# dbking77/ar_slam

Hardware: AMD Instinct MI355X
Metric: LM iterations/sec + ms-to-converged reproj-RMS, 10k-capture synthetic graph (higher is better)
Workload: dtype f64

## Files before the change

### ar_slam_amd/csrc/lm_capi.hip

```cpp
#include "lm_handle.h"

arslam_lm::~arslam_lm() {
  for (auto &t : timers) t.destroy();
  for (auto e : upd_events) (void)hipEventDestroy(e);
  if (ev_sync) (void)hipEventDestroy(ev_sync);
  for (auto e : cov_ev)
    if (e) (void)hipEventDestroy(e);
  arslam::selinv_plan_free(cov_sp);
  for (auto e : pair_ev)
    if (e) (void)hipEventDestroy(e);
  arslam::tile_solve_plan_free(cov_tp);
  arslam::llt_plan_free(plan);
  if (comm) (void)ncclCommDestroy(comm);
  if (stream) (void)hipStreamDestroy(stream);
}


namespace {
thread_local std::string g_last_error;
}
namespace arslam {
void set_last_error(const std::string &msg) { g_last_error = msg; }
}
namespace {
// ... 310 lines not shown
            "parameter block is not part of the problem");
    fail_if(!h->pk_loaded || h->pk_dirty, ARSLAM_E_STATE,
            "covariance_block: no completed arslam_lm_solve of the problem as it stands");
    if (!h->cov_valid) h->covariance();
    if (key == h->camera_ptr) {
      std::fill(cov, cov + 9, 0.0);
      cov[0] = h->cov_var_f;
      const bool ok = h->cov_var_f >= 0.0;
      if (!ok) std::fill(cov, cov + 9, -1.0);
      if (status)
        *status = ok ? ARSLAM_COV_OK
                     : h->cov_info.status == ARSLAM_COV_RANK_DEFICIENT && !h->constant.count(key) ? ARSLAM_COV_RANK_DEFICIENT
                                                                                                   : ARSLAM_COV_UNAVAILABLE;
      return;
    }
    const bool is_cap = ci != h->cap_of.end();
    const int i = is_cap ? ci->second : ti->second;
    const std::vector<double> &c = is_cap ? h->cov_cap : h->cov_tag;
    const std::vector<int> &st = is_cap ? h->cov_cap_status : h->cov_tag_status;
    fail_if((size_t)i >= st.size(), ARSLAM_E_STATE, "covariance_block: the block is not part of the solved problem");
    std::memcpy(cov, c.data() + 36L * i, 36 * sizeof(double));
    if (status) *status = st[i];
  });
}

int arslam_lm_covariance_pairs(arslam_lm *h, const arslam_lm_cov_pair *pairs, int n_pairs, double *cov, int *status,
                               arslam_lm_cov_info *info) {
  if (!h || n_pairs < 0 || (n_pairs > 0 && (!pairs || !cov))) return ARSLAM_E_INVALID_ARG;
  return guarded([&] { h->covariance_pairs(pairs, n_pairs, cov, status, info); });
}

int arslam_lm_covariance_block_pair(arslam_lm *h, const double *block_a, const double *block_b, double *cov,
                                    int *status) {
  if (!h || !block_a || !block_b || !cov) return ARSLAM_E_INVALID_ARG;
  return guarded([&] {
    arslam_lm_cov_pair pr{};
    int size[2] = {6, 6};
    const double *blocks[2] = {block_a, block_b};
    for (int s = 0; s < 2; ++s) {
      double *key = const_cast<double *>(blocks[s]);
      const auto ci = h->cap_of.find(key);
      const auto ti = h->tag_of.find(key);
      fail_if(key != h->camera_ptr && ci == h->cap_of.end() && ti == h->tag_of.end(), ARSLAM_E_INVALID_ARG,
              "parameter block is not part of the problem");
      const int kind = key == h->camera_ptr ? ARSLAM_BLOCK_CAMERA : ci != h->cap_of.end() ? ARSLAM_BLOCK_CAPTURE : ARSLAM_BLOCK_TAG;
      const int index = kind == ARSLAM_BLOCK_CAMERA ? 0 : kind == ARSLAM_BLOCK_CAPTURE ? ci->second : ti->second;
      if (kind == ARSLAM_BLOCK_CAMERA) size[s] = 3;
      (s == 0 ? pr.kind_a : pr.kind_b) = kind;
      (s == 0 ? pr.index_a : pr.index_b) = index;
    }
    fail_if(!h->pk_loaded || h->pk_dirty, ARSLAM_E_STATE,
            "covariance_block_pair: no completed arslam_lm_solve of the problem as it stands");
    double c[36];
    int st = ARSLAM_COV_UNAVAILABLE;
    h->covariance_pairs(&pr, 1, c, &st, nullptr);
    const int ra = size[0], cb = size[1];
    if (st != ARSLAM_COV_OK) {
      std::fill(cov, cov + ra * cb, -1.0);
    } else {
      std::fill(cov, cov + ra * cb, 0.0);
      if (ra == 6 && cb == 6) std::copy(c, c + 36, cov);
      else if (ra == 3 && cb == 6) std::copy(c, c + 6, cov);
      else if (ra == 6 && cb == 3) for (int r = 0; r < 6; ++r) cov[3 * r] = c[r];
      else cov[0] = c[0];
    }
    if (status) *status = st;
  });
}

int arslam_lm_debug_reduced_rows(arslam_lm *h, int *cap_row, int *tag_row, int *cam_row) {
  if (!h) return ARSLAM_E_INVALID_ARG;
  return guarded([&] {
    fail_if(!h->loaded || h->multi() || h->elim_used == ARSLAM_ELIM_MIXED, ARSLAM_E_STATE,
            "reduced_rows: a one-rank problem loaded with capture or tag elimination");
    const bool swapped = h->elim_used == ARSLAM_ELIM_TAGS;
    int *e_row = swapped ? tag_row : cap_row, *f_row = swapped ? cap_row : tag_row;
    for (int c = 0; c < h->nc && e_row; ++c) e_row[c] = -1;
    for (int t = 0; t < h->nt && f_row; ++t) f_row[t] = (size_t)t < h->lay.tag_row.size() ? h->lay.tag_row[t] : -1;
    if (cam_row) *cam_row = h->has_f ? h->P.cam_row : -1;
  });
}

int arslam_comm_unique_id(unsigned char id[ARSLAM_COMM_ID_BYTES]) {
  if (!id) return ARSLAM_E_INVALID_ARG;
  return guarded([&] {
    static_assert(sizeof(ncclUniqueId) <= ARSLAM_COMM_ID_BYTES, "id size");
    ncclUniqueId u;
    NCCL_CHECK(ncclGetUniqueId(&u));
    std::memset(id, 0, ARSLAM_COMM_ID_BYTES);
    std::memcpy(id, &u, sizeof(u));
  });
}

int arslam_lm_set_comm_callback(arslam_lm *h, int rank, int nranks, arslam_allreduce_fn fn, void *ctx) {
  if (!h || nranks < 1 || rank < 0 || rank >= nranks || ((nranks > 1 || h->force_multi) && !fn))
    return ARSLAM_E_INVALID_ARG;
  return guarded([&] {
    if (h->comm) { (void)ncclCommDestroy(h->comm); h->comm = nullptr; }
    h->rank = rank;
    h->nranks = nranks;
    h->comm_cb = h->multi() ? fn : nullptr;
    h->comm_cb_ctx = ctx;
    h->loaded = false;
    h->pk_dirty = true;
  });
}

int arslam_lm_set_comm(arslam_lm *h, int rank, int nranks, const unsigned char id[ARSLAM_COMM_ID_BYTES]) {
  if (!h || !id || nranks < 1 || rank < 0 || rank >= nranks) return ARSLAM_E_INVALID_ARG;
  return guarded([&] {
    h->ensure_stream();
    if (h->comm) { (void)ncclCommDestroy(h->comm); h->comm = nullptr; }
    h->comm_cb = nullptr;
    h->rank = rank;
    h->nranks = nranks;
    h->loaded = false;
    h->pk_dirty = true;
    if (h->multi()) {
      ncclUniqueId u;
      std::memcpy(&u, id, sizeof(u));
      NCCL_CHECK(ncclCommInitRank(&h->comm, nranks, u, rank));
    }
  });
}

int arslam_lm_owned_captures(const arslam_lm *h, int *out, int cap, int *n) {
  if (!h || !n || (cap > 0 && !out)) return ARSLAM_E_INVALID_ARG;
  if (!h->loaded) return ARSLAM_E_STATE;
  const int k = h->multi() ? (int)h->own_caps.size() : h->nc_user;
  for (int i = 0; i < k && i < cap; ++i) out[i] = h->multi() ? h->own_caps[i] : i;
  *n = k;
  return ARSLAM_OK;
}

int arslam_device_count(void) {
  int n = 0;
  if (hipGetDeviceCount(&n) != hipSuccess) return 0;
  return n;
}

int arslam_lm_set_iteration_callback(arslam_lm *h, arslam_iteration_callback fn, void *ctx) {
  if (!h) return ARSLAM_E_INVALID_ARG;
  h->iter_cb = fn;
  h->iter_cb_ctx = ctx;
  return ARSLAM_OK;
}

int arslam_lm_debug_force_indefinite(arslam_lm *h, unsigned long long step_mask) {
  if (!h) return ARSLAM_E_INVALID_ARG;
  h->dbg_indefinite_mask = step_mask;
  return ARSLAM_OK;
}

int arslam_lm_debug_force_multirank(arslam_lm *h, int on) {
  if (!h || (on != 0 && on != 1)) return ARSLAM_E_INVALID_ARG;
  return guarded([&] {
    if (h->comm) { (void)ncclCommDestroy(h->comm); h->comm = nullptr; }
    h->comm_cb = nullptr;
    h->rank = 0;
    h->nranks = 1;
    h->force_multi = on != 0;
    h->loaded = false;
    h->pk_dirty = true;
  });
}

int arslam_lm_debug_break_dependency(arslam_lm *h, long ticket, long *broken) {
  if (!h || ticket < 0) return ARSLAM_E_INVALID_ARG;
  return guarded([&] {
    fail_if(!h->loaded || !h->has_f || h->opt.factor_executor != 1, ARSLAM_E_STATE,
            "break_dependency needs a loaded problem on the persistent executor");
    arslam::LltPlan &pl = h->plan;
    long t = ticket;
    while (t < pl.n_dag_tasks && pl.h_dag_wait_off[t] == pl.h_dag_wait_off[t + 1]) ++t;
    fail_if(t >= pl.n_dag_tasks, ARSLAM_E_INVALID_ARG, "no task at or after this ticket waits on anything");
    const int w = pl.h_dag_wait_off[t];
    h->restore_patched_wait();
    pl.h_dag_waits[w].y += 1 << 28;
    h->dbg_patched_wait = w;
    HIP_CHECK(hipMemcpyAsync(pl.dag_waits + w, &pl.h_dag_waits[w], sizeof(int2), hipMemcpyHostToDevice,
                             h->stream));
    HIP_CHECK(hipStreamSynchronize(h->stream));
    if (broken) *broken = t;
  });
}

int arslam_lm_debug_tag_pair_tile(arslam_lm *h, const double *tag_a, const double *tag_b, int *status) {
  if (!h || !tag_a || !tag_b || !status) return ARSLAM_E_INVALID_ARG;
  return guarded([&] {
    fail_if(!h->loaded || h->multi() || h->elim_used != ARSLAM_ELIM_CAPTURES || !h->has_f, ARSLAM_E_STATE,
            "tag_pair_tile needs a pointer-keyed problem loaded with capture elimination on one rank");
    const auto ia = h->tag_of.find(const_cast<double *>(tag_a)), ib = h->tag_of.find(const_cast<double *>(tag_b));
    *status = -1;
    if (ia == h->tag_of.end() || ib == h->tag_of.end()) return;
    const int ra = h->lay.tag_row[ia->second], rb = h->lay.tag_row[ib->second];
    if (ra < 0 || rb < 0) return;
    const int T = h->lay.T;
    int st = 2;
    for (int x : {ra, ra + 5})
      for (int y : {rb, rb + 5}) {
        int ti = x / 64, tj = y / 64;
        if (ti < tj) std::swap(ti, tj);
        const int id = h->plan.h_tile_id[(size_t)ti * T + tj];
        st = std::min(st, id < 0 ? 0 : (id < h->plan.n_assembled ? 2 : 1));
      }
    *status = st;
  });
}

const char *arslam_lm_last_error(void) { return g_last_error.c_str(); }

#ifndef ARSLAM_BUILD_ID
#define ARSLAM_BUILD_ID "unknown"
#endif
const char *arslam_lm_version(void) { return "arslam_lm 0.2 (gfx950, fp64) build " ARSLAM_BUILD_ID; }

}
```

### ar_slam_amd/csrc/lm_handle.h

```cpp
#pragma once
#include "host_threads.h"
#include "lm_internal.h"
#include "loss.h"
#include "arslam_lm.h"
#include "arslam_lm_debug.h"

#include <rccl/rccl.h>

#include <algorithm>
#include <atomic>
#include <cfloat>
#include <chrono>
#include <cmath>
#include <cstddef>
#include <cstdio>
#include <cstdlib>
#include <cstring>
#include <memory>
#include <stdexcept>
#include <string>
#include <unordered_map>
#include <thread>
#include <unordered_set>
#include <vector>

namespace arslam {
namespace lmh {

using Error = arslam::ApiError;

#define HIP_CHECK(expr)                                                                      \
  do {                                                                                       \
    hipError_t _e = (expr);                                                                  \
    if (_e != hipSuccess)                                                                    \
      throw Error(_e == hipErrorOutOfMemory ? ARSLAM_E_OUT_OF_MEMORY : ARSLAM_E_HIP,         \
                  std::string(#expr) + ": " + hipGetErrorString(_e));                       \
  } while (0)

#define NCCL_CHECK(expr)                                                                     \
  do {                                                                                       \
    ncclResult_t _r = (expr);                                                                \
    if (_r != ncclSuccess)                                                                   \
      throw Error(ARSLAM_E_COMM, std::string(#expr) + ": " + ncclGetErrorString(_r));       \
  } while (0)

inline void fail_if(bool cond, int code, const std::string &msg) {
  if (cond) throw Error(code, msg);
}

inline double now_s() {
  return std::chrono::duration<double>(std::chrono::steady_clock::now().time_since_epoch()).count();
}

struct DebugEnv {
  const char *dag_trace = std::getenv("ARSLAM_DAG_TRACE");
  int dag_trace_skip = std::getenv("ARSLAM_DAG_TRACE_SKIP") ? std::atoi(std::getenv("ARSLAM_DAG_TRACE_SKIP")) : 0;
  bool setup_profile = std::getenv("ARSLAM_SETUP_PROFILE") != nullptr;
  bool write_back_dma = std::getenv("ARSLAM_WRITE_BACK_DMA") != nullptr;
};
inline const DebugEnv &debug_env() {
  static const DebugEnv e;
  return e;
}

std::string executor_fault_message(int code, int rank, int iteration, const arslam::LltPlan &plan, hipStream_t s);

template <class T>
struct DevBuf {
  T *p = nullptr;
  size_t n = 0, cap = 0;
  void alloc(size_t count) {
    n = count;
    if (count <= cap) return;
    if (p) (void)hipFree(p);
    p = nullptr;
    cap = 0;
    const size_t want = cap == 0 && count <= 16 ? count : count + count / 2;
    HIP_CHECK(hipMalloc(&p, want * sizeof(T)));
    cap = want;
  }
  void upload(const T *h, size_t count, hipStream_t s) {
    if (count) HIP_CHECK(hipMemcpyAsync(p, h, count * sizeof(T), hipMemcpyHostToDevice, s));
  }
  void release() {
    if (p) (void)hipFree(p);
    p = nullptr;
    n = cap = 0;
  }
  ~DevBuf() { release(); }
};

struct PinnedBuf {
  double *p = nullptr;
  size_t cap = 0;
  void alloc(size_t count) {
    if (count <= cap) return;
    if (p) (void)hipHostFree(p);
    p = nullptr;
    cap = 0;
    const size_t want = count + count / 2;
    HIP_CHECK(hipHostMalloc(&p, want * sizeof(double), hipHostMallocDefault));
    cap = want;
  }
  ~PinnedBuf() {
    if (p) (void)hipHostFree(p);
  }
};

struct UploadArena {
  char *dev = nullptr, *host = nullptr;
  size_t dev_cap = 0, host_cap = 0;
  struct Piece { void **dst; const void *src; size_t bytes, off; };
  std::vector<Piece> pieces;
  hipEvent_t copied = nullptr;
  template <class T>
  void add(T **dst, const T *src, size_t count) { pieces.push_back({reinterpret_cast<void **>(dst), src, count * sizeof(T), 0}); }
  void commit(hipStream_t s) {
    if (copied) HIP_CHECK(hipEventSynchronize(copied));
    size_t used = 0;
    for (Piece &p : pieces) {
      p.off = used;
      used += (std::max<size_t>(p.bytes, 1) + 255) & ~size_t(255);
    }
    if (used > host_cap) {
      if (host) (void)hipHostFree(host);
      host = nullptr;
      host_cap = 0;
      HIP_CHECK(hipHostMalloc(&host, used + used / 2, hipHostMallocDefault));
      host_cap = used + used / 2;
    }
    if (used > dev_cap) {
      if (dev) (void)hipFree(dev);
      dev = nullptr;
      dev_cap = 0;
      HIP_CHECK(hipMalloc(&dev, used + used / 2));
      dev_cap = used + used / 2;
    }
    for (Piece &p : pieces) {
      if (p.bytes) std::memcpy(host + p.off, p.src, p.bytes);
      *p.dst = dev + p.off;
    }
    if (used) {
      HIP_CHECK(hipMemcpyAsync(dev, host, used, hipMemcpyHostToDevice, s));
      if (!copied) HIP_CHECK(hipEventCreateWithFlags(&copied, hipEventDisableTiming));
      HIP_CHECK(hipEventRecord(copied, s));
    }
    pieces.clear();
  }
  ~UploadArena() {
    if (copied) (void)hipEventDestroy(copied);
    if (dev) (void)hipFree(dev);
    if (host) (void)hipHostFree(host);
  }
};

struct Timer {
  hipEvent_t a = nullptr, b = nullptr;
  double acc_ms = 0.0;
  bool pending = false;
  bool on = true;
  void init() {
    if (!a) {
      HIP_CHECK(hipEventCreateWithFlags(&a, hipEventDisableSystemFence));
      HIP_CHECK(hipEventCreateWithFlags(&b, hipEventDisableSystemFence));
    }
  }
  void start(hipStream_t s) {
    if (on) HIP_CHECK(hipEventRecord(a, s));
  }
  void stop(hipStream_t s) {
    if (!on) return;
    HIP_CHECK(hipEventRecord(b, s));
    pending = true;
  }
  void collect() {
    if (!pending) return;
    float ms = 0.f;
    HIP_CHECK(hipEventSynchronize(b));
    HIP_CHECK(hipEventElapsedTime(&ms, a, b));
    acc_ms += ms;
    pending = false;
  }
  void destroy() {
    if (a) (void)hipEventDestroy(a);
    if (b) (void)hipEventDestroy(b);
    a = b = nullptr;
  }
};

enum { PH_LIN, PH_SCHUR, PH_CHOL, PH_SOLVE, PH_BACK, PH_COST, PH_FAC0, PH_FAC1, PH_N };

}
}
using namespace arslam::lmh;

struct arslam_lm {
  arslam_lm_options opt;

  double *camera_ptr = nullptr;
  std::unordered_map<double *, int> cap_of, tag_of;
  std::vector<double *> cap_ptrs, tag_ptrs;
  std::vector<int> pk_obs_cap, pk_obs_tag;
  std::vector<double> pk_corners;
  std::vector<unsigned char> pk_loss_kind;
  std::vector<double> pk_loss_a;
  int def_loss_kind = ARSLAM_LOSS_NONE;
  double def_loss_a = 0.0;
  std::vector<unsigned char> soa_loss_kind;
  std::vector<double> soa_loss_a;
  arslam::ObsLoss default_obs_loss(int n_obs) {
    if (def_loss_kind == ARSLAM_LOSS_NONE || n_obs <= 0) return arslam::ObsLoss{};
    soa_loss_kind.assign(n_obs, (unsigned char)def_loss_kind);
    soa_loss_a.assign(n_obs, def_loss_a);
    return arslam::ObsLoss{soa_loss_kind.data(), soa_loss_a.data()};
  }
  std::unordered_set<double *> constant;
  bool pk_dirty = true;

  bool loaded = false;
  arslam_soa_problem soa{};
  int nc = 0, nt = 0, nb = 0;
  long n = 0, nR = 0, N = 0;
  bool has_f = false;
  std::vector<unsigned char> slot_free;
  std::vector<double> x0;
  long nb_global = 0;
  double setup_s = 0.0;
  double setup_phase[5] = {0, 0, 0, 0, 0};
  double comm_bytes = 0.0;
  long comm_calls = 0;
  arslam::DevProblem P{};
  hipStream_t stream = nullptr;
  int device = 0;

  UploadArena upload;
  int *u_cap_start = nullptr, *u_obs_tag = nullptr, *u_obs_lblk = nullptr, *u_cap_blk_start = nullptr,
      *u_blk_tag = nullptr, *u_tag_start = nullptr, *u_obs_tpos = nullptr, *u_tag_row = nullptr,
      *u_row_slot = nullptr, *u_fslot_row = nullptr, *u_dest_start = nullptr, *u_big_caps = nullptr;
  unsigned char *u_f_own = nullptr;
  unsigned char *u_cap_kind = nullptr;
  int *u_f_alias = nullptr;
  std::vector<unsigned char> f_own;
  std::vector<int> big_caps;
  std::vector<int> chunk_caps;
  int *u_chunk_caps = nullptr;
  unsigned char *u_obs_active = nullptr, *u_slot_free = nullptr;
  double *u_corners = nullptr, *u_x0 = nullptr;
  unsigned char *u_loss_kind = nullptr;
  double *u_loss_a = nullptr;
  long *u_cap_off = nullptr;
  int2 *u_dest_row = nullptr;
  int4 *u_gather_items = nullptr, *u_gather_splits = nullptr;
  arslam::SchurContrib *u_contrib = nullptr;
  long n_clear = 0;
  DevBuf<double> d_xa, d_xb, d_xbest, d_g, d_colnorm, d_scale, d_diag;
  DevBuf<double> d_obs_tg, d_parts, d_fparts, d_red, d_S, d_z, d_yF;
  double *Sp = nullptr;
  long s_pre = 0;
  int *u_top_slots = nullptr;
  int n_top_slots = 0;
  long top_tail_len() const { return 2L * n_top_slots + 2; }
  double *d_norms_p = nullptr;
  DevBuf<int> d_flag;
  DevBuf<double> d_slab, d_jrows, d_cap_ui;
  DevBuf<double> d_gather_part;
  arslam::LltPlan plan;
  double *x = nullptr, *xc = nullptr, *xbest = nullptr;
  unsigned long long dbg_indefinite_mask = 0;
  arslam_iteration_callback iter_cb = nullptr;
  void *iter_cb_ctx = nullptr;
  int n_fparts = 0;

  Timer timers[PH_N];
  arslam::LaunchTiming upd_timing;
  std::vector<hipEvent_t> upd_events;
  double dom_ms = 0.0, dom_flops = 0.0;
  double scalar_flops = 0.0;
  long dom_launches = 0;

  void timing_begin();
  void timing_collect();

  int rank = 0, nranks = 1;
  ncclComm_t comm = nullptr;
  bool force_multi = false;
  bool multi() const { return nranks > 1 || force_multi; }

  ~arslam_lm();

  arslam_allreduce_fn comm_cb = nullptr;
  void *comm_cb_ctx = nullptr;
  std::vector<unsigned char> comm_stage;

  void allreduce_any(void *buf, size_t count, int dtype, int op);
  void allreduce(double *buf, size_t count, int op) { allreduce_any(buf, count, ARSLAM_DT_F64, op); }

  DevBuf<double> d_split_hash;
  void check_same_split(const arslam::RankSplit &sp);

  int dag_workgroups = 512;
  const DebugEnv &env = debug_env();

  int cus_device = -1, cus = 0;
  std::thread::id ready_thread{};
  int ready_opt_device = -2;
  void ensure_stream();

  void load(const arslam_soa_problem *p, const arslam::ObsLoss &in_loss);
  int choose_side(const arslam::SchurSide &cs);
  void local_rank_problem(const arslam_soa_problem *p, const arslam::ObsLoss &in_loss, bool can_reuse,
                          arslam::HostProblem &h, arslam::ReducedLayout &L, std::vector<int> &col_class);
  void upload_problem(const arslam::HostProblem &h, const arslam::ReducedLayout &L, int extend_from = -1);
  void alloc_solve_buffers();
  arslam::SchurGather sg;
  bool sg_ready = false;
  bool try_append(const arslam_soa_problem *p, const arslam::ObsLoss &in_loss);
  bool append_as_captures(const arslam_soa_problem *p);
  bool append_as_mixed(const arslam_soa_problem *p, arslam::MixedProblem &m);
  bool same_reduced_rows(const arslam::HostProblem &h) const;
  bool groups_fit_plan(const arslam::HostProblem &h, const std::vector<int> &groups) const;
  bool order_outgrown(const arslam::HostProblem &h, const std::vector<int> &groups);
  arslam::ReducedLayout lay;
  bool pk_appended_only = false;
  int setup_kind = ARSLAM_SETUP_LOAD;
  int elim_used = ARSLAM_ELIM_CAPTURES;
  arslam::MixedProblem mx;
  int ceres_e_cap = 0, ceres_e_tag = 0;
  void reload_values(const arslam_soa_problem *p);
  bool pk_loaded = false;
  int nc_full = 0;
  int nc_user = 0;
  std::vector<int> own_caps;
  std::vector<double> loc_cap, loc_corners;
  std::vector<int> loc_obs_cap, loc_obs_tag;
  std::vector<unsigned char> loc_cap_const;
  std::vector<unsigned char> loc_loss_kind;
  std::vector<double> loc_loss_a;
  double split_top_work = 0.0, split_max_rank_work = 0.0, split_total_work = 0.0;
  int split_active = 1;
  std::vector<uint64_t> covis;
  long covis_nt = 0, covis_edges = 0;
  void covis_build(const arslam::HostProblem &h, const arslam::ReducedLayout &L);
  void covis_add(const arslam::HostProblem &h, const arslam::ReducedLayout &L, int c);
  bool reuse_order = false;
  std::vector<int> prev_tag_row;
  std::vector<int> prev_mx_tag_row, prev_mx_cap_row;
  int prev_ordering = -1, prev_skip = -1;
  long prev_order_edges = 0;
  int prev_order_nc = 0;
  bool last_order_reused = false;
  int prev_order_height = 0;
  static int etree_height(const arslam::ReducedLayout &L);
  void linearize(double *x_cost, double *fixed_cost, double *gmax, double *gnorm, double *xnorm);
  void linearize_launch();
  void linearize_collect(double *x_cost, double *fixed_cost, double *gmax, double *gnorm, double *xnorm);
  bool lin_xpending = false, norms_pending = false;
  DevBuf<double> d_lx, d_ag;
  static constexpr int kLinSave = 16 + 8 + 6 * arslam::kNormBlocks;
  void complete_pending_lin();
  void lin_norms();
  void exchange_scalars(arslam::AgFields fl, arslam::HostOut *ho = nullptr);
  void exchange_norms() {
    if (norms_pending) exchange_scalars(arslam::AgFields{});
  }
  PinnedBuf h_lin;
  double lin_seq = 0.0;
  void lin_sync() {
    if (!multi() && lin_seq > 0.0) flag_sync(h_lin.p + 16 + arslam::kHostSeq, lin_seq);
    else spin_sync();
  }
  bool diag_in_lin = false;
  PinnedBuf h_x;
  PinnedBuf h_step;
  hipEvent_t ev_sync = nullptr;
  void spin_sync() {
    if (!ev_sync) HIP_CHECK(hipEventCreateWithFlags(&ev_sync, hipEventDisableTiming));
    HIP_CHECK(hipEventRecord(ev_sync, stream));
    hipError_t e;
    while ((e = hipEventQuery(ev_sync)) == hipErrorNotReady) {
    }
    HIP_CHECK(e);
  }
  double host_seq = 0.0;
  DevBuf<int> d_seq_done;
  double next_seq(double *word) {
    *(volatile double *)word = -1.0;
    return host_seq += 1.0;
  }
  void flag_sync(const double *word, double seq) {
    for (long k = 1;; ++k) {
      if (*(const volatile double *)word == seq) break;
      if ((k & 4095) == 0) {
        const hipError_t e = hipStreamQuery(stream);
        if (e == hipErrorNotReady) continue;
        HIP_CHECK(e);
        if (*(const volatile double *)word == seq) break;
        throw Error(ARSLAM_E_DEVICE, "the stream finished without storing the host sequence word");
      }
    }
    std::atomic_thread_fence(std::memory_order_acquire);
  }
  void solve(arslam_lm_summary *s);
  void begin_solve(arslam_lm_summary *s);
  double enqueue_step(double radius, bool reuse_diag, int solve_index);
  bool prepare_step(bool reuse_diag, arslam::ExecReset *er);
  void factor_reduced(long first_store, bool record, double radius = 0.0, bool force_indefinite = false);
  void dump_dag_trace(long first_store);
  void back_substitute(double radius);
  double reduce_step_scalars();
  void fill_summary(arslam_lm_summary *s);
  void write_back(const double *d_src);
  const arslam_soa_problem *pk_stage = nullptr;
  void scatter_to_blocks();
  int dbg_patched_wait = -1;
  void restore_patched_wait();
  bool any_iter_cb = false;
  DevBuf<double> d_cb;
  int agree_callback(int r);

  int solve_state = 0;
  arslam::SelinvPlan cov_sp;
  bool cov_sp_ready = false;
  DevBuf<double> d_cov_Z, d_cov_Q, d_cov_Y, d_cov_R, d_cov_out, d_cov_diag;
  DevBuf<int> d_cov_status;
  hipEvent_t cov_ev[5] = {nullptr, nullptr, nullptr, nullptr, nullptr};
  bool cov_valid = false;
  std::vector<double> cov_cap, cov_tag;
  std::vector<int> cov_cap_status, cov_tag_status;
  double cov_var_f = -1.0;
  arslam_lm_cov_info cov_info{};
  void covariance();
  void cov_invalidate() {
    solve_state = 0;
    cov_valid = false;
  }
  struct CovFactor {
    std::vector<int> cap_start;
    bool deficient = false;
    bool factored = false;
    arslam_lm_cov_info info{};
  };
  bool cov_e_free(int c) const { return slot_free[3 + 6L * c] != 0; }
  bool cov_f_free(int t) const { return slot_free[3 + 6L * nc + 6L * t] != 0; }
  void cov_check_state(const char *who) const;
  void cov_factor(CovFactor &cf);
  void cov_numeric_test(CovFactor &cf);

  arslam::TileSolvePlan cov_tp;
  bool cov_tp_ready = false;
  static constexpr int kCovBatchPanels = 16;
  static constexpr size_t kCovBatchBytes = 256u << 20;
  DevBuf<unsigned char> d_pair_mask;
  DevBuf<double> d_pair_B, d_pair_out;
  DevBuf<int2> d_pair_rhs;
  DevBuf<arslam::CovPairTask> d_pair_tasks;
  DevBuf<int> d_pair_status;
  std::vector<hipEvent_t> pair_ev;
  void covariance_pairs(const arslam_lm_cov_pair *pairs, int n_pairs, double *cov, int *status,
                        arslam_lm_cov_info *info);
};
```

### ar_slam_amd/csrc/lm_internal.h

```cpp
#pragma once
#include <hip/hip_runtime.h>
#include <algorithm>
#include <climits>
#include <cstdint>
#include <stdexcept>
#include <vector>

#include "host_structure.h"

namespace arslam {
constexpr int kCuFlags = 2048;
constexpr int kDagOffTicket0 = 0;
constexpr int kDagOffInflight = 1;
constexpr int kDagOffCuFlags = 2;
constexpr int kDagOffTicket1 = 2 + kCuFlags;
constexpr int kDagOffFault = 3 + kCuFlags;
enum DagFaultField {
  kFaultTicket = 0,
  kFaultKind = 1,
  kFaultCounter = 2,
  kFaultSeen = 3,
  kFaultNeed = 4,
  kFaultDrawn = 5,
  kFaultInflight = 6,
// ... 93 lines not shown
  const int4 *gather_splits;
  double *gather_part;
  int n_items, n_splits;
  const signed char *tile_class;
  const unsigned char *f_own = nullptr;
  double *jrows;
  double *cap_ui;
  const unsigned char *obs_loss_kind = nullptr;
  const double *obs_loss_a = nullptr;
};

__device__ inline double *reduced_elem(double *S, const DevProblem &P, long r, long c) {
  return S + (long)P.tile_id[(r >> 6) * P.T + (c >> 6)] * 4096 + (r & 63) * 64 + (c & 63);
}

#ifndef ARSLAM_NORM_BLOCKS
#define ARSLAM_NORM_BLOCKS 64
#endif
constexpr int kNormBlocks = ARSLAM_NORM_BLOCKS;
static_assert(kNormBlocks <= 256 && (kNormBlocks & (kNormBlocks - 1)) == 0, "k_slot_norms: one 256-thread tree");

enum DagRecField {
  kRecType = 0, kRecY, kRecZ, kRecW,
  kRecSub, kRecLate, kRecWait0, kRecWait1,
  kRecCont, kRecContAkk, kRecMaxdep,
  kRecContMaxdep, kRecContWait0, kRecContLate,
  kRecQ0 = 16, kRecQ1,
  kRecFoldK0, kRecFoldTile0,
  kRecSid = 18, kRecTi, kRecTj,
  kRecSplitN, kRecSplitP,
  kRecTile0I, kRecTile0J,
  kDagRecInts = 32
};

enum DagTraceWord {
  kTrDraw = 0,
  kTrMet = 1,
  kTrEnd = 2,
  kTrWg = 3,
  kTrLoaded = 4,
  kTrFactored = 5,
  kTrPublished = 6,
  kTrSubPublished = 7,
  kDagTraceWords = 8
};
enum DagProgressSlot {
  kProgTicket = 0,
  kProgPhase = 1,
  kProgType = 2,
  kDagProgressInts = 4
};

struct LltPlan {
  char *arena = nullptr;
  size_t arena_bytes = 0;
  int T = 0;
  long lda = 0;
  int nlev = 0;
  int2 *panel = nullptr;
  int2 *upd_targets = nullptr;
  int *upd_kstart = nullptr;
  int *upd_ks = nullptr;
  int4 *upd_items = nullptr;
  int2 *upd_split = nullptr;
  int *upd_cnt = nullptr;
  double *upd_part = nullptr;
  long n_split = 0, n_part = 0;
  std::vector<int> h_item_off;
  int *bs_cols = nullptr;
  int2 *bs_gather = nullptr;
  int *bs_gbeg = nullptr;
  int *bs_gtile = nullptr;
  double *bs_part = nullptr;
  int *bs_counters = nullptr;
  int *tile_id = nullptr;
  std::vector<int> h_tile_id;
  long n_tiles = 0;
  long n_assembled = 0;
  bool fill_first_ok = false;
  int n_phases = 1;
  long phase_split = 0;
  long n_top_tiles = 0;
  std::vector<int> h_col_class;
  std::vector<int> h_dag_phase;
  signed char *tile_class = nullptr;
  double *ldiag = nullptr;
  std::vector<int> h_panel_off;
  std::vector<int> h_upd_off;
  std::vector<int> h_bs_off;
  std::vector<int> h_bsg_off;
  std::vector<double> h_upd_flops;
  std::vector<int2> h_dag_sub;
  int *dag_claimed = nullptr;
  std::vector<int> h_dag_cont, h_dag_maxdep, h_dag_cont_akk;
  int *dag_rec = nullptr;
  int2 *dag_ks_tiles = nullptr;
  std::vector<int> h_dag_rec;
  std::vector<int2> h_dag_ks_tiles;
  int2 *dag_waits = nullptr;
  int *dag_counters = nullptr;
  long n_dag_tasks = 0;
  std::vector<int4> h_dag_tasks;
  std::vector<int> h_dag_wait_off;
  std::vector<int2> h_dag_waits;
  std::vector<int2> h_panel, h_targets, h_gather, h_split;
  std::vector<int> h_kstart, h_ks, h_bcols, h_gbeg, h_gtile;
  std::vector<int4> h_items;
  double total_upd_flops = 0.0;
  double total_factor_flops = 0.0;
  long total_upd_tiles = 0;
};

void llt_plan_symbolic(LltPlan &plan, int T, long lda, std::vector<uint8_t> &pattern,
                       const std::vector<int> *col_class = nullptr);
void tile_fill(int T, std::vector<uint8_t> &pattern, std::vector<int> &parent);
struct RankSplit {
  std::vector<int> col_owner;
  std::vector<int> cap_owner;
  int n_top_cols = 0;
  int n_active = 0;
  double top_work = 0.0, max_rank_work = 0.0, total_work = 0.0;
  std::vector<int> col_class(int rank) const {
    std::vector<int> c(col_owner.size());
    for (size_t k = 0; k < c.size(); ++k) c[k] = col_owner[k] < 0 ? 1 : (col_owner[k] == rank ? 0 : 2);
    return c;
  }
};
RankSplit rank_split(const HostProblem &h, const ReducedLayout &L, int nranks);
bool dag_check(const LltPlan &plan);
bool dag_simulate(const LltPlan &plan, int n_workers, unsigned seed, int policy = 0, int n_started = -1);
constexpr int kDagSimPolicies = 4;
constexpr int kDagSimNoCap = 16;
constexpr int kDagSimGridCap = 32;
std::string dag_fault_detail(const LltPlan &plan, const int *rec);
void llt_plan_upload(LltPlan &plan, hipStream_t s);
void llt_plan_build(LltPlan &plan, int T, long lda, std::vector<uint8_t> &pattern, hipStream_t s,
                    const std::vector<int> *col_class = nullptr);
void llt_plan_free(LltPlan &plan);
void llt_plan_reset(LltPlan &plan);


struct ExecReset;
void launch_linearize(const DevProblem &P, const double *x, double *g, double *colnorm,
                      double *obs_tg, double *parts, hipStream_t s);
void launch_lin_reduce(const DevProblem &P, const double *obs_tg, double *g, double *colnorm,
                       const double *parts, double *out, hipStream_t s, double *hout = nullptr,
                       double *save = nullptr);
struct LmDiagArgs;
void launch_scale(const DevProblem &P, const double *colnorm, int jacobi, double *scale,
                  hipStream_t s, const LmDiagArgs *ld = nullptr);
void launch_lm_diag(const DevProblem &P, const double *scale, const double *colnorm, double dmin,
                    double dmax, double *diag, hipStream_t s);
void set_schur_big_lds_attribute();
void launch_schur(const DevProblem &P, const double *x, const double *scale, const double *diag,
                  double radius, double *S, hipStream_t s, bool prep = false, long zero_tiles = 0,
                  const ExecReset *er = nullptr);
void launch_schur_gather(const DevProblem &P, const double *diag, double radius, double *S, hipStream_t s);
void launch_prep_reduced(const DevProblem &P, const double *diag, double radius, double *S,
                         hipStream_t s, int which = -1);
void launch_mask_y(const DevProblem &P, double *yF, int rank, hipStream_t s, bool keep_top = false);
void launch_own_copy(const DevProblem &P, long first, long count, const double *src, double *dst, hipStream_t s);
void launch_backsub(const DevProblem &P, const double *x, const double *scale, const double *diag,
                    double radius, const double *yF, double *xc, double *parts, hipStream_t s,
                    bool reuse_ui = false, bool with_cost = false);
void launch_update_f(const DevProblem &P, const double *x, const double *scale, const double *yF,
                     double *xc, double *fparts, hipStream_t s);
void launch_cost(const DevProblem &P, const double *x, double *parts, hipStream_t s);
void launch_copy_out(const double *src, long n, double *dst, int *seq_done, double *word, double seq, hipStream_t s);
void launch_reduce_parts(const double *parts, int nc, const double *fparts, int nfparts,
                         double *out, hipStream_t s, const int *flag = nullptr,
                         double *hout = nullptr, int *seq_done = nullptr, double seq = 0.0);
void debug_set_reduced_diag(const DevProblem &P, double *S, long row, double v, hipStream_t s);
struct PackSegs {
  int n = 0;
  double *p[4] = {nullptr, nullptr, nullptr, nullptr};
  long len[4] = {0, 0, 0, 0}, off[4] = {0, 0, 0, 0};
  void add(double *ptr, long count) {
    p[n] = ptr;
    len[n] = count;
    off[n] = n ? off[n - 1] + len[n - 1] : 0;
    ++n;
  }
  long total() const { return n ? off[n - 1] + len[n - 1] : 0; }
};
void launch_pack(const PackSegs &sg, double *buf, bool unpack, hipStream_t s);
void launch_top_tail(const int *idx, int m, double *g, double *cn, double *red, double *tail, bool unpack,
                     hipStream_t s);
constexpr int kAgFields = 32;
struct AgFields {
  int n = 0;
  int idx[kAgFields] = {};
  unsigned max = 0;
  void add(int i, bool is_max) {
    if (n >= kAgFields) throw std::logic_error("AgFields: more than kAgFields scalars");
    if (is_max) max |= 1u << n;
    idx[n++] = i;
  }
};
void launch_ag_put(const double *src, const AgFields &fl, double *ag, int nranks, int rank, hipStream_t s);
struct HostOut {
  const double *src[3] = {};
  double *dst[3] = {};
  int len[3] = {};
  int n = 0;
  double *seq_word = nullptr;
  double seq = 0.0;
  void add(const double *s, double *d, int l) {
    if (n >= 3) throw std::logic_error("HostOut: more than 3 ranges");
    src[n] = s;
    dst[n] = d;
    len[n++] = l;
  }
};
void launch_ag_reduce(const double *ag, const AgFields &fl, double *dst, int nranks, hipStream_t s,
                      const HostOut *ho = nullptr);
void launch_slot_norms(const DevProblem &P, const double *red, double *g, double *colnorm, const double *x,
                       double *out, hipStream_t s, double *hout = nullptr, const LmDiagArgs *ld = nullptr,
                       double seq = 0.0);
constexpr int kHostSeq = 15;

struct LaunchTiming {
  hipEvent_t *ev = nullptr;
  int cap = 0;
  int used = 0;
  double flops = 0.0;
};

void launch_dense_llt(const LltPlan &P, double *S, int *flag, hipStream_t s,
                      LaunchTiming *timing = nullptr);
void set_dag_workgroup_limit(int k);
inline int dag_launch_grid(long n_tasks, int n_workgroups) {
  return (int)std::min<long>(n_workgroups, std::max<long>(std::min<long>(64, n_tasks), n_tasks / 4));
}
void launch_dense_llt_dag(const LltPlan &P, double *S, int *flag, hipStream_t s, int n_workgroups,
                          int *progress = nullptr, unsigned long long *trace = nullptr, bool reset = true,
                          int phase = -1, long first_store = LONG_MAX);
struct LmDiagArgs {
  long n;
  const double *scale, *colnorm;
  double dmin, dmax;
  double *diag;
  double *ysent = nullptr;
  long nys = 0;
};
constexpr unsigned long long kYSentinel = 0x7ff47ff47ff47ff4ull;
void launch_exec_reset(const LltPlan &P, int *flag, hipStream_t s, const LmDiagArgs *ld = nullptr);
struct ExecReset {
  int *flag = nullptr;
  int *a = nullptr, *b = nullptr, *c = nullptr, *d = nullptr;
  long na = 0, nb = 0, nc = 0, nd = 0;
  double *ysent = nullptr;
  long nys = 0;
  __host__ __device__ long n() const { return na + nb + nc + nd > nys ? na + nb + nc + nd : nys; }
};
ExecReset exec_reset_args(const LltPlan &P, int *flag, double *ysent, long nys);
__device__ __forceinline__ void exec_reset_elem(const ExecReset &r, long e) {
  if (e < r.nys) r.ysent[e] = __longlong_as_double((long long)kYSentinel);
  if (e < r.na) r.a[e] = 0;
  else if (e < r.na + r.nb) r.b[e - r.na] = 0;
  else if (e < r.na + r.nb + r.nc) r.c[e - r.na - r.nb] = 0;
  else if (e < r.na + r.nb + r.nc + r.nd) r.d[e - r.na - r.nb - r.nc] = 0;
  if (e == 0 && r.flag) *r.flag = 0;
}
void launch_dense_back_solve(const LltPlan &P, const double *S, long nR, double *z, double *yF,
                             const int *flag, hipStream_t s);
void launch_dense_back_solve_dag(const LltPlan &P, const double *S, long nR, double *yF, int *flag,
                                 hipStream_t s, int n_workgroups, bool reset = true);
void launch_zero_tiles(const LltPlan &P, double *S, hipStream_t s);
void launch_scatter_diag(const LltPlan &P, double *S, hipStream_t s);

struct SelinvPlan {
  int *gcol = nullptr;
  long n_products = 0;
};
void selinv_plan_build(const LltPlan &P, SelinvPlan &sp, hipStream_t s);
void selinv_plan_free(SelinvPlan &sp);
void launch_selinv(const LltPlan &P, const SelinvPlan &sp, double *S, long nR, double *Z, const int *flag,
                   hipStream_t s);
void launch_cov_blocks(const DevProblem &P, const double *Z, const double *scale, const double *Gb, const double *Rb,
                       double *cov_e, int *status_e, double *cov_f, double *var_f, const int *flag, hipStream_t s);
void launch_cov_schur(const DevProblem &P, const double *scale, double *Qb, double *Gb, double *Rb, bool write_slab,
                      hipStream_t s);

struct TileSolvePlan {
  int *fbeg = nullptr;
  int2 *flist = nullptr;
  std::vector<int> h_fbeg;
  std::vector<int2> h_flist;
  std::vector<int> parent;
};
void tile_solve_plan_build(const LltPlan &P, TileSolvePlan &tp, hipStream_t s);
void tile_solve_plan_free(TileSolvePlan &tp);
void tile_solve_mark(const TileSolvePlan &tp, unsigned char *mask, long row);
long tile_solve_products(const LltPlan &P, const TileSolvePlan &tp, const unsigned char *active,
                         const unsigned char *needed);
void launch_tile_solve(const LltPlan &P, const TileSolvePlan &tp, const double *S, long nR, double *B, int n_panels,
                       const unsigned char *active, const unsigned char *needed, const int *flag, hipStream_t s);
enum { kCovFocal = 0, kCovF = 1, kCovE = 2 };
constexpr int kCovPanelBlocks = 10;
void launch_cov_pair_rhs(const DevProblem &P, const double *Gb, const double *Rb, const int2 *rhs, int n_rhs,
                         double *B, hipStream_t s);
struct CovPairTask {
  int role_a, idx_a, role_b, idx_b, slot, out;
};
void launch_cov_pair_blocks(const DevProblem &P, const double *X, const double *scale, const double *Gb,
                            const double *Rb, const CovPairTask *tasks, int n_tasks, double *out, int *status,
                            const int *flag, hipStream_t s);

}
// ... 1 lines not shown
```

### ar_slam_amd/csrc/lm_kernels.hip

```cpp
#include "lm_internal.h"
#include "projection.h"
#include "loss.h"
#include "schur_store_table.h"

#include <cfloat>
#include <mutex>
#include <string>
#include <vector>

#include "arslam_lm.h"
#include <cmath>

namespace arslam {

#ifdef ARSLAM_SCHUR_STAMPS
__device__ unsigned long long g_schur_ph[16];
#define SCHUR_STAMP_INIT unsigned long long _st0 = clock64()
#define SCHUR_STAMP(k)                                                         \
  do {                                                                         \
    const unsigned long long _n = clock64();                                   \
    if (threadIdx.x == 0) atomicAdd(&g_schur_ph[k], _n - _st0);                \
    _st0 = _n;                                                                 \
  } while (0)
void debug_read_schur_stamps(unsigned long long *out) {
  (void)hipMemcpyFromSymbol(out, HIP_SYMBOL(g_schur_ph), sizeof(g_schur_ph));
}
#else
#define SCHUR_STAMP_INIT do {} while (0)
#define SCHUR_STAMP(k) do {} while (0)
void debug_read_schur_stamps(unsigned long long *out) {
  for (int i = 0; i < 16; ++i) out[i] = 0;
}
#endif

namespace {

__device__ const SchurStoreTable g_schur_store = make_schur_store_table();

__device__ __forceinline__ long slot_cap(const DevProblem &P, int c) { return 3 + 6L * c; }
__device__ __forceinline__ long slot_tag(const DevProblem &P, int t) { return 3 + 6L * P.nc + 6L * t; }

__device__ __forceinline__ bool group_swapped(const DevProblem &P, int c) {
  return P.cap_kind ? P.cap_kind[c] == kMixTag : P.swap_roles != 0;
}
__device__ __forceinline__ bool group_direct(const DevProblem &P, int c) {
  return P.cap_kind && P.cap_kind[c] == kMixDirect;
}

__device__ __forceinline__ double lm_d2(const double *diag, long slot, double radius) {
  const double d = sqrt(diag[slot] / radius);
  return d * d;
}

__device__ __forceinline__ double robustify_row(int kind, double a, double &r, double J[13]) {
  const double s = obs_sum8(r * r);
  double rho, rho1;
  loss_eval(kind, a, s, &rho, &rho1);
  const double w = sqrt(rho1);
#pragma unroll
  for (int j = 0; j < 13; ++j) J[j] *= w;
  r *= w;
  return rho;
}

template <bool kLoss = false>
__device__ __forceinline__ void fill_rows(const DevProblem &P, const double *x, const double *scale, int c,
                          int o0, int row0, int nr, int nrows, double *rows, double *gout = nullptr,
                          double *ocost = nullptr) {
  const double *cam = x;
  const double *cap = x + slot_cap(P, c);
  for (int lr = threadIdx.x; lr < nr; lr += kWave) {
    const int row = row0 + lr;
    const int q = row >> 3, corner = (row >> 1) & 3, comp = row & 1;
    const int obs = o0 + q;
    const int t = P.obs_tag[obs];
    const double *tag = x + slot_tag(P, t);
    double J[13];
    const bool sw = group_swapped(P, c);
    double r = residual_jacobian_row(cam, sw ? tag : cap, sw ? cap : tag, corner, comp,
                                     P.corners[8L * obs + 2 * corner + comp], J);
    if (kLoss) {
      const double rho = robustify_row(P.obs_loss_kind[obs], P.obs_loss_a[obs], r, J);
      if (ocost && (lr & 7) == 0) ocost[lr >> 3] = 0.5 * rho;
    }
    if (sw) {
#pragma unroll
      for (int j = 1; j < 7; ++j) {
        const double v = J[j];
        J[j] = J[j + 6];
        J[j + 6] = v;
      }
    }
    double *dst = rows + (long)lr * kRowStride;
    if (scale) {
      const double *sc = scale + slot_cap(P, c);
      const double *st = scale + slot_tag(P, t);
      dst[0] = J[0] * scale[0];
#pragma unroll
      for (int j = 0; j < 6; ++j) {
        dst[1 + j] = J[1 + j] * sc[j];
        dst[7 + j] = J[7 + j] * st[j];
      }
    } else {
#pragma unroll
      for (int j = 0; j < 13; ++j) dst[j] = J[j];
    }
    dst[13] = r;
    if (gout) {
      double *g = gout + 8L * o0 * kJStored + row;
#pragma unroll
      for (int j = 0; j < 13; ++j)
        if (j < 7 || j > 9) g[(long)jrow_col(j) * nrows] = J[j];
      g[(long)jrow_col(13) * nrows] = r;
    }
  }
}

__device__ __forceinline__ void load_rows_q(const DevProblem &P, const double *scale, const double *yF, double yf, int c, int o0,
                            int row0, int nr, int nrows, double *rows, double *qv) {
  const double *sc = scale + slot_cap(P, c);
  for (int lr = threadIdx.x; lr < nr; lr += kWave) {
    const int row = row0 + lr;
    const double *g = P.jrows + 8L * o0 * kJStored + row;
    const int t = P.obs_tag[o0 + (row >> 3)];
    const int tr = P.tag_row[t];
    double u[kJStored], v[14];
#pragma unroll
    for (int j = 0; j < kJStored; ++j) u[j] = g[(long)j * nrows];
#pragma unroll
    for (int j = 0; j < 14; ++j) v[j] = u[jrow_col(j)];
    const double *st = scale + slot_tag(P, t);
    double yt[6];
#pragma unroll
    for (int j = 0; j < 6; ++j) yt[j] = tr >= 0 ? yF[tr + j] : 0.0;
    double *dst = rows + (long)lr * kRowStride;
    double d[14];
    d[0] = v[0] * scale[0];
#pragma unroll
    for (int j = 0; j < 6; ++j) {
      d[1 + j] = v[1 + j] * sc[j];
      d[7 + j] = v[7 + j] * st[j];
    }
    d[13] = v[13];
#pragma unroll
    for (int j = 0; j < 14; ++j) dst[j] = d[j];
    double q = d[0] * yf;
    if (tr >= 0) {
#pragma unroll
      for (int j = 0; j < 6; ++j) q += d[7 + j] * yt[j];
    }
    qv[lr] = q;
  }
}

#ifdef ARSLAM_BACKSUB_RECOMPUTE
template <bool kLoss>
__device__ __forceinline__ void eval_rows_q(const DevProblem &P, const double *x, const double *scale, const double *yF,
                                            double yf, int c, int o0, int row0, int nr, int nrows, double *rows,
                                            double *qv) {
  fill_rows<kLoss>(P, x, scale, c, o0, row0, nr, nrows, rows);
  for (int lr = threadIdx.x; lr < nr; lr += kWave) {
    const int row = row0 + lr;
    const int tr = P.tag_row[P.obs_tag[o0 + (row >> 3)]];
    const double *d = rows + (long)lr * kRowStride;
    double q = d[0] * yf;
    if (tr >= 0) {
#pragma unroll
      for (int j = 0; j < 6; ++j) q += d[7 + j] * yF[tr + j];
    }
    qv[lr] = q;
  }
}
#define ARSLAM_BACKSUB_ROWS(...) eval_rows_q<kLoss>(P, x, __VA_ARGS__)
#else
#define ARSLAM_BACKSUB_ROWS(...) load_rows_q(P, __VA_ARGS__)
#endif

__device__ __forceinline__ void upper6(int e, int &a, int &b) {
  a = 0;
  int rem = e;
  while (rem >= 6 - a) { rem -= 6 - a; ++a; }
  b = a + rem;
}

__device__ void inv6(const double *U, double *Ui) {
  double L[36];
#pragma unroll
  for (int i = 0; i < 36; ++i) L[i] = U[i];
#pragma unroll
  for (int j = 0; j < 6; ++j) {
    double xj = L[6 * j + j];
#pragma unroll
    for (int p = 0; p < j; ++p) xj -= L[6 * j + p] * L[6 * j + p];
    const double d = sqrt(xj);
    L[6 * j + j] = d;
#pragma unroll
    for (int i = j + 1; i < 6; ++i) {
      double v = L[6 * i + j];
#pragma unroll
      for (int p = 0; p < j; ++p) v -= L[6 * i + p] * L[6 * j + p];
      L[6 * i + j] = v / d;
    }
  }
#pragma unroll
  for (int col = 0; col < 6; ++col) {
    double e[6];
#pragma unroll
    for (int i = 0; i < 6; ++i) {
      double v = (i == col) ? 1.0 : 0.0;
#pragma unroll
      for (int p = 0; p < i; ++p) v -= L[6 * i + p] * e[p];
      e[i] = v / L[6 * i + i];
    }
#pragma unroll
    for (int i = 5; i >= 0; --i) {
      double v = e[i];
#pragma unroll
      for (int p = i + 1; p < 6; ++p) v -= L[6 * p + i] * e[p];
      e[i] = v / L[6 * i + i];
    }
#pragma unroll
    for (int i = 0; i < 6; ++i) Ui[6 * i + col] = e[i];
  }
}


__device__ __forceinline__ double row_prod(const double *rr, int ca, int cb) {
#pragma clang fp contract(off)
  return rr[ca] * rr[cb];
}

template <bool kChunked>
__device__ __forceinline__ int chunk_capture(const DevProblem &P, int &k) {
  const int c = kChunked ? P.chunk_caps[blockIdx.x] : (int)blockIdx.x;
  k = P.cap_start[c + 1] - P.cap_start[c];
  return (!kChunked && k > kObsChunk) ? -1 : c;
}

template <bool kChunked, bool kLoss>
__global__ __launch_bounds__(kWave) __attribute__((amdgpu_waves_per_eu(4, 8))) void k_linearize(DevProblem P, const double *__restrict__ x,
                                                     double *__restrict__ g,
                                                     double *__restrict__ colnorm,
                                                     double *__restrict__ obs_tg,
                                                     double *__restrict__ parts) {
  extern __shared__ __attribute__((aligned(16))) double sm[];
  const int c = kChunked ? P.chunk_caps[blockIdx.x] : (int)blockIdx.x, lane = threadIdx.x;
  const int o0 = P.cap_start[c], k = P.cap_start[c + 1] - o0;
  if (!kChunked && k > kObsChunk) return;
  const int nrows = 8 * k;
  double *rows = sm;
  double *ocost = rows + (long)8 * kObsChunk * kRowStride;
  double *accs = ocost + kObsChunk;
  auto chunk = [&](int q0) __attribute__((always_inline)) {
    const int kc = min(kObsChunk, k - q0), nr = 8 * kc;
    fill_rows<kLoss>(P, x, nullptr, c, o0, 8 * q0, nr, nrows, rows, P.jrows, kLoss ? ocost : nullptr);
    __syncthreads();
    for (int e = lane; e < 13 * kc; e += kWave) {
      const int q = e / 13, it = e % 13;
      const double *rq = rows + (long)q * 8 * kRowStride;
      const int ca = it == 0 ? 13 : it <= 6 ? 6 + it : it, cb = it <= 6 ? 13 : it;
      double s = 0.0;
#pragma unroll
      for (int rr = 0; rr < 8; ++rr) s += rq[rr * kRowStride + ca] * rq[rr * kRowStride + cb];
      if (it == 0) {
        if (!kLoss) ocost[q] = 0.5 * s;
      }
      else obs_tg[12L * P.obs_tpos[o0 + q0 + q] + (it - 1)] = s;
    }
    if (lane < 14) {
      const int ca = lane < 6 ? 1 + lane : lane < 12 ? lane - 5 : 0;
      const int cb = lane < 6 ? 13 : lane < 12 ? lane - 5 : lane == 12 ? 13 : 0;
      double ps = q0 ? accs[lane] : 0.0;
#pragma unroll 8
      for (int r = 0; r < nr; ++r) ps += row_prod(rows + (long)r * kRowStride, ca, cb);
      accs[lane] = ps;
    }
    __syncthreads();
    if (lane == 0) {
      double act = q0 ? accs[14] : 0.0, fix = q0 ? accs[15] : 0.0;
      for (int q = 0; q < kc; ++q) {
        if (P.obs_active[o0 + q0 + q]) act += ocost[q]; else fix += ocost[q];
      }
      accs[14] = act;
      accs[15] = fix;
    }
  };
  if (!kChunked) {
    chunk(0);
  } else {
    for (int q0 = 0; q0 < k; q0 += kObsChunk) {
      if (q0) __syncthreads();
      chunk(q0);
    }
  }
  if (lane < 14) {
    const double ps = k ? accs[lane] : 0.0;
    if (lane < 12) {
      const long slot = slot_cap(P, c) + (lane % 6);
      const double v = P.slot_free[slot] ? ps : 0.0;
      if (lane < 6) g[slot] = v; else colnorm[slot] = v;
    } else if (lane == 12) {
      parts[(long)P_GF * P.nc + c] = ps;
    } else {
      parts[(long)P_CF * P.nc + c] = ps;
    }
  }
  if (lane == 0) {
    parts[(long)P_COST * P.nc + c] = k ? accs[14] : 0.0;
    parts[(long)P_FIXED * P.nc + c] = k ? accs[15] : 0.0;
  }
}

__device__ __forceinline__ void tag_reduce_elem(const DevProblem &P, const double *__restrict__ obs_tg, long e,
                                                double *__restrict__ g, double *__restrict__ colnorm) {
  if (e >= 12L * P.nt) return;
  const int t = (int)(e / 12), j = (int)(e % 12);
  double s = 0.0;
  const int qa = P.tag_start[t], qb = P.tag_start[t + 1];
  for (int q0 = qa; q0 < qb; q0 += 32) {
    double v[32];
#pragma unroll
    for (int u = 0; u < 32; ++u) v[u] = obs_tg[12L * min(q0 + u, qb - 1) + j];
#pragma unroll
    for (int u = 0; u < 32; ++u) s += (q0 + u < qb) ? v[u] : 0.0;
  }
  const long slot = slot_tag(P, t) + (j % 6);
  if (P.f_alias) {
    const int d = P.f_alias[t];
    if (d >= 0) {
      double *dv = (j < 6 ? g : colnorm) + slot_cap(P, d) + (j % 6);
      s += *dv;
      *dv = P.slot_free[slot] ? s : 0.0;
    }
  }
  const double v = P.slot_free[slot] ? s : 0.0;
  if (j < 6) g[slot] = v; else colnorm[slot] = v;
}

__global__ void k_scale(long n, const unsigned char *__restrict__ free_, const double *__restrict__ colnorm,
                        int jacobi, double *__restrict__ scale, double dmin, double dmax, double *__restrict__ diag) {
  const long i = (long)blockIdx.x * blockDim.x + threadIdx.x;
  if (i >= n) return;
  const double sv = free_[i] ? (jacobi ? 1.0 / (1.0 + sqrt(colnorm[i])) : 1.0) : 0.0;
  scale[i] = sv;
  if (diag) diag[i] = fmin(fmax(sv * sv * colnorm[i], dmin), dmax);
}

__global__ void k_lm_diag(long n, const double *__restrict__ scale, const double *__restrict__ colnorm,
                          double dmin, double dmax, double *__restrict__ diag) {
  const long i = (long)blockIdx.x * blockDim.x + threadIdx.x;
  if (i >= n) return;
  const double d = scale[i] * scale[i] * colnorm[i];
  diag[i] = fmin(fmax(d, dmin), dmax);
}

__device__ void store_direct_group(double *out, int nblk, int m, const double *U, const double *Etr, const double *W,
                                   const double *Ftr, const double *FF, double ff00, int lane) {
  const int own = nblk - 1;
  auto cls = [&](int x, int &u, int &i) {
    u = x >= 1 && x < m ? (x - 1) / 6 : 0;
    i = x >= 1 && x < m ? (x - 1) - 6 * u : 0;
    return x == 0 ? 0 : x == m ? 3 : (u == own ? 2 : 1);
  };
  for (int Ub = 0; Ub <= nblk + 1; ++Ub) {
    const int sU = schur_blk_size(Ub, nblk), p0 = schur_blk_start(Ub, nblk), ncol = p0 + sU;
    double *dst = out + schur_block_off(Ub, 0, nblk);
    for (int e = lane; e < sU * ncol; e += kWave) {
      const int ip = e / ncol, q = e - ip * ncol, p = p0 + ip;
      int ua, ia, ub, ib;
      int ka = cls(q, ua, ia), kb = cls(p, ub, ib);
      if (ka > kb || (ka == kb && q > p)) {
        const int tk = ka, tu = ua, ti = ia;
        ka = kb; ua = ub; ia = ib;
        kb = tk; ub = tu; ib = ti;
      }
      double v = 0.0;
      if (ka == 0) {
        v = kb == 0 ? ff00 : kb == 1 ? FF[28 * ub + 21 + ib] : kb == 2 ? W[ib * m] : Ftr[0];
      } else if (ka == 1) {
        if (kb == 1) {
          if (ua == ub) {
            const int lo = min(ia, ib), hi = max(ia, ib);
            v = FF[28 * ua + lo * 6 - lo * (lo - 1) / 2 + (hi - lo)];
          }
        } else {
          v = kb == 2 ? W[ib * m + 1 + 6 * ua + ia] : Ftr[1 + 6 * ua + ia];
        }
      } else if (ka == 2) {
        v = kb == 2 ? U[6 * ia + ib] : Etr[ia];
      }
      const int V = schur_blk(q, m), q0V = schur_blk_start(V, nblk);
      dst[(long)sU * q0V + ip * schur_blk_size(V, nblk) + (q - q0V)] = v;
    }
  }
}

template <bool kBig>
__global__ __launch_bounds__(kWave) void k_schur(DevProblem P, const double *__restrict__ scale,
                                                 const double *__restrict__ diag, double radius,
                                                 double *__restrict__ zero_tiles, long n_zero, ExecReset er,
                                                 const int *__restrict__ cap_list) {
  extern __shared__ __attribute__((aligned(16))) double sm[];
  SCHUR_STAMP_INIT;
  const int c = kBig ? cap_list[blockIdx.x] : (int)blockIdx.x, lane = threadIdx.x;
  if (c >= P.nc + n_zero) {
    exec_reset_elem(er, (long)(c - P.nc - n_zero) * kWave + lane);
    return;
  }
  if (c >= P.nc) {
    typedef double d2 __attribute__((ext_vector_type(2)));
    d2 *z = reinterpret_cast<d2 *>(zero_tiles + (long)(c - P.nc) * 4096);
#pragma unroll 8
    for (int e = lane; e < 2048; e += kWave) z[e] = d2{0.0, 0.0};
    return;
  }
  const int o0 = P.cap_start[c], k = P.cap_start[c + 1] - o0;
  if (k == 0) return;
  const int nrows = 8 * k;
  const int b0 = P.cap_blk_start[c], nblk = P.cap_blk_start[c + 1] - b0;
  if (!kBig && nblk > kSchurMfmaBlocks) return;
  const int m = 1 + 6 * nblk;
  const SchurLds lds = schur_lds(nblk);
  double *stage = sm;
  double *tscale = sm + lds.tscale;
  double *U = sm + lds.U;
  double *Ui = sm + lds.Ui;
  double *Etr = sm + lds.Etr;
  double *W = sm + lds.W;
  double *Ftr = sm + lds.Ftr;
  double *FF = sm + lds.FF;
  int *lblk = (int *)(sm + lds.lblk);
  double *ff00 = sm + lds.ff00;

  const int li = lane & 15, lk = lane >> 4;
  const bool valid = li < 14;
  const double *jb = P.jrows + 8L * o0 * kJStored + (long)jrow_col(min(li, 13)) * nrows;
  double jv[16];
#pragma unroll
  for (int u = 0; u < 8; ++u)
#pragma unroll
    for (int st = 0; st < 2; ++st)
      jv[2 * u + st] = (valid && u < k) ? jb[8 * u + 4 * st + lk] : 0.0;
  static_assert(kObsChunk == 8, "k_schur's operand registers hold eight observations");
  auto stage_chunk = [&](int q0) {
    const int kc = min(kObsChunk, k - q0);
    if (lane < kc) lblk[lane] = P.obs_lblk[o0 + q0 + lane];
    if (lane < 6 * kc) tscale[lane] = scale[slot_tag(P, P.obs_tag[o0 + q0 + lane / 6]) + lane % 6];
  };
  stage_chunk(0);
  __syncthreads();
  SCHUR_STAMP(0);
  {
    for (int e = lane; e < 6 * m + m + (m & 1) + 28 * nblk; e += kWave) W[e] = 0.0;
    __builtin_amdgcn_fence(__ATOMIC_RELEASE, "wavefront");
    __builtin_amdgcn_wave_barrier();
    __builtin_amdgcn_fence(__ATOMIC_ACQUIRE, "wavefront");
    typedef double dbl4v __attribute__((ext_vector_type(4)));
    dbl4v tot = {0, 0, 0, 0};
    const double *sc = scale + slot_cap(P, c);
    const double cs = li == 0 ? scale[0] : li <= 6 ? sc[li - 1] : 1.0;
    const bool tagcol = li >= 7 && li <= 12;
    int acc_off[4], acc_stride[4];
    const int w_base = (int)(W - sm);
    {
      const int c = li, ftr0 = 6 * m, ff0 = ftr0 + m + (m & 1);
#pragma unroll
      for (int reg = 0; reg < 4; ++reg) {
        const int r = lk + 4 * reg;
        int off = -1, st = 0;
        if (r >= 1 && r <= 6 && c >= 7 && c <= 12) { off = (r - 1) * m + 1 + (c - 7); st = 6; }
        else if (r >= 7 && r <= 12 && c == 13) { off = ftr0 + 1 + (r - 7); st = 6; }
        else if (r >= 7 && r <= 12 && c >= r && c <= 12) {
          const int a = r - 7, b = c - 7;
          off = ff0 + a * 6 - a * (a - 1) / 2 + (b - a); st = 28;
        } else if (r == 0 && c >= 7 && c <= 12) { off = ff0 + 21 + (c - 7); st = 28; }
        acc_off[reg] = off >= 0 ? w_base + off : 0;
        acc_stride[reg] = st;
      }
    }
    for (int q = 0; q < k; ++q) {
      if ((q & 7) == 0 && q > 0) {
#pragma unroll
        for (int u = 0; u < 8; ++u)
#pragma unroll
          for (int st = 0; st < 2; ++st)
            jv[2 * u + st] = (valid && q + u < k) ? jb[8 * (q + u) + 4 * st + lk] : 0.0;
        stage_chunk(q);
        __builtin_amdgcn_fence(__ATOMIC_RELEASE, "wavefront");
        __builtin_amdgcn_wave_barrier();
        __builtin_amdgcn_fence(__ATOMIC_ACQUIRE, "wavefront");
      }
      dbl4v g = {0, 0, 0, 0};
      const double s = tagcol ? tscale[6 * (q & 7) + li - 7] : cs;
#pragma unroll
      for (int st = 0; st < 2; ++st) {
        double v = 0.0;
        switch (q & 7) {
          case 0: v = jv[0 + st]; break;
          case 1: v = jv[2 + st]; break;
          case 2: v = jv[4 + st]; break;
          case 3: v = jv[6 + st]; break;
          case 4: v = jv[8 + st]; break;
          case 5: v = jv[10 + st]; break;
          case 6: v = jv[12 + st]; break;
          default: v = jv[14 + st]; break;
        }
        v = li == 13 ? v : v * s;
        g = __builtin_amdgcn_mfma_f64_16x16x4f64(v, v, g, 0, 0, 0);
      }
      tot += g;
      const int u = lblk[q & 7] - 1;
      int di[4];
      double dv[4];
#pragma unroll
      for (int reg = 0; reg < 4; ++reg) {
        di[reg] = acc_off[reg] + acc_stride[reg] * u;
        dv[reg] = sm[di[reg]];
      }
#pragma unroll
      for (int reg = 0; reg < 4; ++reg) sm[di[reg]] = dv[reg] + g[reg];
      __builtin_amdgcn_fence(__ATOMIC_RELEASE, "wavefront");
      __builtin_amdgcn_wave_barrier();
      __builtin_amdgcn_fence(__ATOMIC_ACQUIRE, "wavefront");
    }
#pragma unroll
    for (int reg = 0; reg < 4; ++reg) {
      const int r = lk + 4 * reg, c = li;
      const double v = tot[reg];
      if (r >= 1 && r <= 6 && c >= 1 && c <= 6) U[6 * (r - 1) + (c - 1)] = v;
      else if (r >= 1 && r <= 6 && c == 13) Etr[r - 1] = v;
      else if (r >= 1 && r <= 6 && c == 0) W[(r - 1) * m] = v;
      else if (r == 0 && c == 13) Ftr[0] = v;
      else if (r == 0 && c == 0) *ff00 = v;
    }
  }
  __syncthreads();
  SCHUR_STAMP(1);
  if (group_direct(P, c)) {
    store_direct_group(P.slab + P.cap_off[c], nblk, m, U, Etr, W, Ftr, FF, *ff00, lane);
    return;
  }
  {
    const long sc = slot_cap(P, c);
    double L[21];
    double rd[6];
    int e = 0;
#pragma unroll
    for (int i = 0; i < 6; ++i)
#pragma unroll
      for (int j = 0; j <= i; ++j) L[e++] = U[6 * i + j] + (i == j ? lm_d2(diag, sc + i, radius) : 0.0);
#define LI6(i, j) L[(i) * ((i) + 1) / 2 + (j)]
#pragma unroll
    for (int j = 0; j < 6; ++j) {
      double d = LI6(j, j);
#pragma unroll
      for (int p = 0; p < j; ++p) d -= LI6(j, p) * LI6(j, p);
      const double sd = sqrt(d);
      rd[j] = 1.0 / sd;
      LI6(j, j) = sd;
#pragma unroll
      for (int i = j + 1; i < 6; ++i) {
        double v = LI6(i, j);
#pragma unroll
        for (int p = 0; p < j; ++p) v -= LI6(i, p) * LI6(j, p);
        LI6(i, j) = v * rd[j];
      }
    }
    if (lane < 6) {
      double ev[6];
#pragma unroll
      for (int i = 0; i < 6; ++i) {
        double v = (i == lane) ? 1.0 : 0.0;
#pragma unroll
        for (int p = 0; p < i; ++p) v -= LI6(i, p) * ev[p];
        ev[i] = v * rd[i];
      }
#pragma unroll
      for (int i = 5; i >= 0; --i) {
        double v = ev[i];
#pragma unroll
        for (int p = i + 1; p < 6; ++p) v -= LI6(p, i) * ev[p];
        ev[i] = v * rd[i];
      }
#pragma unroll
      for (int i = 0; i < 6; ++i) Ui[6 * i + lane] = ev[i];
    }
#undef LI6
  }
  __syncthreads();
  if (lane < 36) P.cap_ui[36L * c + lane] = Ui[lane];
  SCHUR_STAMP(2);
  SCHUR_STAMP(3);
  double *out = P.slab + P.cap_off[c];
  auto make_z = [&](int q, double z[6]) {
    if (q < m) {
      double wq[6];
#pragma unroll
      for (int b = 0; b < 6; ++b) wq[b] = W[b * m + q];
#pragma unroll
      for (int a = 0; a < 6; ++a) {
        double s = 0.0;
#pragma unroll
        for (int b = 0; b < 6; ++b) s += Ui[6 * a + b] * wq[b];
        z[a] = s;
      }
    } else {
#pragma unroll
      for (int a = 0; a < 6; ++a) z[a] = 0.0;
    }
  };
  const bool one_chunk = !kBig;
  typedef unsigned int u4v __attribute__((ext_vector_type(4)));
  const u4v *desc = reinterpret_cast<const u4v *>(&g_schur_store.e[one_chunk ? nblk - 1 : 0][0][lane][0]);
  u4v dsc[4];
  if (one_chunk) {
    dsc[0] = desc[0];
    dsc[1] = desc[kWave];
  }
  double z[6];
  if (one_chunk) make_z(lane, z);
  if (one_chunk) {
    const int M = m + 1;
    const int li = lane & 15, lk = lane >> 4;
    double *Zs = stage;
    if (lane < M)
#pragma unroll
      for (int a = 0; a < 6; ++a) Zs[a * M + lane] = z[a];
    __builtin_amdgcn_fence(__ATOMIC_RELEASE, "wavefront");
    __builtin_amdgcn_wave_barrier();
    __builtin_amdgcn_fence(__ATOMIC_ACQUIRE, "wavefront");
    double Aop[4][2], Bop[4][2];
#pragma unroll
    for (int r = 0; r < 4; ++r)
#pragma unroll
      for (int kb = 0; kb < 2; ++kb) {
        const int a = 4 * kb + lk, pq = 16 * r + li;
        const bool in = a < 6 && pq < M;
        Aop[r][kb] = in ? (pq < m ? W[a * m + pq] : Etr[a]) : 0.0;
        Bop[r][kb] = in ? Zs[a * M + pq] : 0.0;
      }
    typedef double dbl4v __attribute__((ext_vector_type(4)));
    typedef unsigned int u2v __attribute__((ext_vector_type(2)));
    const __amdgpu_buffer_rsrc_t slab_rsrc =
        __builtin_amdgcn_make_buffer_rsrc(out, 0, (int)(schur_slab_size(nblk) * sizeof(double)), 0x00020000);
#pragma unroll
    for (int r = 0; r < 4; ++r) {
      if (16 * r >= M) break;
      u4v dn[4];
      if (r < 3) {
#pragma unroll
        for (int cc = 0; cc < 4; ++cc)
          if (cc <= r + 2) dn[cc] = desc[(schur_store_row_tile(r + 1) + cc) * kWave];
      }
#pragma unroll
      for (int cc = 0; cc < 4; ++cc) {
        if (cc > r + 1 || 16 * cc >= M) break;
        dbl4v acc = {0, 0, 0, 0};
        acc = __builtin_amdgcn_mfma_f64_16x16x4f64(Aop[r][0], Bop[cc][0], acc, 0, 0, 0);
        acc = __builtin_amdgcn_mfma_f64_16x16x4f64(Aop[r][1], Bop[cc][1], acc, 0, 0, 0);
        double ff[4];
#pragma unroll
        for (int reg = 0; reg < 4; ++reg)
          ff[reg] = *reinterpret_cast<const double *>(
              reinterpret_cast<const char *>(sm) + ((dsc[cc][reg] >> kSchurStoreLdsShift) & kSchurStoreMask));
#pragma unroll
        for (int reg = 0; reg < 4; ++reg)
          __builtin_amdgcn_raw_buffer_store_b64(__builtin_bit_cast(u2v, ff[reg] - acc[reg]), slab_rsrc,
                                                (int)(dsc[cc][reg] & kSchurStoreMask), 0, 0);
      }
      if (r < 3) {
#pragma unroll
        for (int cc = 0; cc < 4; ++cc)
          if (cc <= r + 2) dsc[cc] = dn[cc];
      }
    }
  } else
  for (int U = 0; U <= nblk + 1; ++U) {
    const int sU = schur_blk_size(U, nblk), p0U = schur_blk_start(U, nblk), ncol = p0U + sU;
    double *dst = out + schur_block_off(U, 0, nblk);
    for (int q0 = 0; q0 < ncol; q0 += kWave) {
      const int q = q0 + lane;
      if (!one_chunk) make_z(q, z);
      const int V = schur_blk(min(q, m), m), sV = schur_blk_size(V, nblk), q0V = schur_blk_start(V, nblk);
      const int uq = V - 1, iq = q - q0V;
      if (sU == 6) {
        const int up = U - 1;
        double wv[6][6];
#pragma unroll
        for (int i = 0; i < 6; ++i)
#pragma unroll
          for (int a = 0; a < 6; ++a) wv[i][a] = W[a * m + p0U + i];
#pragma unroll
        for (int i = 0; i < 6; ++i) {
          double s = 0.0;
#pragma unroll
          for (int a = 0; a < 6; ++a) s += wv[i][a] * z[a];
          double ff = 0.0;
          if (q == 0) {
            ff = FF[28 * up + 21 + i];
          } else if (uq == up) {
            const int lo = min(i, iq), hi = max(i, iq);
            ff = FF[28 * up + lo * 6 - lo * (lo - 1) / 2 + (hi - lo)];
          }
          if (q < ncol) dst[6 * q0V + i * sV + (q - q0V)] = ff - s;
        }
      } else {
        const int p = p0U;
        const double *wp = p < m ? W + p : Etr;
        const int st = p < m ? m : 1;
        double s = 0.0;
#pragma unroll
        for (int a = 0; a < 6; ++a) s += wp[a * st] * z[a];
        double ff = 0.0;
        if (p == m) ff = q < m ? Ftr[q] : 0.0;
        else ff = *ff00;
        if (q < ncol) dst[q0V + (q - q0V)] = ff - s;
      }
    }
  }
  SCHUR_STAMP(4);
}

struct GatherLane {
  int E, G, el, grp, i, j;
  __device__ GatherLane(const DevProblem &P, int2 rr, int lane) {
    const int sx = (rr.x == P.nR || rr.x == P.cam_row) ? 1 : 6;
    const int sy = rr.y == P.cam_row ? 1 : 6;
    E = sx * sy;
    G = kWave / E;
    el = lane % E;
    grp = lane / E;
    i = el / sy;
    j = el % sy;
  }
};

__device__ __forceinline__ double gather_groups(double s, const GatherLane &g, double *part, int lane) {
  if (g.G == 1) return s;
  part[lane] = s;
  __builtin_amdgcn_fence(__ATOMIC_RELEASE, "wavefront");
  __builtin_amdgcn_wave_barrier();
  __builtin_amdgcn_fence(__ATOMIC_ACQUIRE, "wavefront");
  double t = 0.0;
  if (lane < g.E)
    for (int q = 0; q < g.G; ++q) t += part[q * g.E + lane];
  return t;
}

__device__ __forceinline__ double prep_d2(const DevProblem &P, const double *diag, double radius, long r,
                                          long col) {
  if (!diag || r != col || r >= P.nR) return 0.0;
  const int slot = P.row_slot[r];
  return slot >= 0 ? lm_d2(diag, slot, radius) : 0.0;
}

__device__ __forceinline__ void prep_pad_row(const DevProblem &P, const double *diag, double radius, double *S,
                                             long i) {
  if (i >= P.N) return;
  if (i < P.nR && P.row_slot[i] >= 0) {
    if (P.cam_row >= 0 && i > P.cam_row && i <= P.cam_row + 2)
      *reduced_elem(S, P, i, i) = lm_d2(diag, P.row_slot[i], radius);
    return;
  }
  *reduced_elem(S, P, i, i) = i == P.nR ? 1e300 : 1.0;
}

__global__ __launch_bounds__(256) void k_schur_gather(DevProblem P, double *__restrict__ S,
                                                      const double *__restrict__ diag, double radius) {
  __shared__ double part[4][kWave];
  __shared__ SchurContrib cts[4][kWave];
  const int w = threadIdx.x >> 6, lane = threadIdx.x & 63;
  const int n_item_blocks = (P.n_items + 3) / 4;
  if (diag && (int)blockIdx.x >= n_item_blocks) {
    prep_pad_row(P, diag, radius, S, (long)(blockIdx.x - n_item_blocks) * 256 + threadIdx.x);
    return;
  }
  const int it = blockIdx.x * 4 + w;
  if (it >= P.n_items) return;
  const int4 item = P.gather_items[it];
  const int2 rr = P.dest_row[item.x];
  const GatherLane g(P, rr, lane);
  const int nk = item.z - item.y;
  const bool staged = nk <= kWave;
  if (staged && lane < nk) cts[w][lane] = P.contrib[item.y + lane];
  __builtin_amdgcn_fence(__ATOMIC_RELEASE, "wavefront");
  __builtin_amdgcn_wave_barrier();
  __builtin_amdgcn_fence(__ATOMIC_ACQUIRE, "wavefront");
  double s = 0.0;
  auto sum = [&](const SchurContrib *src) __attribute__((always_inline)) {
    for (int t0 = g.grp; t0 < nk; t0 += 8 * g.G) {
      double v[8];
#pragma unroll
      for (int u = 0; u < 8; ++u) {
        const int t = min(t0 + u * g.G, nk - 1);
        const SchurContrib ct = src[t];
        v[u] = P.slab[ct.off + (ct.tr ? g.j * ct.ld + g.i : g.i * ct.ld + g.j)];
      }
#pragma unroll
      for (int u = 0; u < 8; ++u) s += (t0 + u * g.G < nk) ? v[u] : 0.0;
    }
  };
  if (g.grp < g.G) {
    if (staged) sum(cts[w]);
    else sum(P.contrib + item.y);
  }
  s = gather_groups(s, g, part[w], lane);
  if (lane >= g.E) return;
  if (item.w >= 0) {
    P.gather_part[(long)item.w * 36 + lane] = s;
  } else {
    const long r = rr.x + g.i, col = rr.y + g.j;
    if (r >= col && !(diag && r == P.nR && col == P.nR)) *reduced_elem(S, P, r, col) = s + prep_d2(P, diag, radius, r, col);
  }
}

__global__ __launch_bounds__(256) void k_schur_combine(DevProblem P, double *__restrict__ S,
                                                       const double *__restrict__ diag, double radius) {
  __shared__ double part[4][kWave];
  const int w = threadIdx.x >> 6, lane = threadIdx.x & 63;
  const int sp = blockIdx.x * 4 + w;
  if (sp >= P.n_splits) return;
  const int4 split = P.gather_splits[sp];
  const int2 rr = P.dest_row[split.x];
  const GatherLane g(P, rr, lane);
  double s = 0.0;
  if (g.grp < g.G) {
    for (int t0 = g.grp; t0 < split.z; t0 += 8 * g.G) {
      double v[8];
#pragma unroll
      for (int u = 0; u < 8; ++u)
        v[u] = P.gather_part[(long)(split.y + min(t0 + u * g.G, split.z - 1)) * 36 + g.el];
#pragma unroll
      for (int u = 0; u < 8; ++u) s += (t0 + u * g.G < split.z) ? v[u] : 0.0;
    }
  }
  s = gather_groups(s, g, part[w], lane);
  const long r = rr.x + g.i, col = rr.y + g.j;
  if (lane < g.E && r >= col && !(diag && r == P.nR && col == P.nR))
    *reduced_elem(S, P, r, col) = s + prep_d2(P, diag, radius, r, col);
}

__global__ void k_prep_reduced(DevProblem P, const double *__restrict__ diag, double radius,
                               double *__restrict__ S, int which) {
  const long i = (long)blockIdx.x * blockDim.x + threadIdx.x;
  if (i >= P.N) return;
  if (which >= 0 && P.tile_class[i >> 6] != which) return;
  double *d = reduced_elem(S, P, i, i);
  if (i < P.nR) {
    const int slot = P.row_slot[i];
    if (slot >= 0) *d += lm_d2(diag, slot, radius);
    else *d = 1.0;
  } else if (i == P.nR) {
    *d = 1e300;
  } else {
    *d = 1.0;
  }
}

__global__ void k_mask_y(DevProblem P, double *__restrict__ yF, int rank, int keep_top) {
  const long i = (long)blockIdx.x * blockDim.x + threadIdx.x;
  if (i >= P.nR) return;
  const int c = P.tile_class[i >> 6];
  if (!(c == 0 || (c == 1 && (rank == 0 || keep_top)))) yF[i] = 0.0;
}

__global__ void k_own_copy(DevProblem P, long first, long count, const double *__restrict__ src,
                           double *__restrict__ dst) {
  const long i = (long)blockIdx.x * blockDim.x + threadIdx.x;
  if (i < count) dst[i] = P.f_own[first + i] ? src[i] : 0.0;
}

template <bool kChunked, bool kLoss>
__device__ __forceinline__ void capture_cost(const DevProblem &P, const double *__restrict__ x, const double *cap,
                                             int c, double *__restrict__ parts) {
  __shared__ double sq[kWave];
  __shared__ double ocost[kObsChunk];
  const int lane = threadIdx.x;
  const int o0 = P.cap_start[c], k = P.cap_start[c + 1] - o0;
  const int nrows = 8 * k;
  const double *cam = x;
  const AngleAxis ac = aa_prepare(cap + 3);
  double bad = 0.0, act = 0.0, fix = 0.0;
  for (int base = 0; base < (kChunked ? nrows : 1); base += kWave) {
    const int row = base + lane;
    double r2 = 0.0;
    if (row < nrows) {
      const int q = row >> 3, corner = (row >> 1) & 3, comp = row & 1;
      const int obs = o0 + q;
      const double *tag = x + slot_tag(P, P.obs_tag[obs]);
      const AngleAxis at = aa_prepare(tag + 3);
      const double obsv = P.corners[8L * obs + 2 * corner + comp];
      const bool sw = group_swapped(P, c);
      const double r = residual_row(sw ? at : ac, sw ? tag : cap, sw ? ac : at, sw ? cap : tag, cam[0], corner,
                                    comp, obsv, nullptr, nullptr);
      if (!isfinite(r)) bad = 1.0;
      r2 = r * r;
    }
    sq[lane] = r2;
    __syncthreads();
    if (lane < 8 && base / 8 + lane < k) {
      double s = 0.0;
#pragma unroll
      for (int rr = 0; rr < 8; ++rr) s += sq[8 * lane + rr];
      if (kLoss) {
        const int obs = o0 + base / 8 + lane;
        double rho1;
        loss_eval(P.obs_loss_kind[obs], P.obs_loss_a[obs], s, &s, &rho1);
      }
      ocost[lane] = 0.5 * s;
    }
    __syncthreads();
    if (kChunked && lane == 0)
      for (int q = base / 8; q < min(k, base / 8 + kObsChunk); ++q) {
        if (P.obs_active[o0 + q]) act += ocost[q - base / 8]; else fix += ocost[q - base / 8];
      }
  }
  if (!kChunked && lane == 0)
    for (int q = 0; q < k; ++q) {
      if (P.obs_active[o0 + q]) act += ocost[q]; else fix += ocost[q];
    }
  bad = wave_max(bad);
  if (lane == 0) {
    parts[(long)P_COST * P.nc + c] = act;
    parts[(long)P_FIXED * P.nc + c] = fix;
    parts[(long)P_CBAD * P.nc + c] = bad;
  }
}

template <bool kChunked, bool kLoss>
__global__ __launch_bounds__(kWave) void k_cost(DevProblem P, const double *__restrict__ x,
                                                double *__restrict__ parts) {
  int k;
  const int c = chunk_capture<kChunked>(P, k);
  if (c < 0) return;
  capture_cost<kChunked, kLoss>(P, x, x + slot_cap(P, c), c, parts);
}

template <bool kChunked, bool kLoss>
__global__ __launch_bounds__(kWave) void k_backsub(DevProblem P, const double *__restrict__ x,
                                                   const double *__restrict__ scale,
                                                   const double *__restrict__ diag, double radius,
                                                   const double *__restrict__ yF,
                                                   double *__restrict__ xc,
                                                   double *__restrict__ parts, int reuse_ui, int with_cost) {
  extern __shared__ __attribute__((aligned(16))) double sm[];
  int k;
  const int c = chunk_capture<kChunked>(P, k), lane = threadIdx.x;
  if (c < 0) return;
  const int o0 = P.cap_start[c];
  const long sc = slot_cap(P, c);
  if (k == 0) {
    if (lane < 6) xc[sc + lane] = x[sc + lane];
    if (lane == 0) {
      parts[(long)P_MODEL * P.nc + c] = 0.0;
      parts[(long)P_STEP2 * P.nc + c] = 0.0;
      parts[(long)P_YBAD * P.nc + c] = 0.0;
      if (with_cost) {
        parts[(long)P_COST * P.nc + c] = 0.0;
        parts[(long)P_FIXED * P.nc + c] = 0.0;
        parts[(long)P_CBAD * P.nc + c] = 0.0;
      }
    }
    return;
  }
  const int nrows = 8 * k;
  constexpr int kChunkRows = 8 * kObsChunk;
  double *rows = sm;
  double *qv = rows + (long)kChunkRows * kRowStride;
  double *U = qv + kChunkRows;
  double *Ui = U + 36;
  double *v = Ui + 36;
  double *yc = v + 8;
  const double yf = P.cam_row >= 0 ? yF[P.cam_row] : 0.0;
  if (reuse_ui && lane < 36) Ui[lane] = P.cap_ui[36L * c + lane];
  auto chunk = [&](int r0) __attribute__((always_inline)) {
    const int nr = min(kChunkRows, nrows - r0);
    ARSLAM_BACKSUB_ROWS(scale, yF, yf, c, o0, r0, nr, nrows, rows, qv);
    __syncthreads();
    const int va = reuse_ui ? lane - 32 : lane - 21;
    if (!reuse_ui && lane < 21) {
      int a, b;
      upper6(lane, a, b);
      double s = r0 ? U[6 * a + b] : 0.0;
      for (int r = 0; r < nr; ++r) s += rows[(long)r * kRowStride + 1 + a] * rows[(long)r * kRowStride + 1 + b];
      U[6 * a + b] = s;
      U[6 * b + a] = s;
    } else if (va >= 0 && va < 6) {
      double s = r0 ? v[va] : 0.0;
      for (int r = 0; r < nr; ++r) {
        const double *rr = rows + (long)r * kRowStride;
        s += rr[1 + va] * (rr[13] - qv[r]);
      }
// ... 60 lines not shown
  double st = 0.0, bad = 0.0;
  double *capc = v;
  if (lane < 6) {
    const double yv = yc[lane];
    const double d = -yv * scale[sc + lane];
    const double xo = x[sc + lane];
    const double xn = xo + d;
    xc[sc + lane] = xn;
    capc[lane] = xn;
    if (P.slot_free[sc + lane] && !direct) st = (xo - xn) * (xo - xn);
    bad = isfinite(yv) ? 0.0 : 1.0;
  }
  st = wave_sum(st);
  bad = wave_max(bad);
  if (lane == 0) {
    parts[(long)P_MODEL * P.nc + c] = mpart;
    parts[(long)P_STEP2 * P.nc + c] = st;
    parts[(long)P_YBAD * P.nc + c] = bad;
  }
  if (with_cost) {
    __syncthreads();
    capture_cost<kChunked, kLoss>(P, xc, capc, c, parts);
  }
}

__device__ __forceinline__ double wave_tree_sum(double v, int n) {
#pragma unroll
  for (int off = 32; off > 0; off >>= 1)
    if (off < n) v += __shfl_down(v, off, kWave);
  return v;
}
__device__ __forceinline__ double wave_tree_max(double v, int n) {
#pragma unroll
  for (int off = 32; off > 0; off >>= 1)
    if (off < n) v = fmax(v, __shfl_down(v, off, kWave));
  return v;
}

__global__ __launch_bounds__(256) void k_update_f(DevProblem P, const double *__restrict__ x,
                                                  const double *__restrict__ scale,
                                                  const double *__restrict__ yF,
                                                  double *__restrict__ xc,
                                                  double *__restrict__ fparts) {
  __shared__ double red[2][256];
  const long i = (long)blockIdx.x * blockDim.x + threadIdx.x;
  double st = 0.0, bad = 0.0;
  const long slot = i < P.nR ? P.row_slot[i] : -1;
  if (slot >= 0) {
    const double yv = yF[i];
    const double xo = x[slot];
    const double xn = xo + (-yv * scale[slot]);
    xc[slot] = xn;
    if (P.slot_free[slot] && (!P.f_own || P.f_own[slot])) st = (xo - xn) * (xo - xn);
    bad = isfinite(yv) ? 0.0 : 1.0;
  }
  if (i < P.nf && P.fslot_row[i] < 0) {
    const long fs = i < 3 ? i : 3 + 6L * P.nc + (i - 3);
    xc[fs] = x[fs];
  }
  if ((long)blockIdx.x * blockDim.x >= P.nR) return;
  red[0][threadIdx.x] = st;
  red[1][threadIdx.x] = bad;
  __syncthreads();
  for (int off = 128; off >= kWave; off >>= 1) {
    if (threadIdx.x < off) {
      red[0][threadIdx.x] += red[0][threadIdx.x + off];
      red[1][threadIdx.x] = fmax(red[1][threadIdx.x], red[1][threadIdx.x + off]);
    }
    __syncthreads();
  }
  if (threadIdx.x < kWave) {
    const double s0 = wave_tree_sum(red[0][threadIdx.x], kWave);
    const double s1 = wave_tree_max(red[1][threadIdx.x], kWave);
    if (threadIdx.x == 0) {
      fparts[2L * blockIdx.x] = s0;
      fparts[2L * blockIdx.x + 1] = s1;
    }
  }
}

__device__ __forceinline__ void reduce_parts_block(int p, const double *__restrict__ parts, int nc,
                                                   const double *__restrict__ fparts, int nfparts,
                                                   double *__restrict__ out, const int *__restrict__ flag,
                                                   double *red, double *__restrict__ hout,
                                                   int *seq_done = nullptr, double seq = 0.0,
                                                   double *__restrict__ save = nullptr) {
  const int t = threadIdx.x;
  const bool is_max = (p == P_YBAD || p == P_CBAD || p == NPART + 1);
  const double *src = p < NPART ? parts + (long)p * nc : fparts;
  const int len = p < NPART ? nc : (fparts ? nfparts : 0);
  const int stride = p < NPART ? 1 : 2, off0 = p < NPART ? 0 : p - NPART;
  double acc = 0.0;
  for (int i0 = t; i0 < len; i0 += 8 * 1024) {
    double v[8];
#pragma unroll
    for (int u = 0; u < 8; ++u) v[u] = src[(long)stride * min(i0 + u * 1024, len - 1) + off0];
#pragma unroll
    for (int u = 0; u < 8; ++u) {
      const double w = (i0 + u * 1024 < len) ? v[u] : 0.0;
      acc = is_max ? fmax(acc, w) : acc + w;
    }
  }
  red[t] = acc;
  __syncthreads();
  for (int off = 512; off >= kWave; off >>= 1) {
    if (t < off) red[t] = is_max ? fmax(red[t], red[t + off]) : red[t] + red[t + off];
    __syncthreads();
  }
  if (t < kWave) {
    const double r = is_max ? wave_tree_max(red[t], kWave) : wave_tree_sum(red[t], kWave);
    if (t == 0) {
      out[p] = r;
      if (hout) hout[p] = r;
      if (save && p < 2) save[p] = r;
    }
  }
  if (flag && p == 0 && t == 0) {
    const int f = *flag;
    const double v[3] = {f > 0 ? 1.0 : 0.0,
                         f < 0 ? 1.0 : 0.0,
                         (double)f};
    for (int q = 0; q < 3; ++q) {
      out[NPART + 2 + q] = v[q];
      if (hout) hout[NPART + 2 + q] = v[q];
    }
  }
  if (hout && t == 0) {
    __threadfence_system();
    if (seq_done && seq > 0.0 &&
        __hip_atomic_fetch_add(seq_done, 1, __ATOMIC_ACQ_REL, __HIP_MEMORY_SCOPE_SYSTEM) == (int)gridDim.x - 1) {
      atomicExch(seq_done, 0);
      __hip_atomic_store(hout + kHostSeq, seq, __ATOMIC_RELEASE, __HIP_MEMORY_SCOPE_SYSTEM);
    }
  }
}

__global__ __launch_bounds__(1024) void k_reduce_parts(const double *__restrict__ parts, int nc,
                                                       const double *__restrict__ fparts,
                                                       int nfparts, double *__restrict__ out,
                                                       const int *__restrict__ flag,
                                                       double *__restrict__ hout, int *seq_done, double seq) {
  __shared__ double red[1024];
  reduce_parts_block(blockIdx.x, parts, nc, fparts, nfparts, out, flag, red, hout, seq_done, seq);
}

__global__ __launch_bounds__(1024) void k_lin_reduce(DevProblem P, const double *__restrict__ obs_tg,
                                                     double *__restrict__ g, double *__restrict__ colnorm,
                                                     const double *__restrict__ parts, double *__restrict__ out,
                                                     double *__restrict__ hout, double *__restrict__ save) {
  __shared__ double red[1024];
  if ((int)blockIdx.x < NPART + 2)
    reduce_parts_block(blockIdx.x, parts, P.nc, nullptr, 0, out, nullptr, red, hout, nullptr, 0.0, save);
  else
    tag_reduce_elem(P, obs_tg, (long)(blockIdx.x - (NPART + 2)) * 1024 + threadIdx.x, g, colnorm);
}


__global__ __launch_bounds__(256) void k_slot_norms(long n, long cap_lo, long cap_hi,
                                                    const unsigned char *__restrict__ free_,
                                                    const unsigned char *__restrict__ f_own,
                                                    double *__restrict__ g, double *__restrict__ colnorm,
                                                    const double *__restrict__ red,
                                                    const double *__restrict__ x,
                                                    double *__restrict__ out,
                                                    double *__restrict__ hout, const double *__restrict__ scale,
                                                    double dmin, double dmax, double *__restrict__ diag, double seq) {
  __shared__ double rs[6][256];
  __shared__ int last;
  const int t = threadIdx.x;
  const double g0 = free_[0] ? red[P_GF] : 0.0;
  if (blockIdx.x == 0 && t == 0) {
    g[0] = g0;
    colnorm[0] = free_[0] ? red[P_CF] : 0.0;
    g[1] = g[2] = 0.0;
    colnorm[1] = colnorm[2] = 0.0;
  }
  const double cn0 = free_[0] ? red[P_CF] : 0.0;
  double v[6] = {0, 0, 0, 0, 0, 0};
  for (long i = (long)blockIdx.x * 256 + t; i < n; i += (long)kNormBlocks * 256) {
    if (diag) {
      const double cn = i >= 3 ? colnorm[i] : (i == 0 ? cn0 : 0.0);
      diag[i] = fmin(fmax(scale[i] * scale[i] * cn, dmin), dmax);
    }
    if (!free_[i] || (f_own && !f_own[i])) continue;
    const int o = (i >= cap_lo && i < cap_hi) ? 0 : 3;
    const double gv = i >= 3 ? g[i] : (i == 0 ? g0 : 0.0), xv = x[i];
    v[o] = fmax(v[o], fabs(gv));
    v[o + 1] += gv * gv;
    v[o + 2] += xv * xv;
  }
  for (int q = 0; q < 6; ++q) rs[q][t] = v[q];
  __syncthreads();
  for (int off = 128; off >= kWave; off >>= 1) {
    if (t < off) {
      rs[0][t] = fmax(rs[0][t], rs[0][t + off]);
      rs[1][t] += rs[1][t + off];
      rs[2][t] += rs[2][t + off];
      rs[3][t] = fmax(rs[3][t], rs[3][t + off]);
      rs[4][t] += rs[4][t + off];
      rs[5][t] += rs[5][t + off];
    }
    __syncthreads();
  }
  if (t < kWave)
    for (int q = 0; q < 6; ++q) {
      const double r = (q % 3 == 0) ? wave_tree_max(rs[q][t], kWave) : wave_tree_sum(rs[q][t], kWave);
      if (t == 0) rs[q][0] = r;
    }
  double *part = out + 8;
  int *done = reinterpret_cast<int *>(out + 7);
  if (t == 0) {
    for (int q = 0; q < 6; ++q) part[6L * blockIdx.x + q] = rs[q][0];
    __threadfence();
    last = atomicAdd(done, 1) == kNormBlocks - 1;
  }
  __syncthreads();
  if (!last) return;
  __threadfence();
  if (t < kNormBlocks)
    for (int q = 0; q < 6; ++q) rs[q][t] = part[6L * t + q];
  __syncthreads();
  for (int off = kNormBlocks / 2; off >= kWave; off >>= 1) {
    if (t < off)
      for (int q = 0; q < 6; ++q)
        rs[q][t] = (q % 3 == 0) ? fmax(rs[q][t], rs[q][t + off]) : rs[q][t] + rs[q][t + off];
    __syncthreads();
  }
  if (t < kWave) {
    const int left = kNormBlocks < kWave ? kNormBlocks : kWave;
    double r6[6];
    for (int q = 0; q < 6; ++q) {
      const double v0 = t < left ? rs[q][t] : 0.0;
      r6[q] = (q % 3 == 0) ? wave_tree_max(v0, left) : wave_tree_sum(v0, left);
    }
    if (t == 0)
      for (int q = 0; q < 6; ++q) rs[q][0] = r6[q];
  }
  __syncthreads();
  if (t < 6) {
    out[t] = rs[t][0];
    if (hout) {
      hout[t] = rs[t][0];
      __threadfence_system();
    }
  }
  if (t == 0) atomicExch(done, 0);
  if (hout && seq > 0.0) {
    __syncthreads();
    if (t == 0) __hip_atomic_store(hout + kHostSeq, seq, __ATOMIC_RELEASE, __HIP_MEMORY_SCOPE_SYSTEM);
  }
}

__global__ void k_pack(PackSegs sg, double *__restrict__ buf, int unpack) {
  long e = (long)blockIdx.x * blockDim.x + threadIdx.x;
  for (int q = 0; q < sg.n; ++q) {
    if (e < sg.len[q]) {
      if (unpack) sg.p[q][e] = buf[sg.off[q] + e];
      else buf[sg.off[q] + e] = sg.p[q][e];
      return;
    }
    e -= sg.len[q];
  }
}

__global__ void k_top_tail(const int *__restrict__ idx, int m, double *__restrict__ g, double *__restrict__ cn,
                           double *__restrict__ red, double *__restrict__ tail, int unpack) {
  const int e = blockIdx.x * blockDim.x + threadIdx.x;
  if (e >= 2 * m + 2) return;
  double *v = e < m ? g + idx[e] : e < 2 * m ? cn + idx[e - m] : red + (e == 2 * m ? P_GF : P_CF);
  if (unpack) *v = tail[e];
  else tail[e] = *v;
}

__global__ void k_ag_put(const double *__restrict__ src, AgFields fl, double *__restrict__ ag, int nranks, int rank) {
  const int e = blockIdx.x * blockDim.x + threadIdx.x;
  if (e >= nranks * kAgFields) return;
  const int r = e / kAgFields, f = e % kAgFields;
  ag[e] = (r == rank && f < fl.n) ? src[fl.idx[f]] : 0.0;
}

__global__ void k_ag_reduce(const double *__restrict__ ag, AgFields fl, double *__restrict__ dst, int nranks,
                            HostOut ho) {
  const int f = threadIdx.x;
  if (f < fl.n) {
    const bool mx = (fl.max >> f) & 1u;
    double v = ag[f];
    for (int r = 1; r < nranks; ++r) {
      const double w = ag[r * kAgFields + f];
      v = mx ? fmax(v, w) : v + w;
    }
    dst[fl.idx[f]] = v;
  }
  if (!ho.seq_word) return;
  __syncthreads();
  for (int q = 0; q < ho.n; ++q)
    for (int e = f; e < ho.len[q]; e += blockDim.x) ho.dst[q][e] = ho.src[q][e];
  __threadfence_system();
  __syncthreads();
  if (f == 0) __hip_atomic_store(ho.seq_word, ho.seq, __ATOMIC_RELEASE, __HIP_MEMORY_SCOPE_SYSTEM);
}

__global__ void k_debug_rj(int n, const double *__restrict__ cam, const double *__restrict__ cap,
                           const double *__restrict__ tag, const double *__restrict__ corners,
                           double *__restrict__ r, double *__restrict__ J) {
  const long e = (long)blockIdx.x * blockDim.x + threadIdx.x;
  if (e >= 8L * n) return;
  const long o = e / 8;
  const int row = (int)(e % 8), corner = row >> 1, comp = row & 1;
  double j13[13];
  r[e] = residual_jacobian_row(cam + 3 * o, cap + 6 * o, tag + 6 * o, corner, comp,
                               corners[8 * o + row], j13);
  double *out = J + e * 15;
  out[0] = j13[0];
  out[1] = 0.0;
  out[2] = 0.0;
  for (int j = 0; j < 12; ++j) out[3 + j] = j13[1 + j];
}

__global__ void k_debug_rj_loss(int n, const double *__restrict__ cam, const double *__restrict__ cap,
                                const double *__restrict__ tag, const double *__restrict__ corners,
                                const unsigned char *__restrict__ kind, const double *__restrict__ a,
                                double *__restrict__ r, double *__restrict__ J, double *__restrict__ rho) {
  const long e = (long)blockIdx.x * blockDim.x + threadIdx.x;
  if (e >= 8L * n) return;
  const long o = e / 8;
  const int row = (int)(e % 8), corner = row >> 1, comp = row & 1;
  double j13[13];
  double rv = residual_jacobian_row(cam + 3 * o, cap + 6 * o, tag + 6 * o, corner, comp,
                                    corners[8 * o + row], j13);
  const double rh = robustify_row(kind[o], a[o], rv, j13);
  r[e] = rv;
  if (row == 0) rho[o] = rh;
  double *out = J + e * 15;
  out[0] = j13[0];
  out[1] = 0.0;
  out[2] = 0.0;
  for (int j = 0; j < 12; ++j) out[3 + j] = j13[1 + j];
}

__global__ void k_debug_aa(int n, const double *__restrict__ w, const double *__restrict__ p,
                           double *__restrict__ out, int *__restrict__ branch) {
  const int i = blockIdx.x * blockDim.x + threadIdx.x;
  if (i >= n) return;
  const AngleAxis a = aa_prepare(w + 3L * i);
  aa_rotate(a, p + 3L * i, out + 3L * i);
  branch[i] = a.big ? 1 : 0;
}

__global__ void k_debug_set_diag(DevProblem P, double *S, long row, double v) {
  if (threadIdx.x == 0) *reduced_elem(S, P, row, row) = v;
}

size_t lds_rows(int maxk) { return (size_t)8 * maxk * kRowStride * sizeof(double); }

}


void launch_linearize(const DevProblem &P, const double *x, double *g, double *colnorm,
                      double *obs_tg, double *parts, hipStream_t s) {
  if (P.nc == 0) return;
  const size_t lds = lds_rows(kObsChunk) + sizeof(double) * (kObsChunk + 16);
  const bool loss = P.obs_loss_kind != nullptr;
  hipLaunchKernelGGL((loss ? k_linearize<false, true> : k_linearize<false, false>), dim3(P.nc), dim3(kWave), lds, s, P,
                     x, g, colnorm, obs_tg, parts);
  if (P.n_chunk_caps)
    hipLaunchKernelGGL((loss ? k_linearize<true, true> : k_linearize<true, false>), dim3(P.n_chunk_caps), dim3(kWave),
                       lds, s, P, x, g, colnorm, obs_tg, parts);
}

void launch_lin_reduce(const DevProblem &P, const double *obs_tg, double *g, double *colnorm,
                       const double *parts, double *out, hipStream_t s, double *hout, double *save) {
  const unsigned tag_blocks = (unsigned)((12L * P.nt + 1023) / 1024);
  hipLaunchKernelGGL(k_lin_reduce, dim3(NPART + 2 + tag_blocks), dim3(1024), 0, s, P, obs_tg, g, colnorm, parts,
                     out, hout, save);
}

void launch_scale(const DevProblem &P, const double *colnorm, int jacobi, double *scale, hipStream_t s,
                  const LmDiagArgs *ld) {
  hipLaunchKernelGGL(k_scale, dim3((unsigned)((P.n + 255) / 256)), dim3(256), 0, s, P.n, P.slot_free,
                     colnorm, jacobi, scale, ld ? ld->dmin : 0.0, ld ? ld->dmax : 0.0, ld ? ld->diag : nullptr);
}

void launch_lm_diag(const DevProblem &P, const double *scale, const double *colnorm, double dmin,
                    double dmax, double *diag, hipStream_t s) {
  hipLaunchKernelGGL(k_lm_diag, dim3((unsigned)((P.n + 255) / 256)), dim3(256), 0, s, P.n, scale,
                     colnorm, dmin, dmax, diag);
}

void set_schur_big_lds_attribute() {
  static std::mutex m;
  static std::vector<char> done;
  int dev = 0;
  if (hipGetDevice(&dev) != hipSuccess) throw ApiError(ARSLAM_E_HIP, "hipGetDevice");
  std::lock_guard<std::mutex> g(m);
  if ((int)done.size() <= dev) done.resize(dev + 1, 0);
  if (done[dev]) return;
  const hipError_t e = hipFuncSetAttribute(reinterpret_cast<const void *>(&k_schur<true>),
                                           hipFuncAttributeMaxDynamicSharedMemorySize,
                                           (int)schur_lds_bytes(kMaxSchurBlocks));
  if (e != hipSuccess)
    throw ApiError(ARSLAM_E_HIP, std::string("hipFuncSetAttribute(k_schur, dynamic LDS): ") + hipGetErrorString(e));
  done[dev] = 1;
}

void launch_schur(const DevProblem &P, const double *x, const double *scale, const double *diag,
                  double radius, double *S, hipStream_t s, bool prep, long zero_tiles, const ExecReset *er) {
  const ExecReset r = er ? *er : ExecReset{};
  if (P.nc == 0) {
    if (zero_tiles) (void)hipMemsetAsync(S, 0, (size_t)zero_tiles * 4096 * sizeof(double), s);
    if (prep) launch_prep_reduced(P, diag, radius, S, s);
    return;
  }
  const size_t lds = schur_lds_bytes(std::min(P.max_blk_per_cap, kSchurMfmaBlocks));
  const long reset_blocks = (r.n() + kWave - 1) / kWave;
  hipLaunchKernelGGL(k_schur<false>, dim3((unsigned)(P.nc + zero_tiles + reset_blocks)), dim3(kWave), lds, s, P, scale,
                     diag, radius, S, zero_tiles, r, (const int *)nullptr);
  if (P.n_big_caps > 0) {
    const size_t lds_big = schur_lds_bytes(P.max_blk_per_cap);
    hipLaunchKernelGGL(k_schur<true>, dim3((unsigned)P.n_big_caps), dim3(kWave), lds_big, s, P, scale, diag, radius, S,
                       0L, ExecReset{}, P.big_caps);
  }
  const double *pd = prep ? diag : nullptr;
  const unsigned gb = (unsigned)((P.n_items + 3) / 4) + (prep ? (unsigned)((P.N + 255) / 256) : 0u);
  if (gb) hipLaunchKernelGGL(k_schur_gather, dim3(gb), dim3(256), 0, s, P, S, pd, radius);
  if (P.n_splits)
    hipLaunchKernelGGL(k_schur_combine, dim3((unsigned)((P.n_splits + 3) / 4)), dim3(256), 0, s, P, S, pd,
                       radius);
}

void launch_schur_gather(const DevProblem &P, const double *diag, double radius, double *S, hipStream_t s) {
  const unsigned gb = (unsigned)((P.n_items + 3) / 4) + (unsigned)((P.N + 255) / 256);
  hipLaunchKernelGGL(k_schur_gather, dim3(gb), dim3(256), 0, s, P, S, diag, radius);
  if (P.n_splits)
    hipLaunchKernelGGL(k_schur_combine, dim3((unsigned)((P.n_splits + 3) / 4)), dim3(256), 0, s, P, S, diag, radius);
}

void launch_prep_reduced(const DevProblem &P, const double *diag, double radius, double *S,
                         hipStream_t s, int which) {
  hipLaunchKernelGGL(k_prep_reduced, dim3((unsigned)((P.N + 255) / 256)), dim3(256), 0, s, P, diag,
                     radius, S, which);
}

void launch_mask_y(const DevProblem &P, double *yF, int rank, hipStream_t s, bool keep_top) {
  if (P.nR == 0) return;
  hipLaunchKernelGGL(k_mask_y, dim3((unsigned)((P.nR + 255) / 256)), dim3(256), 0, s, P, yF, rank, keep_top ? 1 : 0);
}

void launch_own_copy(const DevProblem &P, long first, long count, const double *src, double *dst, hipStream_t s) {
  if (count <= 0) return;
  hipLaunchKernelGGL(k_own_copy, dim3((unsigned)((count + 255) / 256)), dim3(256), 0, s, P, first, count, src, dst);
}

void launch_backsub(const DevProblem &P, const double *x, const double *scale, const double *diag,
                    double radius, const double *yF, double *xc, double *parts, hipStream_t s,
                    bool reuse_ui, bool with_cost) {
  if (P.nc == 0) return;
  const size_t lds = lds_rows(kObsChunk) + sizeof(double) * (8L * kObsChunk + 36 + 36 + 16);
  const bool loss = P.obs_loss_kind != nullptr;
  hipLaunchKernelGGL((loss ? k_backsub<false, true> : k_backsub<false, false>), dim3(P.nc), dim3(kWave), lds, s, P, x,
                     scale, diag, radius, yF, xc, parts, reuse_ui ? 1 : 0, with_cost ? 1 : 0);
  if (P.n_chunk_caps)
    hipLaunchKernelGGL((loss ? k_backsub<true, true> : k_backsub<true, false>), dim3(P.n_chunk_caps), dim3(kWave), lds, s,
                       P, x, scale, diag, radius, yF, xc, parts, reuse_ui ? 1 : 0, with_cost ? 1 : 0);
}

void launch_update_f(const DevProblem &P, const double *x, const double *scale, const double *yF,
                     double *xc, double *fparts, hipStream_t s) {
  const long n = std::max<long>(P.nR, P.nf);
  if (n == 0) return;
  hipLaunchKernelGGL(k_update_f, dim3((unsigned)((n + 255) / 256)), dim3(256), 0, s, P, x, scale, yF, xc, fparts);
}

void launch_cost(const DevProblem &P, const double *x, double *parts, hipStream_t s) {
  if (P.nc == 0) return;
  const bool loss = P.obs_loss_kind != nullptr;
  hipLaunchKernelGGL((loss ? k_cost<false, true> : k_cost<false, false>), dim3(P.nc), dim3(kWave), 0, s, P, x, parts);
  if (P.n_chunk_caps)
    hipLaunchKernelGGL((loss ? k_cost<true, true> : k_cost<true, false>), dim3(P.n_chunk_caps), dim3(kWave), 0, s, P, x,
                       parts);
}

__global__ __launch_bounds__(256) void k_copy_out(const double *__restrict__ src, long n, double *__restrict__ dst,
                                                  int *seq_done, double *word, double seq) {
  for (long i = (long)blockIdx.x * 256 + threadIdx.x; i < n; i += (long)gridDim.x * 256) dst[i] = src[i];
  __threadfence_system();
  __syncthreads();
  if (threadIdx.x == 0 &&
      __hip_atomic_fetch_add(seq_done, 1, __ATOMIC_ACQ_REL, __HIP_MEMORY_SCOPE_SYSTEM) == (int)gridDim.x - 1) {
    atomicExch(seq_done, 0);
    __hip_atomic_store(word, seq, __ATOMIC_RELEASE, __HIP_MEMORY_SCOPE_SYSTEM);
  }
}

void launch_copy_out(const double *src, long n, double *dst, int *seq_done, double *word, double seq, hipStream_t s) {
  const unsigned blocks = (unsigned)std::min<long>((n + 255) / 256, 1024);
  hipLaunchKernelGGL(k_copy_out, dim3(std::max(blocks, 1u)), dim3(256), 0, s, src, n, dst, seq_done, word, seq);
}

void launch_reduce_parts(const double *parts, int nc, const double *fparts, int nfparts, double *out,
                         hipStream_t s, const int *flag, double *hout, int *seq_done, double seq) {
  hipLaunchKernelGGL(k_reduce_parts, dim3(NPART + 2), dim3(1024), 0, s, parts, nc, fparts, nfparts, out, flag, hout,
                     seq_done, seq);
}

void launch_slot_norms(const DevProblem &P, const double *red, double *g, double *colnorm, const double *x,
                       double *out, hipStream_t s, double *hout, const LmDiagArgs *ld, double seq) {
  hipLaunchKernelGGL(k_slot_norms, dim3(kNormBlocks), dim3(256), 0, s, P.n, 3L, 3L + 6L * P.nc, P.slot_free, P.f_own, g,
                     colnorm, red, x, out, hout, ld ? ld->scale : nullptr, ld ? ld->dmin : 0.0,
                     ld ? ld->dmax : 0.0, ld ? ld->diag : nullptr, seq);
}

void launch_pack(const PackSegs &sg, double *buf, bool unpack, hipStream_t s) {
  long tot = 0;
  for (int q = 0; q < sg.n; ++q) tot += sg.len[q];
  if (tot == 0) return;
  hipLaunchKernelGGL(k_pack, dim3((unsigned)((tot + 255) / 256)), dim3(256), 0, s, sg, buf, unpack ? 1 : 0);
}

void launch_top_tail(const int *idx, int m, double *g, double *cn, double *red, double *tail, bool unpack,
                     hipStream_t s) {
  hipLaunchKernelGGL(k_top_tail, dim3((unsigned)((2 * m + 2 + 255) / 256)), dim3(256), 0, s, idx, m, g, cn, red, tail,
                     unpack ? 1 : 0);
}

void launch_ag_put(const double *src, const AgFields &fl, double *ag, int nranks, int rank, hipStream_t s) {
  hipLaunchKernelGGL(k_ag_put, dim3((unsigned)((nranks * kAgFields + 255) / 256)), dim3(256), 0, s, src, fl, ag,
                     nranks, rank);
}

void launch_ag_reduce(const double *ag, const AgFields &fl, double *dst, int nranks, hipStream_t s,
                      const HostOut *ho) {
  hipLaunchKernelGGL(k_ag_reduce, dim3(1), dim3(kAgFields), 0, s, ag, fl, dst, nranks, ho ? *ho : HostOut{});
}

void debug_residual_jacobian(int n, const double *cam, const double *cap, const double *tag,
                             const double *corners, double *r, double *J, hipStream_t s) {
  const long m = 8L * n;
  hipLaunchKernelGGL(k_debug_rj, dim3((unsigned)((m + 127) / 128)), dim3(128), 0, s, n, cam, cap, tag,
                     corners, r, J);
}

void debug_residual_jacobian_loss(int n, const double *cam, const double *cap, const double *tag,
                                  const double *corners, const unsigned char *kind, const double *a, double *r,
                                  double *J, double *rho, hipStream_t s) {
  const long m = 8L * n;
  hipLaunchKernelGGL(k_debug_rj_loss, dim3((unsigned)((m + 127) / 128)), dim3(128), 0, s, n, cam, cap, tag, corners,
                     kind, a, r, J, rho);
}

void debug_set_reduced_diag(const DevProblem &P, double *S, long row, double v, hipStream_t s) {
  hipLaunchKernelGGL(k_debug_set_diag, dim3(1), dim3(64), 0, s, P, S, row, v);
}

void debug_angle_axis(int n, const double *w, const double *p, double *out, int *branch, hipStream_t s) {
  hipLaunchKernelGGL(k_debug_aa, dim3((unsigned)((n + 127) / 128)), dim3(128), 0, s, n, w, p, out, branch);
}

}
```

### ar_slam_amd/csrc/lm_solve.hip

```cpp
#include "lm_handle.h"

std::string arslam::lmh::executor_fault_message(int code, int rank, int iteration, const arslam::LltPlan &plan,
                                                hipStream_t s) {
  std::string what;
  const int c = -code;
  if (code == 0) what = "on another rank";
  else if (c >= 4000000) what = "backward-solve column " + std::to_string(c - 4000000) + ": dependency wait timed out";
  else if (c >= 3000000) what = "ticket " + std::to_string(c - 3000000) + ": late wait (fused TRSM / folded TRSM's L_kk) timed out";
  else if (c >= 2000000) what = "ticket " + std::to_string(c - 2000000) + ": in-order update wait timed out";
  else if (c >= 1000000) what = "ticket " + std::to_string(c - 1000000) + ": dependency wait timed out";
  else what = "code " + std::to_string(code);
  const std::string m = "reduced-system executor fault (rank " + std::to_string(rank) + ", LM iteration " +
                        std::to_string(iteration) + "): " + what;
  if (code > -1000000 || code <= -4000000 || !plan.dag_counters) return m;
  int rec[arslam::kDagFaultSlots];
  if (hipMemcpyAsync(rec, plan.dag_counters + 2 * plan.n_tiles + arslam::kDagOffFault, sizeof(rec),
                     hipMemcpyDeviceToHost, s) != hipSuccess ||
      hipStreamSynchronize(s) != hipSuccess || rec[arslam::kFaultTicket] != (-code) % 1000000)
    return m;
  return m + " -- " + arslam::dag_fault_detail(plan, rec);
}

void arslam_lm::timing_begin() {
  if (!opt.kernel_timing || !has_f) return;
  const int need = plan.nlev + 1;
  if ((int)upd_events.size() < 2 * need) {
    for (auto e : upd_events) (void)hipEventDestroy(e);
    upd_events.assign(2 * need, nullptr);
    for (auto &e : upd_events) HIP_CHECK(hipEventCreateWithFlags(&e, hipEventDisableSystemFence));
  }
  upd_timing.ev = upd_events.data();
  upd_timing.cap = need;
  upd_timing.used = 0;
  upd_timing.flops = 0.0;
}

void arslam_lm::timing_collect() {
  if (!opt.kernel_timing || !has_f) return;
  for (int i = 0; i < upd_timing.used; ++i) {
    float ms = 0.f;
    HIP_CHECK(hipEventSynchronize(upd_events[2 * i + 1]));
    HIP_CHECK(hipEventElapsedTime(&ms, upd_events[2 * i], upd_events[2 * i + 1]));
    dom_ms += ms;
  }
  dom_launches += upd_timing.used;
  dom_flops += upd_timing.flops;
  upd_timing.used = 0;
  upd_timing.flops = 0.0;
}

void arslam_lm::allreduce_any(void *buf, size_t count, int dtype, int op) {
  if (!multi() || count == 0) return;
  const size_t bytes = count * (dtype == ARSLAM_DT_F64 ? sizeof(double) : 1);
  comm_bytes += (double)bytes;
  ++comm_calls;
  if (comm_cb) {
    comm_stage.resize(bytes);
    HIP_CHECK(hipMemcpyAsync(comm_stage.data(), buf, bytes, hipMemcpyDeviceToHost, stream));
    HIP_CHECK(hipStreamSynchronize(stream));
    fail_if(comm_cb(comm_cb_ctx, comm_stage.data(), count, dtype, op) != 0, ARSLAM_E_COMM,
            "all-reduce callback failed");
    HIP_CHECK(hipMemcpyAsync(buf, comm_stage.data(), bytes, hipMemcpyHostToDevice, stream));
    HIP_CHECK(hipStreamSynchronize(stream));
    return;
  }
  fail_if(!comm, ARSLAM_E_STATE, "the multi-rank path without a communicator");
  NCCL_CHECK(ncclAllReduce(buf, buf, count, dtype == ARSLAM_DT_F64 ? ncclDouble : ncclUint8,
                           op == ARSLAM_OP_SUM ? ncclSum : ncclMax, comm, stream));
}

void arslam_lm::linearize_launch() {
  h_lin.alloc(32);
  const bool direct = !multi();
  timers[PH_LIN].start(stream);
  arslam::launch_linearize(P, x, d_g.p, d_colnorm.p, d_obs_tg.p, d_parts.p, stream);
  arslam::launch_lin_reduce(P, d_obs_tg.p, d_g.p, d_colnorm.p, d_parts.p, d_red.p, stream,
                            direct ? h_lin.p : nullptr, multi() ? d_red.p + kLinSave : nullptr);
  if (multi()) lin_xpending = true;
  const arslam::LmDiagArgs ld{n, d_scale.p, d_colnorm.p, opt.min_lm_diagonal, opt.max_lm_diagonal, d_diag.p};
  lin_seq = direct ? next_seq(h_lin.p + 16 + arslam::kHostSeq) : 0.0;
  arslam::launch_slot_norms(P, d_red.p, d_g.p, d_colnorm.p, x, d_norms_p, stream, direct ? h_lin.p + 16 : nullptr,
                            diag_in_lin ? &ld : nullptr, lin_seq);
  timers[PH_LIN].stop(stream);
}

void arslam_lm::lin_norms() {
  const arslam::LmDiagArgs ld{n, d_scale.p, d_colnorm.p, opt.min_lm_diagonal, opt.max_lm_diagonal, d_diag.p};
  arslam::launch_slot_norms(P, d_red.p, d_g.p, d_colnorm.p, x, d_norms_p, stream, nullptr, diag_in_lin ? &ld : nullptr);
  lin_xpending = false;
  norms_pending = true;
}

void arslam_lm::complete_pending_lin() {
  if (!lin_xpending) return;
  const long t0 = 3 + 6L * nc;
  arslam::PackSegs sg;
  sg.add(d_g.p + t0, n - t0);
  sg.add(d_colnorm.p + t0, n - t0);
  sg.add(d_red.p + arslam::P_GF, 2);
  d_lx.alloc(sg.total());
  arslam::launch_pack(sg, d_lx.p, false, stream);
  allreduce(d_lx.p, sg.total(), ARSLAM_OP_SUM);
  arslam::launch_pack(sg, d_lx.p, true, stream);
  lin_norms();
}

void arslam_lm::exchange_scalars(arslam::AgFields fl, arslam::HostOut *ho) {
  const bool with_norms = norms_pending;
  if (with_norms) {
    const int nb0 = (int)(d_norms_p - d_red.p);
    for (int q = 0; q < 6; ++q) fl.add(nb0 + q, q % 3 == 0);
    fl.add(kLinSave, false);
    fl.add(kLinSave + 1, false);
  }
  if (fl.n == 0 && !ho) return;
  d_ag.alloc((size_t)nranks * arslam::kAgFields);
  arslam::launch_ag_put(d_red.p, fl, d_ag.p, nranks, rank, stream);
  allreduce(d_ag.p, (size_t)nranks * arslam::kAgFields, ARSLAM_OP_SUM);
  if (with_norms && ho) {
    h_lin.alloc(32);
    ho->add(d_norms_p, h_lin.p + 16, 6);
    ho->add(d_red.p + kLinSave, h_lin.p, 2);
  }
  arslam::launch_ag_reduce(d_ag.p, fl, d_red.p, nranks, stream, ho);
  if (with_norms) {
    if (!ho) {
      HIP_CHECK(hipMemcpyAsync(h_lin.p + 16, d_norms_p, 6 * sizeof(double), hipMemcpyDeviceToHost, stream));
      HIP_CHECK(hipMemcpyAsync(h_lin.p, d_red.p + kLinSave, 2 * sizeof(double), hipMemcpyDeviceToHost, stream));
    }
    norms_pending = false;
  }
}

void arslam_lm::linearize_collect(double *x_cost, double *fixed_cost, double *gmax, double *gnorm,
                                  double *xnorm) {
  const double *red = h_lin.p, *norms = h_lin.p + 16;
  *x_cost = red[arslam::P_COST];
  *fixed_cost = red[arslam::P_FIXED];
  *gmax = std::max(norms[0], norms[3]);
  *gnorm = std::sqrt(norms[1] + norms[4]);
  *xnorm = std::sqrt(norms[2] + norms[5]);
  timers[PH_LIN].collect();
}

void arslam_lm::linearize(double *x_cost, double *fixed_cost, double *gmax, double *gnorm,
                          double *xnorm) {
  linearize_launch();
  complete_pending_lin();
  exchange_norms();
  lin_sync();
  linearize_collect(x_cost, fixed_cost, gmax, gnorm, xnorm);
}

void arslam_lm::write_back(const double *d_src) {
  h_x.alloc(n + 1);
  const bool dma = env.write_back_dma;
  if (!multi() && !dma) {
    const double seq = next_seq(h_x.p + n);
    arslam::launch_copy_out(d_src, n, h_x.p, d_seq_done.p, h_x.p + n, seq, stream);
    flag_sync(h_x.p + n, seq);
  } else {
    HIP_CHECK(hipMemcpyAsync(h_x.p, d_src, n * sizeof(double), hipMemcpyDeviceToHost, stream));
  }
  if (multi()) {
    const long t0 = 3 + 6L * nc;
    d_lx.alloc(3 + n - t0);
    arslam::launch_own_copy(P, 0, 3, d_src, d_lx.p, stream);
    arslam::launch_own_copy(P, t0, n - t0, d_src + t0, d_lx.p + 3, stream);
    allreduce(d_lx.p, 3 + n - t0, ARSLAM_OP_SUM);
    HIP_CHECK(hipMemcpyAsync(h_x.p, d_lx.p, 3 * sizeof(double), hipMemcpyDeviceToHost, stream));
    HIP_CHECK(hipMemcpyAsync(h_x.p + t0, d_lx.p + 3, (n - t0) * sizeof(double), hipMemcpyDeviceToHost, stream));
  }
  if (multi() || dma) spin_sync();
  const double *h = h_x.p;
  std::memcpy(soa.camera, h, 3 * sizeof(double));
  if (elim_used == ARSLAM_ELIM_MIXED) {
    for (int g = 0; g < nc; ++g)
      if (mx.kind[g] != arslam::kMixDirect)
        std::memcpy((mx.kind[g] == arslam::kMixTag ? soa.tag : soa.cap) + 6L * mx.group_src[g], h + 3 + 6L * g,
                    6 * sizeof(double));
    for (int f = 0; f < nt; ++f)
      std::memcpy((mx.f_is_cap[f] ? soa.cap : soa.tag) + 6L * mx.f_src[f], h + 3 + 6L * nc + 6L * f,
                  6 * sizeof(double));
  } else if (multi()) {
    for (int c = 0; c < nc; ++c) std::memcpy(soa.cap + 6L * own_caps[c], h + 3 + 6L * c, 6 * sizeof(double));
  } else if (nc) {
    std::memcpy(soa.cap, h + 3, 6L * nc * sizeof(double));
  }
  if (nt && elim_used != ARSLAM_ELIM_MIXED) std::memcpy(soa.tag, h + 3 + 6L * nc, 6L * nt * sizeof(double));
  if (pk_stage) scatter_to_blocks();
}

void arslam_lm::scatter_to_blocks() {
  const arslam_soa_problem &p = *pk_stage;
  std::memcpy(camera_ptr, p.camera, 3 * sizeof(double));
  for (size_t c = 0; c < cap_ptrs.size(); ++c) std::memcpy(cap_ptrs[c], p.cap + 6 * c, 6 * sizeof(double));
  for (size_t t = 0; t < tag_ptrs.size(); ++t) std::memcpy(tag_ptrs[t], p.tag + 6 * t, 6 * sizeof(double));
}

void arslam_lm::restore_patched_wait() {
  if (dbg_patched_wait < 0) return;
  const int w = dbg_patched_wait;
  dbg_patched_wait = -1;
  plan.h_dag_waits[w].y -= 1 << 28;
  HIP_CHECK(hipMemcpyAsync(plan.dag_waits + w, &plan.h_dag_waits[w], sizeof(int2), hipMemcpyHostToDevice, stream));
  HIP_CHECK(hipStreamSynchronize(stream));
}

int arslam_lm::agree_callback(int r) {
  if (!multi()) return r;
  const double v = r == ARSLAM_SOLVER_ABORT ? 2.0 : r == ARSLAM_SOLVER_TERMINATE_SUCCESSFULLY ? 1.0 : 0.0;
  d_cb.alloc(1);
  HIP_CHECK(hipMemcpyAsync(d_cb.p, &v, sizeof(double), hipMemcpyHostToDevice, stream));
  allreduce(d_cb.p, 1, ARSLAM_OP_MAX);
  double m = 0.0;
  HIP_CHECK(hipMemcpyAsync(&m, d_cb.p, sizeof(double), hipMemcpyDeviceToHost, stream));
  HIP_CHECK(hipStreamSynchronize(stream));
  return m >= 2.0 ? ARSLAM_SOLVER_ABORT : m >= 1.0 ? ARSLAM_SOLVER_TERMINATE_SUCCESSFULLY : ARSLAM_SOLVER_CONTINUE;
}

namespace {

void print_header() {
  std::printf("iter      cost      cost_change  |gradient|   |step|    tr_ratio  tr_radius  ls_iter  iter_time  total_time\n");
}

void print_row(const arslam_lm_iteration &it) {
  std::printf("% 4d % 8e   % 3.2e   % 3.2e  % 3.2e  % 3.2e % 3.2e     % 4d   % 3.2e   % 3.2e\n",
              it.iteration, it.cost, it.cost_change, it.gradient_max_norm, it.step_norm,
              it.relative_decrease, it.trust_region_radius, 0, it.iteration_time, it.cumulative_time);
  std::fflush(stdout);
}

}

void arslam_lm::begin_solve(arslam_lm_summary *s) {
  std::memset(s, 0, sizeof(*s));
  for (auto &t : timers) {
    t.acc_ms = 0.0;
    t.on = opt.phase_timing != 0;
  }
  dom_ms = dom_flops = 0.0;
  dom_launches = 0;
  norms_pending = lin_xpending = false;
  s->n_obs = nb;
  s->n_reduced = has_f ? (int)nR : 0;
  s->setup_time_s = setup_s;
  for (int i = 0; i < 5; ++i) s->setup_phase_s[i] = setup_phase[i];
  s->setup_kind = setup_kind;
  x = d_xa.p;
  xc = d_xb.p;
  xbest = x;
  HIP_CHECK(hipMemcpyAsync(x, u_x0, n * sizeof(double), hipMemcpyDeviceToDevice, stream));
  if (opt.minimizer_progress_to_stdout && rank == 0) print_header();
  any_iter_cb = agree_callback(iter_cb ? ARSLAM_SOLVER_TERMINATE_SUCCESSFULLY : ARSLAM_SOLVER_CONTINUE) !=
                ARSLAM_SOLVER_CONTINUE;
  comm_bytes = 0.0;
  comm_calls = 0;
}

bool arslam_lm::prepare_step(bool reuse_diag, arslam::ExecReset *er) {
  const bool exec_dag = has_f && opt.factor_executor == 1;
  if (exec_dag && nc > 0) {
    *er = arslam::exec_reset_args(plan, d_flag.p, d_yF.p, nR);
    return true;
  }
  if (exec_dag) {
    const arslam::LmDiagArgs ld{0, d_scale.p, d_colnorm.p, opt.min_lm_diagonal, opt.max_lm_diagonal, d_diag.p, d_yF.p, nR};
    arslam::launch_exec_reset(plan, d_flag.p, stream, &ld);
  } else {
    if (!reuse_diag)
      arslam::launch_lm_diag(P, d_scale.p, d_colnorm.p, opt.min_lm_diagonal, opt.max_lm_diagonal, d_diag.p, stream);
    HIP_CHECK(hipMemsetAsync(d_flag.p, 0, sizeof(int), stream));
  }
  return false;
}

namespace {
bool g_dag_traced = false;
int g_dag_trace_seen = 0;
}

void arslam_lm::dump_dag_trace(long first_store) {
  DevBuf<unsigned long long> tr;
  tr.alloc(arslam::kDagTraceWords * plan.n_dag_tasks);
  HIP_CHECK(hipMemsetAsync(tr.p, 0, tr.n * 8, stream));
  arslam::launch_dense_llt_dag(plan, Sp, d_flag.p, stream, dag_workgroups, nullptr, tr.p, false, -1, first_store);
  std::vector<unsigned long long> h(arslam::kDagTraceWords * plan.n_dag_tasks);
  HIP_CHECK(hipMemcpyAsync(h.data(), tr.p, h.size() * 8, hipMemcpyDeviceToHost, stream));
  HIP_CHECK(hipStreamSynchronize(stream));
  if (FILE *f = std::fopen(env.dag_trace, "wb")) {
    const long n = plan.n_dag_tasks;
    std::fwrite(&n, 8, 1, f);
    std::fwrite(plan.h_dag_tasks.data(), sizeof(int4), n, f);
    std::fwrite(h.data(), 8, h.size(), f);
    const long nw = (long)plan.h_dag_waits.size();
    std::fwrite(&nw, 8, 1, f);
    std::fwrite(plan.h_dag_wait_off.data(), sizeof(int), n + 1, f);
    std::fwrite(plan.h_dag_waits.data(), sizeof(int2), nw, f);
    std::fwrite(plan.h_dag_sub.data(), sizeof(int2), n, f);
    std::fclose(f);
  }
  g_dag_traced = true;
}

void arslam_lm::factor_reduced(long first_store, bool record, double radius, bool force_indefinite) {
  if (opt.factor_executor != 1) {
    arslam::launch_dense_llt(plan, Sp, d_flag.p, stream, record ? &upd_timing : nullptr);
    return;
  }
  const bool rec = record && upd_timing.used < upd_timing.cap;
  if (rec) HIP_CHECK(hipEventRecord(upd_timing.ev[2 * upd_timing.used], stream));
  if (env.dag_trace && !g_dag_traced && g_dag_trace_seen++ >= env.dag_trace_skip) {
    dump_dag_trace(first_store);
  } else if (multi()) {
    timers[PH_FAC0].start(stream);
    arslam::launch_dense_llt_dag(plan, Sp, d_flag.p, stream, dag_workgroups, nullptr, nullptr, false, 0);
    timers[PH_FAC0].stop(stream);
    const long tail = lin_xpending ? top_tail_len() : 0;
    if (tail) arslam::launch_top_tail(u_top_slots, n_top_slots, d_g.p, d_colnorm.p, d_red.p, Sp - tail, false, stream);
    allreduce(Sp - tail, (size_t)tail + (size_t)plan.n_top_tiles * 4096, ARSLAM_OP_SUM);
    if (tail) {
      arslam::launch_top_tail(u_top_slots, n_top_slots, d_g.p, d_colnorm.p, d_red.p, Sp - tail, true, stream);
      lin_norms();
    }
    arslam::launch_prep_reduced(P, d_diag.p, radius, Sp, stream, 1);
    if (force_indefinite)
      arslam::debug_set_reduced_diag(P, Sp, P.cam_row >= 0 ? P.cam_row : nR - 1, -1.0, stream);
    timers[PH_FAC1].start(stream);
    arslam::launch_dense_llt_dag(plan, Sp, d_flag.p, stream, dag_workgroups, nullptr, nullptr, false, 1);
    timers[PH_FAC1].stop(stream);
  } else {
    arslam::launch_dense_llt_dag(plan, Sp, d_flag.p, stream, dag_workgroups, nullptr, nullptr, false, -1, first_store);
  }
  if (rec) {
    HIP_CHECK(hipEventRecord(upd_timing.ev[2 * upd_timing.used + 1], stream));
    upd_timing.used++;
    upd_timing.flops += plan.total_factor_flops;
  }
}

void arslam_lm::back_substitute(double radius) {
  if (has_f) {
    timers[PH_SOLVE].start(stream);
    if (opt.factor_executor == 1)
      arslam::launch_dense_back_solve_dag(plan, Sp, nR, d_yF.p, d_flag.p, stream, dag_workgroups, false);
    else
      arslam::launch_dense_back_solve(plan, Sp, nR, d_z.p, d_yF.p, d_flag.p, stream);
    if (multi()) {
      arslam::launch_mask_y(P, d_yF.p, rank, stream, true);
    }
    timers[PH_SOLVE].stop(stream);
  }
  timers[PH_BACK].start(stream);
  arslam::launch_update_f(P, x, d_scale.p, d_yF.p, xc, d_fparts.p, stream);
  arslam::launch_backsub(P, x, d_scale.p, d_diag.p, radius, d_yF.p, xc, d_parts.p, stream, has_f, true);
  timers[PH_BACK].stop(stream);
}

double arslam_lm::reduce_step_scalars() {
  timers[PH_COST].start(stream);
  h_step.alloc(16);
  double step_seq = !multi() ? next_seq(h_step.p + arslam::kHostSeq) : 0.0;
  arslam::launch_reduce_parts(d_parts.p, nc, d_fparts.p, n_fparts, d_red.p, stream, d_flag.p,
                              !multi() ? h_step.p : nullptr, d_seq_done.p, step_seq);
  if (multi()) {
    arslam::AgFields fl;
    for (int f : {(int)arslam::P_COST, (int)arslam::P_FIXED, (int)arslam::P_MODEL, (int)arslam::P_STEP2,
                  (int)arslam::NPART})
      fl.add(f, false);
    for (int f : {(int)arslam::P_YBAD, (int)arslam::P_CBAD, arslam::NPART + 1, arslam::NPART + 2, arslam::NPART + 3})
      fl.add(f, true);
    arslam::HostOut ho;
    ho.add(d_red.p, h_step.p, arslam::NPART + 5);
    step_seq = next_seq(h_step.p + arslam::kHostSeq);
    ho.seq_word = h_step.p + arslam::kHostSeq;
    ho.seq = step_seq;
    exchange_scalars(fl, &ho);
  }
  timers[PH_COST].stop(stream);
  return step_seq;
}

double arslam_lm::enqueue_step(double radius, bool reuse_diag, int solve_index) {
  arslam::ExecReset er{};
  const bool reset_in_schur = prepare_step(reuse_diag, &er);
  if (lin_xpending && !(has_f && opt.factor_executor == 1 && !env.dag_trace)) complete_pending_lin();
  if (has_f) {
    timers[PH_SCHUR].start(stream);
    const bool fill_first_store = !multi() && opt.factor_executor == 1;
    arslam::launch_schur(P, x, d_scale.p, d_diag.p, radius, Sp, stream, !multi(),
                         fill_first_store ? n_clear : plan.n_tiles, reset_in_schur ? &er : nullptr);
    const bool force_indefinite = dbg_indefinite_mask >> std::min(solve_index, 63) & 1ull;
    if (multi()) arslam::launch_prep_reduced(P, d_diag.p, radius, Sp, stream, 0);
    else if (force_indefinite)
      arslam::debug_set_reduced_diag(P, Sp, P.cam_row >= 0 ? P.cam_row : nR - 1, -1.0, stream);
    timers[PH_SCHUR].stop(stream);
    timers[PH_CHOL].start(stream);
    timing_begin();
    factor_reduced(fill_first_store ? n_clear : LONG_MAX, opt.kernel_timing != 0, radius, force_indefinite);
    timers[PH_CHOL].stop(stream);
  }
  back_substitute(radius);
  return reduce_step_scalars();
}

void arslam_lm::fill_summary(arslam_lm_summary *s) {
  const long nb_all = nb_global;
  s->n_obs = (int)nb_all;
  s->final_rms_px = nb_all ? std::sqrt(2.0 * s->final_cost / (4.0 * nb_all)) : 0.0;
  s->t_linearize_ms = timers[PH_LIN].acc_ms;
  s->t_schur_ms = timers[PH_SCHUR].acc_ms;
  s->t_cholesky_ms = timers[PH_CHOL].acc_ms;
  s->t_solve_ms = timers[PH_SOLVE].acc_ms;
  s->t_backsub_ms = timers[PH_BACK].acc_ms;
  s->t_cost_ms = timers[PH_COST].acc_ms;
  s->t_factor_own_ms = timers[PH_FAC0].acc_ms;
  s->t_factor_top_ms = timers[PH_FAC1].acc_ms;
  s->t_dominant_ms = dom_ms;
  s->dominant_flops = dom_flops;
  s->n_dominant_launches = dom_launches;
  s->n_factor_tiles = plan.n_tiles;
  s->n_levels = plan.nlev;
  s->n_update_tiles = plan.total_upd_tiles;
  s->factor_update_flops = plan.total_upd_flops;
  s->factor_scalar_flops = scalar_flops;
  s->comm_bytes = comm_bytes;
  s->comm_calls = comm_calls;
  s->elimination_used = elim_used;
  s->ceres_e_captures = ceres_e_cap;
  s->ceres_e_tags = ceres_e_tag;
  s->n_ranks = nranks;
  s->n_owned_captures = multi() ? nc : nc_user;
  s->n_top_tiles = multi() ? plan.n_top_tiles : 0;
  s->split_top_work = split_top_work;
  s->split_max_rank_work = split_max_rank_work;
  s->split_total_work = split_total_work;
  s->n_active_ranks = multi() ? split_active : 1;
  s->order_reused = last_order_reused ? 1 : 0;
}

namespace {

struct TrustRegion {
  double radius;
  double decrease_factor = 2.0;
  bool reuse_diag = false;
  int n_invalid = 0;
  void shrink(int invalid) {
    n_invalid = invalid;
    radius = radius / decrease_factor;
    decrease_factor *= 2.0;
    reuse_diag = true;
  }
  void invalid() { shrink(n_invalid + 1); }
  void rejected() { shrink(0); }
  void accepted(double rho, double max_radius) {
    n_invalid = 0;
    const double q = 2.0 * rho - 1.0;
    radius = radius / std::max(1.0 / 3.0, 1.0 - q * q * q);
    radius = std::min(max_radius, radius);
    decrease_factor = 2.0;
    reuse_diag = false;
  }
};

struct RestoreWait {
  arslam_lm *h;
  ~RestoreWait() {
    try { h->restore_patched_wait(); } catch (...) {}
  }
};
struct DiagInLin {
  arslam_lm *h;
  ~DiagInLin() { h->diag_in_lin = false; }
};

}

void arslam_lm::solve(arslam_lm_summary *s) {
  fail_if(!loaded, ARSLAM_E_STATE, "no problem loaded");
  cov_invalidate();
  const arslam_lm_options &o = opt;
  const double t_start = now_s();
  RestoreWait restore_wait{this};
  begin_solve(s);
  const bool root = rank == 0;
  const auto stop = [s](int termination, int rule) {
    s->termination = termination;
    s->rule = rule;
    return true;
  };

  double x_cost, fixed_cost, gmax, gnorm, x_norm;
  linearize(&x_cost, &fixed_cost, &gmax, &gnorm, &x_norm);
  s->fixed_cost = fixed_cost;
  s->initial_cost = x_cost + fixed_cost;
  s->final_cost = s->initial_cost;
  if (!std::isfinite(x_cost)) {
    stop(ARSLAM_FAILURE, ARSLAM_RULE_EVAL_FAILED);
    s->total_time_s = now_s() - t_start;
    solve_state = 2;
    return;
  }
  const arslam::LmDiagArgs ld{n, d_scale.p, d_colnorm.p, o.min_lm_diagonal, o.max_lm_diagonal, d_diag.p};
  arslam::launch_scale(P, d_colnorm.p, o.jacobi_scaling, d_scale.p, stream, &ld);
  diag_in_lin = true;
  DiagInLin diag_in_lin_guard{this};

  TrustRegion tr{o.initial_trust_region_radius};
  double minimum_cost = x_cost;
  arslam_lm_iteration it{};
  it.iteration = 0;
  it.cost = x_cost + fixed_cost;
  it.gradient_max_norm = gmax;
  it.gradient_norm = gnorm;
  it.step_is_valid = 1;
  it.step_is_successful = 1;
  double t_iter = t_start;

  bool lin_pending = false;
  double prev_gmax = 0.0, prev_gnorm = 0.0;
  auto finalize = [&]() -> bool {
    if (lin_pending) {
      double fc;
      linearize_collect(&x_cost, &fc, &gmax, &gnorm, &x_norm);
      it.cost = x_cost + fixed_cost;
      it.gradient_max_norm = gmax;
      it.gradient_norm = gnorm;
      lin_pending = false;
    }
    if (it.step_is_successful) {
      if (it.iteration > 0) s->num_successful_steps++;
      if (x_cost < minimum_cost || it.iteration == 0) {
        minimum_cost = x_cost;
        xbest = x;
        if (o.update_state_every_iteration) write_back(xbest);
      }
    } else {
      s->num_unsuccessful_steps++;
    }
    it.trust_region_radius = tr.radius;
    const double tn = now_s();
    it.iteration_time = tn - t_iter;
    it.cumulative_time = tn - t_start;
    t_iter = tn;
    if (s->n_iters <= ARSLAM_LM_MAX_ITERS) s->iters[s->n_iters++] = it;
    if (o.minimizer_progress_to_stdout && root) print_row(it);
    if (iter_cb || any_iter_cb) {
      const int r = agree_callback(iter_cb ? iter_cb(iter_cb_ctx, &it) : ARSLAM_SOLVER_CONTINUE);
      if (r == ARSLAM_SOLVER_ABORT) return stop(ARSLAM_USER_FAILURE, ARSLAM_RULE_USER_CALLBACK);
      if (r == ARSLAM_SOLVER_TERMINATE_SUCCESSFULLY) return stop(ARSLAM_USER_SUCCESS, ARSLAM_RULE_USER_CALLBACK);
    }
    if (it.iteration >= o.max_num_iterations) return stop(ARSLAM_NO_CONVERGENCE, ARSLAM_RULE_MAX_ITERS);
    if (it.step_is_successful && it.gradient_max_norm <= o.gradient_tolerance)
      return stop(ARSLAM_CONVERGENCE, ARSLAM_RULE_GRADIENT);
    if (tr.radius <= o.min_trust_region_radius) return stop(ARSLAM_CONVERGENCE, ARSLAM_RULE_MIN_RADIUS);
    prev_gmax = it.gradient_max_norm;
    prev_gnorm = it.gradient_norm;
    const int next_iter = it.iteration + 1;
    it = arslam_lm_iteration{};
    it.iteration = next_iter;
    return false;
  };

  for (;;) {
    const bool stop_rule = it.iteration >= o.max_num_iterations || tr.radius <= o.min_trust_region_radius;
    if (lin_pending && stop_rule) {
      complete_pending_lin();
      exchange_norms();
      lin_sync();
    }
    const bool deferred = lin_pending && !stop_rule;
    if (!deferred && finalize()) break;

    const double step_seq = enqueue_step(tr.radius, tr.reuse_diag, s->num_linear_solves++);
    flag_sync(h_step.p + arslam::kHostSeq, step_seq);
    const double *red = h_step.p;
    if (red[arslam::NPART + 3] != 0.0)
      throw Error(ARSLAM_E_DEVICE, executor_fault_message((int)red[arslam::NPART + 4], rank, it.iteration, plan, stream));
    for (int ph = PH_SCHUR; ph < PH_N; ++ph) timers[ph].collect();
    timing_collect();
    if (deferred && finalize()) {
      s->num_linear_solves--;
      break;
    }

    const bool lin_fail = red[arslam::NPART + 2] != 0.0;
    const bool ybad = red[arslam::P_YBAD] != 0.0 || red[arslam::NPART + 1] != 0.0;
    const double model_cost_change = red[arslam::P_MODEL];
    const bool valid = !lin_fail && !ybad && model_cost_change > 0.0;
    if (!valid) {
      tr.invalid();
      if (tr.n_invalid >= o.max_num_consecutive_invalid_steps) { stop(ARSLAM_FAILURE, ARSLAM_RULE_INVALID_STEPS); break; }
      it.cost = x_cost + fixed_cost;
      it.gradient_max_norm = prev_gmax;
      it.gradient_norm = prev_gnorm;
      it.step_is_valid = 0;
      it.step_is_successful = 0;
      continue;
    }
    it.step_is_valid = 1;
    double candidate_cost = red[arslam::P_COST];
    if (!std::isfinite(candidate_cost) || red[arslam::P_CBAD] != 0.0) candidate_cost = DBL_MAX;
    it.step_norm = std::sqrt(red[arslam::P_STEP2] + red[arslam::NPART]);
    if (it.step_norm <= o.parameter_tolerance * (x_norm + o.parameter_tolerance)) {
      stop(ARSLAM_CONVERGENCE, ARSLAM_RULE_PARAMETER); break;
    }
    it.cost_change = x_cost - candidate_cost;
    if (std::fabs(it.cost_change) <= o.function_tolerance * x_cost) {
      stop(ARSLAM_CONVERGENCE, ARSLAM_RULE_FUNCTION); break;
    }
    it.relative_decrease = candidate_cost >= DBL_MAX ? -DBL_MAX
                                                     : (x_cost - candidate_cost) / model_cost_change;
    if (it.relative_decrease > o.min_relative_decrease) {
      double *old = x;
      x = xc;
      xc = old != xbest ? old : (d_xa.p != x && d_xa.p != xbest) ? d_xa.p : (d_xb.p != x && d_xb.p != xbest) ? d_xb.p : d_xbest.p;
      linearize_launch();
      lin_pending = true;
      it.step_is_successful = 1;
      tr.accepted(it.relative_decrease, o.max_trust_region_radius);
    } else {
      it.step_is_successful = 0;
      tr.rejected();
      it.cost = candidate_cost + fixed_cost;
      it.gradient_max_norm = prev_gmax;
      it.gradient_norm = prev_gnorm;
    }
  }
  s->final_cost = minimum_cost + fixed_cost;
  s->minimizer_time_s = now_s() - t_start;
  write_back(xbest);
  s->total_time_s = now_s() - t_start;
  if (env.setup_profile) std::fprintf(stderr, "arslam write_back %.3f ms\n", 1e3 * (s->total_time_s - s->minimizer_time_s));
  fill_summary(s);
  solve_state = 1;
}
```

### ar_slam_amd/lm.py

```python
from __future__ import annotations

import ctypes as C
import os

import numpy as np

HERE = os.path.dirname(os.path.abspath(__file__))
LIB_PATH = os.environ.get("ARSLAM_LIB") or os.path.join(HERE, "libarslam_lm.so")
MAX_ITERS = 1024
COMM_ID_BYTES = 128

TERMINATION = {0: "CONVERGENCE", 1: "NO_CONVERGENCE", 2: "FAILURE", 3: "USER_SUCCESS", 4: "USER_FAILURE"}
RULES = {0: "none", 1: "gradient_tolerance", 2: "parameter_tolerance", 3: "function_tolerance",
         4: "min_trust_region_radius", 5: "max_num_iterations", 6: "invalid_steps",
         7: "evaluation_failed", 8: "user_callback"}
ERRORS = {-1: "INVALID_ARG", -2: "UNSUPPORTED", -3: "NO_DEVICE", -4: "HIP", -5: "OUT_OF_MEMORY",
          -6: "COMM", -7: "STATE", -8: "DEVICE"}

EXPORTS = ["arslam_lm_options_init", "arslam_lm_create", "arslam_lm_destroy",
           "arslam_lm_set_options", "arslam_lm_get_options",
           "arslam_lm_add_residual_block", "arslam_lm_set_parameter_block_constant",
           "arslam_lm_set_parameter_block_variable", "arslam_lm_solve", "arslam_lm_reset",
           "arslam_lm_num_residual_blocks", "arslam_lm_load_soa", "arslam_lm_solve_loaded",
           "arslam_lm_solve_soa", "arslam_comm_unique_id", "arslam_lm_set_comm", "arslam_lm_set_comm_callback",
           "arslam_device_count", "arslam_lm_last_error", "arslam_lm_version",
           "arslam_lm_set_iteration_callback", "arslam_lm_owned_captures",
           "arslam_lm_set_loss", "arslam_lm_get_loss", "arslam_lm_add_residual_block_loss",
           "arslam_lm_load_soa_loss", "arslam_debug_residual_jacobian_loss", "arslam_slam_set_loss",
           "arslam_debug_residual_jacobian", "arslam_debug_dense_llt", "arslam_debug_dense_llt_ex",
           "arslam_debug_tile_llt", "arslam_debug_tile_plan",
           "arslam_debug_angle_axis_rotate", "arslam_debug_selinv", "arslam_lm_debug_force_indefinite",
           "arslam_lm_covariance", "arslam_lm_covariance_block", "arslam_lm_debug_reduced_rows",
           "arslam_lm_covariance_pairs", "arslam_lm_covariance_block_pair", "arslam_debug_tile_solve",
           "arslam_lm_debug_force_multirank", "arslam_lm_debug_break_dependency", "arslam_lm_debug_tag_pair_tile",
           "arslam_debug_reduced_plan", "arslam_debug_reduced_plan_side", "arslam_debug_schur_stamps", "arslam_debug_ceres_e_blocks",
           "arslam_debug_mixed_groups",
           "arslam_debug_dag_simulate", "arslam_debug_dag_simulate_started", "arslam_debug_dag_workgroup_limit",
           "arslam_debug_dag_fault_detail", "arslam_debug_box_fingerprint",
           "arslam_debug_rank_split", "arslam_debug_gather_extend", "arslam_debug_schur_store_table",
           "arslam_localize_many", "arslam_localizer_create", "arslam_localizer_destroy",
           "arslam_localizer_load", "arslam_localizer_solve",
           "arslam_localizer_set_loss", "arslam_localizer_get_loss", "arslam_localizer_load_loss",
           "arslam_localizer_observation_terms", "arslam_localize_many_loss", "arslam_slam_set_localize_loss",
           "arslam_localizer_covariance", "arslam_localizer_covariance_timed", "arslam_localize_many_cov",
           "arslam_slam_localize_covariance",
           "arslam_slam_create", "arslam_slam_destroy", "arslam_slam_set_verbose", "arslam_slam_load_yaml",
           "arslam_slam_load_yaml_string", "arslam_slam_save_yaml", "arslam_slam_add_detections",
           "arslam_slam_solve", "arslam_slam_solve_incremental", "arslam_slam_localize_many",
           "arslam_slam_num_captures", "arslam_slam_num_arucos", "arslam_slam_num_blocks",
           "arslam_slam_num_solves", "arslam_slam_last_summary", "arslam_slam_solve_summary",
           "arslam_slam_solve_capture", "arslam_slam_unsolved_captures", "arslam_slam_capture", "arslam_slam_set_capture_pose", "arslam_slam_aruco", "arslam_slam_set_aruco_pose",
           "arslam_slam_block", "arslam_slam_camera", "arslam_slam_set_camera",
           "arslam_slam_get_transforms", "arslam_slam_camera_info"]

_dp = C.POINTER(C.c_double)
ALLREDUCE_FN = C.CFUNCTYPE(C.c_int, C.c_void_p, C.c_void_p, C.c_size_t, C.c_int, C.c_int)
SOLVER_CONTINUE, SOLVER_ABORT, SOLVER_TERMINATE_SUCCESSFULLY = 0, 1, 2
ELIM_AUTO, ELIM_CAPTURES, ELIM_TAGS, ELIM_MIXED = 0, 1, 2, 3
SETUP_LOAD, SETUP_VALUES, SETUP_APPEND = 0, 1, 2
LOSS_NONE, LOSS_HUBER, LOSS_SOFT_L_ONE, LOSS_CAUCHY = 0, 1, 2, 3
_ip = C.POINTER(C.c_int)
_up = C.POINTER(C.c_ubyte)


class LMError(RuntimeError):
    def __init__(self, code, msg):
        super().__init__(f"arslam_lm error {code} ({ERRORS.get(code, '?')}): {msg}")
        self.code = code


class Options(C.Structure):
    _fields_ = [("max_num_iterations", C.c_int),
                ("function_tolerance", C.c_double), ("gradient_tolerance", C.c_double),
                ("parameter_tolerance", C.c_double),
                ("initial_trust_region_radius", C.c_double),
                ("max_trust_region_radius", C.c_double),
                ("min_trust_region_radius", C.c_double),
                ("min_relative_decrease", C.c_double),
                ("min_lm_diagonal", C.c_double), ("max_lm_diagonal", C.c_double),
                ("max_num_consecutive_invalid_steps", C.c_int),
                ("jacobi_scaling", C.c_int), ("elimination", C.c_int),
                ("minimizer_progress_to_stdout", C.c_int),
                ("update_state_every_iteration", C.c_int),
                ("device", C.c_int), ("cholesky_skip_zero_tiles", C.c_int),
                ("reduced_ordering", C.c_int), ("kernel_timing", C.c_int), ("factor_executor", C.c_int),
                ("phase_timing", C.c_int)]


class Iteration(C.Structure):
    _fields_ = [("iteration", C.c_int),
                ("cost", C.c_double), ("cost_change", C.c_double),
                ("gradient_max_norm", C.c_double), ("gradient_norm", C.c_double),
                ("step_norm", C.c_double), ("relative_decrease", C.c_double),
                ("trust_region_radius", C.c_double),
                ("step_is_valid", C.c_int), ("step_is_successful", C.c_int),
                ("iteration_time", C.c_double), ("cumulative_time", C.c_double)]


ITER_CB = C.CFUNCTYPE(C.c_int, C.c_void_p, C.POINTER(Iteration))


class Summary(C.Structure):
    _fields_ = [("termination", C.c_int), ("rule", C.c_int),
                ("num_successful_steps", C.c_int), ("num_unsuccessful_steps", C.c_int),
                ("num_linear_solves", C.c_int),
                ("initial_cost", C.c_double), ("final_cost", C.c_double),
                ("fixed_cost", C.c_double), ("final_rms_px", C.c_double),
                ("n_obs", C.c_int), ("n_reduced", C.c_int),
                ("setup_time_s", C.c_double), ("setup_kind", C.c_int), ("minimizer_time_s", C.c_double),
                ("total_time_s", C.c_double),
                ("t_linearize_ms", C.c_double), ("t_schur_ms", C.c_double),
                ("t_cholesky_ms", C.c_double), ("t_solve_ms", C.c_double),
                ("t_backsub_ms", C.c_double), ("t_cost_ms", C.c_double),
                ("t_dominant_ms", C.c_double), ("dominant_flops", C.c_double),
                ("n_dominant_launches", C.c_long),
                ("n_factor_tiles", C.c_long), ("n_levels", C.c_int), ("n_update_tiles", C.c_long),
                ("factor_update_flops", C.c_double), ("factor_scalar_flops", C.c_double),
                ("comm_bytes", C.c_double),
                ("elimination_used", C.c_int), ("ceres_e_captures", C.c_int), ("ceres_e_tags", C.c_int),
                ("n_ranks", C.c_int), ("n_owned_captures", C.c_int), ("n_top_tiles", C.c_long),
                ("split_top_work", C.c_double), ("split_max_rank_work", C.c_double),
                ("split_total_work", C.c_double), ("t_factor_own_ms", C.c_double),
                ("t_factor_top_ms", C.c_double),
                ("n_iters", C.c_int), ("iters", Iteration * (MAX_ITERS + 1)),
                ("setup_phase_s", C.c_double * 5), ("comm_calls", C.c_long), ("n_active_ranks", C.c_int),
                ("order_reused", C.c_int)]

    def to_dict(self):
        its = [{f: getattr(self.iters[i], f) for f, _ in Iteration._fields_}
               for i in range(self.n_iters)]
        d = {f: getattr(self, f) for f, _ in Summary._fields_ if f not in ("iters", "termination", "rule")}
        d["setup_phase_s"] = list(self.setup_phase_s)
        d["termination"] = TERMINATION[self.termination]
        d["rule"] = RULES[self.rule]
        d["iterations"] = its
        return d


COV_OK, COV_UNAVAILABLE, COV_RANK_DEFICIENT = 0, 1, 2
BLOCK_CAMERA, BLOCK_CAPTURE, BLOCK_TAG = 0, 1, 2


class CovInfo(C.Structure):
    _fields_ = [("status", C.c_int), ("min_pivot", C.c_double), ("n_reduced", C.c_long),
                ("n_factor_tiles", C.c_long), ("n_factor_products", C.c_long), ("n_selinv_products", C.c_long),
                ("t_linearize_ms", C.c_double), ("t_factor_ms", C.c_double), ("t_selinv_ms", C.c_double),
                ("t_blocks_ms", C.c_double)]

    def to_dict(self):
        return {f: getattr(self, f) for f, _ in self._fields_}


class SoaProblem(C.Structure):
    _fields_ = [("n_cap", C.c_int), ("n_tag", C.c_int), ("n_obs", C.c_int),
                ("camera", _dp), ("cap", _dp), ("tag", _dp),
                ("obs_cap", _ip), ("obs_tag", _ip), ("corners", _dp),
                ("camera_const", C.c_int), ("cap_const", _up), ("tag_const", _up)]


_lib = None


def library_path():
    return LIB_PATH


def library_info():
    import hashlib
    with open(LIB_PATH, "rb") as f:
        sha = hashlib.sha256(f.read()).hexdigest()[:12]
    v = lib().arslam_lm_version().decode()
    return {"file": os.path.basename(LIB_PATH), "sha256": sha, "version": v.split(" build ")[0],
            "build": v.split(" build ")[-1] if " build " in v else "unknown"}


def lib():
    global _lib
    if _lib is not None:
        return _lib
    if not os.path.exists(LIB_PATH):
        raise ImportError(f"{LIB_PATH} is missing: build it with `python -m ar_slam_amd.build` "
                          "(hipcc --offload-arch=gfx950); there is no CPU fallback")
    L = C.CDLL(LIB_PATH)
    L.arslam_lm_options_init.argtypes = [C.POINTER(Options)]
    L.arslam_lm_create.argtypes = [C.POINTER(C.c_void_p), C.POINTER(Options)]
    L.arslam_lm_set_comm_callback.argtypes = [C.c_void_p, C.c_int, C.c_int, ALLREDUCE_FN, C.c_void_p]
    L.arslam_lm_set_options.argtypes = [C.c_void_p, C.POINTER(Options)]
    L.arslam_debug_rank_split.argtypes = [C.POINTER(SoaProblem), C.c_int, C.c_int, C.POINTER(SplitInfo), _ip]
    L.arslam_lm_owned_captures.argtypes = [C.c_void_p, C.POINTER(C.c_int), C.c_int, C.POINTER(C.c_int)]
# ... 59 lines not shown
    L.arslam_debug_selinv.argtypes = [C.c_long, _dp, _up, _dp, _up, _ip]
    if hasattr(L, "arslam_debug_tile_llt"):
        L.arslam_debug_tile_llt.argtypes = [C.c_long, _dp, _dp, _up, C.c_int, _up, C.c_uint, _dp, _dp, _up, _ip,
                                            C.c_void_p]
        L.arslam_debug_tile_plan.argtypes = [C.c_int, _up, _up, _up, C.c_void_p]
    L.arslam_lm_covariance.argtypes = [C.c_void_p, _dp, _dp, _dp, _ip, _ip, C.POINTER(CovInfo)]
    L.arslam_lm_covariance_block.argtypes = [C.c_void_p, _dp, _dp, _ip]
    L.arslam_lm_covariance_pairs.argtypes = [C.c_void_p, _ip, C.c_int, _dp, _ip, C.POINTER(CovInfo)]
    L.arslam_lm_covariance_block_pair.argtypes = [C.c_void_p, _dp, _dp, _dp, _ip]
    L.arslam_debug_tile_solve.argtypes = [C.c_long, _dp, _up, C.c_int, _dp, _dp, _ip]
    L.arslam_lm_debug_reduced_rows.argtypes = [C.c_void_p, _ip, _ip, _ip]
    L.arslam_debug_ceres_e_blocks.argtypes = [C.POINTER(SoaProblem), _ip]
    L.arslam_debug_mixed_groups.argtypes = [C.POINTER(SoaProblem), _ip, C.POINTER(C.c_ubyte), C.POINTER(C.c_ubyte)]
    L.arslam_lm_debug_force_indefinite.argtypes = [C.c_void_p, C.c_ulonglong]
    L.arslam_lm_debug_force_multirank.argtypes = [C.c_void_p, C.c_int]
    L.arslam_debug_dag_workgroup_limit.argtypes = [C.c_int]
    L.arslam_lm_set_iteration_callback.argtypes = [C.c_void_p, ITER_CB, C.c_void_p]
    L.arslam_lm_debug_break_dependency.argtypes = [C.c_void_p, C.c_long, C.POINTER(C.c_long)]
    if hasattr(L, "arslam_lm_debug_tag_pair_tile"):
        L.arslam_lm_debug_tag_pair_tile.argtypes = [C.c_void_p, _dp, _dp, C.POINTER(C.c_int)]
    if hasattr(L, "arslam_debug_schur_store_table"):
        L.arslam_debug_schur_store_table.argtypes = [C.c_int, _ip, C.POINTER(C.c_ubyte)]
    _lib = L
    return L


def _check(rc):
    if rc != 0:
        raise LMError(rc, lib().arslam_lm_last_error().decode(errors="replace"))


def device_count():
    return lib().arslam_device_count()


def make_options(**kw):
    o = Options()
    lib().arslam_lm_options_init(C.byref(o))
    for k, v in kw.items():
        if not hasattr(o, k):
            raise AttributeError(f"unknown solver option {k}")
        setattr(o, k, v)
    return o


def _f64(a, shape=None):
    a = np.ascontiguousarray(a, dtype=np.float64)
    return a if shape is None else a.reshape(shape)


class _Soa:
    def __init__(self, camera, cap, tag, obs_cap, obs_tag, corners, camera_const=False,
                 cap_const=None, tag_const=None):
        self.camera = _f64(camera).copy()
        self.cap = _f64(cap, (-1, 6)).copy()
        self.tag = _f64(tag, (-1, 6)).copy()
        self.obs_cap = np.ascontiguousarray(obs_cap, np.int32)
        self.obs_tag = np.ascontiguousarray(obs_tag, np.int32)
        self.corners = _f64(corners, (-1, 8))
        self.cap_const = None if cap_const is None else np.ascontiguousarray(cap_const, np.uint8)
        self.tag_const = None if tag_const is None else np.ascontiguousarray(tag_const, np.uint8)
        self.s = SoaProblem(self.cap.shape[0], self.tag.shape[0], self.obs_cap.shape[0],
                            self.camera.ctypes.data_as(_dp), self.cap.ctypes.data_as(_dp),
                            self.tag.ctypes.data_as(_dp), self.obs_cap.ctypes.data_as(_ip),
                            self.obs_tag.ctypes.data_as(_ip), self.corners.ctypes.data_as(_dp),
                            int(bool(camera_const)),
                            None if self.cap_const is None else self.cap_const.ctypes.data_as(_up),
                            None if self.tag_const is None else self.tag_const.ctypes.data_as(_up))


def solve_soa(camera, cap, tag, obs_cap, obs_tag, corners, camera_const=False, cap_const=None,
              tag_const=None, loss=None, obs_loss=None, **opts):
    if loss is not None or obs_loss is not None:
        R = ResidentProblem(camera, cap, tag, obs_cap, obs_tag, corners, camera_const, cap_const, tag_const,
                            loss=loss, obs_loss=obs_loss, **opts)
        try:
            s = R.solve()
            return R.camera, R.cap, R.tag, s
        finally:
            R.close()
    A = _Soa(camera, cap, tag, obs_cap, obs_tag, corners, camera_const, cap_const, tag_const)
    s = Summary()
    _check(lib().arslam_lm_solve_soa(C.byref(A.s), C.byref(make_options(**opts)), C.byref(s)))
    return A.camera, A.cap, A.tag, s.to_dict()


def warm_up(device=0):
    import time
    from . import synth
    t = time.perf_counter()
    g = synth.config_graph("tiny")
    ResidentProblem(g.camera, g.cap, g.tag, g.obs_cap, g.obs_tag, g.corners, device=device).solve()
    return time.perf_counter() - t


def solve_graph(g, loss=None, obs_loss=None, **opts):
    return solve_soa(g.camera, g.cap, g.tag, g.obs_cap, g.obs_tag, g.corners, loss=loss, obs_loss=obs_loss, **opts)


class _Handle:
    def __init__(self, **opts):
        self._h = C.c_void_p()
        _check(lib().arslam_lm_create(C.byref(self._h), C.byref(make_options(**opts))))

    def close(self):
        if self._h:
            lib().arslam_lm_destroy(self._h)
            self._h = C.c_void_p()

    def __del__(self):
        try:
            self.close()
        except Exception:
            pass

    def set_options(self, **opts):
        _check(lib().arslam_lm_set_options(self._h, C.byref(make_options(**opts))))

    def get_options(self) -> Options:
        o = Options()
        _check(lib().arslam_lm_get_options(self._h, C.byref(o)))
        return o

    def set_loss(self, kind, a=0.0):
        _check(lib().arslam_lm_set_loss(self._h, int(kind), float(a)))

    def get_loss(self):
        k, a = C.c_int(0), C.c_double(0.0)
        _check(lib().arslam_lm_get_loss(self._h, C.byref(k), C.byref(a)))
        return k.value, a.value

    def set_iteration_callback(self, fn):
        if fn is None:
            self._iter_cb = None
            _check(lib().arslam_lm_set_iteration_callback(self._h, C.cast(None, ITER_CB), None))
            return

        def tramp(ctx, it):
            try:
                d = {f: getattr(it.contents, f) for f, _ in Iteration._fields_}
                r = fn(d)
                return SOLVER_CONTINUE if r is None else int(r)
            except Exception:
                return SOLVER_ABORT
        self._iter_cb = ITER_CB(tramp)
        _check(lib().arslam_lm_set_iteration_callback(self._h, self._iter_cb, None))

    def debug_force_indefinite(self, step_mask):
        _check(lib().arslam_lm_debug_force_indefinite(self._h, C.c_ulonglong(step_mask & (2**64 - 1))))

    def debug_force_multirank(self, on=True):
        _check(lib().arslam_lm_debug_force_multirank(self._h, 1 if on else 0))

    def set_comm(self, rank, nranks, uid):
        if callable(uid):
            fn = uid

            def tramp(ctx, buf, count, dtype, op):
                try:
                    ct = C.c_double if dtype == 0 else C.c_ubyte
                    arr = np.ctypeslib.as_array(C.cast(buf, C.POINTER(ct)), shape=(count,))
                    fn(arr, "sum" if op == 0 else "max")
                    return 0
                except Exception:
                    return 1
            self._comm_cb = ALLREDUCE_FN(tramp)
            _check(lib().arslam_lm_set_comm_callback(self._h, rank, nranks, self._comm_cb, None))
        else:
            _check(lib().arslam_lm_set_comm(self._h, rank, nranks, uid))


def comm_unique_id() -> bytes:
    buf = C.create_string_buffer(COMM_ID_BYTES)
    _check(lib().arslam_comm_unique_id(buf))
    return buf.raw


class ResidentProblem(_Handle):

    def __init__(self, camera, cap, tag, obs_cap, obs_tag, corners, camera_const=False,
                 cap_const=None, tag_const=None, comm=None, force_multirank=False, loss=None, obs_loss=None,
                 **opts):
        super().__init__(**opts)
        if force_multirank:
            self.debug_force_multirank(True)
        if comm is not None:
            self.set_comm(*comm)
        if loss is not None:
            self.set_loss(*loss)
        self.A = _Soa(camera, cap, tag, obs_cap, obs_tag, corners, camera_const, cap_const, tag_const)
        if obs_loss is None:
            _check(lib().arslam_lm_load_soa(self._h, C.byref(self.A.s)))
        else:
            kinds = np.ascontiguousarray(obs_loss[0], np.uint8).reshape(-1)
            scales = _f64(obs_loss[1]).reshape(-1)
            if kinds.shape[0] != self.A.s.n_obs or scales.shape[0] != self.A.s.n_obs:
                raise ValueError("obs_loss: one kind and one scale per observation")
            _check(lib().arslam_lm_load_soa_loss(self._h, C.byref(self.A.s), kinds.ctypes.data_as(_up),
                                                 scales.ctypes.data_as(_dp)))

    def solve(self):
        s = Summary()
        _check(lib().arslam_lm_solve_loaded(self._h, C.byref(s)))
        return s.to_dict()

    def covariance(self):
        n_cap, n_tag = self.A.s.n_cap, self.A.s.n_tag
        cap = np.zeros((n_cap, 6, 6))
        tag = np.zeros((n_tag, 6, 6))
        var_f = C.c_double(0.0)
        cs = np.zeros(max(n_cap, 1), np.int32)
        ts = np.zeros(max(n_tag, 1), np.int32)
        info = CovInfo()
        _check(lib().arslam_lm_covariance(self._h, cap.ctypes.data_as(_dp), tag.ctypes.data_as(_dp), C.byref(var_f),
                                          cs.ctypes.data_as(_ip), ts.ctypes.data_as(_ip), C.byref(info)))
        return {"cap": cap, "tag": tag, "var_f": var_f.value, "cap_status": cs[:n_cap], "tag_status": ts[:n_tag],
                "info": info.to_dict()}

    def covariance_pairs(self, pairs):
        flat = np.ascontiguousarray([[a[0], a[1], b[0], b[1]] for a, b in pairs], np.int32).reshape(-1, 4)
        n = len(flat)
        cov = np.zeros((n, 6, 6))
        st = np.zeros(max(n, 1), np.int32)
        info = CovInfo()
        _check(lib().arslam_lm_covariance_pairs(self._h, flat.ctypes.data_as(_ip) if n else None, C.c_int(n),
                                                cov.ctypes.data_as(_dp) if n else None, st.ctypes.data_as(_ip),
                                                C.byref(info)))
        return cov, st[:n], info.to_dict()

    def debug_reduced_rows(self):
        cr = np.zeros(max(self.A.s.n_cap, 1), np.int32)
        tr = np.zeros(max(self.A.s.n_tag, 1), np.int32)
        cam = C.c_int(-1)
        _check(lib().arslam_lm_debug_reduced_rows(self._h, cr.ctypes.data_as(_ip), tr.ctypes.data_as(_ip),
                                                  C.byref(cam)))
        return cr[:self.A.s.n_cap], tr[:self.A.s.n_tag], cam.value

    def owned_captures(self):
        n = C.c_int(0)
        _check(lib().arslam_lm_owned_captures(self._h, None, C.c_int(0), C.byref(n)))
        out = (C.c_int * max(n.value, 1))()
        _check(lib().arslam_lm_owned_captures(self._h, out, C.c_int(n.value), C.byref(n)))
        return np.array(out[:n.value], np.int64)

    def debug_break_dependency(self, ticket):
        out = C.c_long(-1)
        _check(lib().arslam_lm_debug_break_dependency(self._h, ticket, C.byref(out)))
        return out.value

    @property
    def camera(self):
        return self.A.camera

    @property
    def cap(self):
        return self.A.cap

    @property
    def tag(self):
        return self.A.tag


class Problem(_Handle):

    def __init__(self, **opts):
        super().__init__(**opts)
        self._keep = []

    @staticmethod
    def _block(a, n):
        if not (isinstance(a, np.ndarray) and a.dtype == np.float64 and a.flags.c_contiguous
                and a.size == n):
            raise TypeError(f"parameter block must be a C-contiguous float64 array of size {n}")
        return a.ctypes.data_as(_dp)

    def add_residual_block(self, corners, camera, capture, tag, loss=None):
        c = _f64(corners).reshape(8)
        self._keep += [camera, capture, tag]
        if loss is not None:
            _check(lib().arslam_lm_add_residual_block_loss(self._h, c.ctypes.data_as(_dp),
                                                           self._block(camera, 3), self._block(capture, 6),
                                                           self._block(tag, 6), int(loss[0]), float(loss[1])))
            return
        _check(lib().arslam_lm_add_residual_block(self._h, c.ctypes.data_as(_dp),
                                                  self._block(camera, 3), self._block(capture, 6),
                                                  self._block(tag, 6)))

    def set_parameter_block_constant(self, block):
        _check(lib().arslam_lm_set_parameter_block_constant(self._h, block.ctypes.data_as(_dp)))

    def set_parameter_block_variable(self, block):
        _check(lib().arslam_lm_set_parameter_block_variable(self._h, block.ctypes.data_as(_dp)))

    def num_residual_blocks(self):
        return lib().arslam_lm_num_residual_blocks(self._h)

    def solve(self):
        s = Summary()
        _check(lib().arslam_lm_solve(self._h, C.byref(s)))
        return s.to_dict()

    def covariance_block(self, block):
        if not (isinstance(block, np.ndarray) and block.dtype == np.float64 and block.size in (3, 6)):
            raise TypeError("parameter block must be a float64 array of size 3 or 6")
        k = block.size
        out = np.zeros((k, k))
# ... 566 lines not shown
```

### include/arslam_lm_debug.h

```cpp
#ifndef ARSLAM_LM_DEBUG_H
#define ARSLAM_LM_DEBUG_H

#include "arslam_lm.h"

#ifdef __cplusplus
extern "C" {
#endif

int arslam_debug_residual_jacobian(int n, const double *cam, const double *cap, const double *tag,
                                   const double *corners, double *r, double *J);

int arslam_debug_residual_jacobian_loss(int n, const double *cam, const double *cap, const double *tag,
                                        const double *corners, const unsigned char *kind, const double *a,
                                        double *r, double *J, double *rho);

int arslam_debug_angle_axis_rotate(int n, const double *w, const double *p, double *out, int *branch);

int arslam_debug_dense_llt(long n, double *A, const double *b, double *y, int *info);
int arslam_debug_dense_llt_ex(long n, double *A, const double *b, double *y, int *info, int executor);

typedef struct {
  int tiles_per_side;
  long n_assembled;
  long n_tiles;
  int n_levels;
  long n_split;
  long n_dag_tasks;
  int fill_first_ok;
  long phase_split;
  int grid[2];
  long n_cont_tasks;
  int dag_valid;
} arslam_tile_plan_facts;

int arslam_debug_tile_llt(long n, const double *A, const double *b, const unsigned char *tile_pattern,
                          int executor, const unsigned char *col_class, unsigned flags, double *L_out,
                          double *y, unsigned char *pattern_out, int *info, arslam_tile_plan_facts *facts);
int arslam_debug_tile_plan(int T, const unsigned char *tile_pattern, const unsigned char *col_class,
                           unsigned char *pattern_out, arslam_tile_plan_facts *facts);

int arslam_debug_selinv(long n, const double *A, const unsigned char *tile_pattern, double *Z_out,
                        unsigned char *pattern_out, int *info);

int arslam_debug_tile_solve(long n, const double *A, const unsigned char *tile_pattern, int nrhs, const double *B,
                            double *X_out, int *info);

int arslam_lm_debug_reduced_rows(arslam_lm *h, int *cap_row, int *tag_row, int *cam_row);

typedef struct {
  long n_reduced;
  long n_padded;
  long pad_rows;
  int tiles_per_side;
  int n_parts;
  int camera_row;
  int n_levels;
  long n_assembled_tiles;
  long n_factor_tiles;
  long n_update_tiles;
  long n_update_items;
  long n_split_targets;
  double update_flops;
  long n_dag_tasks;
  int dag_valid;
  double factor_flops;
  double scalar_flops;
  int fill_first_ok;
} arslam_plan_info;

int arslam_debug_schur_stamps(unsigned long long out[16]);

int arslam_lm_debug_force_indefinite(arslam_lm *h, unsigned long long step_mask);
int arslam_lm_debug_break_dependency(arslam_lm *h, long ticket, long *broken);
int arslam_lm_debug_force_multirank(arslam_lm *h, int on);
int arslam_lm_debug_tag_pair_tile(arslam_lm *h, const double *tag_a, const double *tag_b, int *status);

int arslam_debug_ceres_e_blocks(const arslam_soa_problem *p, int out[4]);

int arslam_debug_mixed_groups(const arslam_soa_problem *p, int out[4], unsigned char *e_cap, unsigned char *e_tag);

int arslam_debug_reduced_plan(const arslam_soa_problem *p, int ordering, int skip_zero_tiles,
                              arslam_plan_info *info, int *tag_row);
int arslam_debug_reduced_plan_side(const arslam_soa_problem *p, int elimination, arslam_plan_info *info);

int arslam_debug_dag_simulate(const arslam_soa_problem *p, int n_workers, unsigned seed, int policy, int *ok);
int arslam_debug_dag_simulate_started(const arslam_soa_problem *p, int n_workers, int n_started, unsigned seed,
                                      int policy, int *ok);
int arslam_debug_dag_workgroup_limit(int k);

int arslam_debug_dag_fault_detail(const arslam_soa_problem *p, const int rec[9], char *buf, int len);

int arslam_debug_box_fingerprint(int device, double out[6]);

typedef struct {
  int tiles_per_side;
  int n_top_cols;
  int n_own_cols;
  long n_top_tiles;
  long n_tiles;
  long n_dag_tasks, phase_split;
  int dag_valid;
  int n_owned_captures;
  double top_work, max_rank_work, total_work;
  int n_active;
} arslam_split_info;
int arslam_debug_rank_split(const arslam_soa_problem *p, int nranks, int rank, arslam_split_info *info,
                            int *cap_owner);
int arslam_debug_gather_extend(const arslam_soa_problem *p, int c0, int *identical, int *n_dest);
int arslam_debug_schur_store_table(int nblk, int *off, unsigned char *stored);

#ifdef __cplusplus
}
#endif
#endif
```

Measured before the change: 1149.

## Fold linearization reductions into the Schur kernel launches as rider blocks

After an accepted step, the launch of the linearization reduction kernels (lin_reduce and slot_norms) is deferred. Their work runs as extra rider blocks inside the next k_schur and k_schur_gather grids. The Schur kernels compute the LM diagonal inline from scale and colnorm instead of reading a precomputed diag buffer, and the parts reduction is redone as a wave-level tree. This removes separate kernel launches and their serialization on the stream. It relies on block-level ordering assumptions between rider and consumer blocks inside one grid, and it adds branches and register pressure to the hot Schur kernels.

New measurement: 1157 (median of 2 runs). No clear change (+0.7%).

```diff
diff --git a/ar_slam_amd/csrc/lin_tree64.h b/ar_slam_amd/csrc/lin_tree64.h
--- /dev/null
+++ b/ar_slam_amd/csrc/lin_tree64.h
@@ -0,0 +1,45 @@
+#pragma once
+
+#if defined(__HIPCC__)
+#define ARSLAM_TREE_HD __host__ __device__ __forceinline__
+#else
+#define ARSLAM_TREE_HD inline
+#endif
+
+namespace arslam {
+
+constexpr int kTreeThreads = 1024;
+constexpr int kTreeFlight = 8;
+constexpr int kTreeLane = 64;
+constexpr int kTreePerLane = kTreeThreads / kTreeLane;
+
+template <class T, class Load, class Op>
+ARSLAM_TREE_HD T tree1024_on_wave(int lane, int len, Load load, Op op, T zero) {
+  T v[kTreePerLane];
+#pragma unroll
+  for (int j = 0; j < kTreePerLane; ++j) v[j] = zero;
+  for (int r0 = 0; r0 < len; r0 += kTreeFlight * kTreeThreads) {
+#pragma unroll 1
+    for (int u = 0; u < kTreeFlight; ++u) {
+      T w[kTreePerLane];
+#pragma unroll
+      for (int j = 0; j < kTreePerLane; ++j) {
+        const int i = lane + kTreeLane * j + r0 + u * kTreeThreads;
+        w[j] = load(i < len ? i : len - 1);
+      }
+#pragma unroll
+      for (int j = 0; j < kTreePerLane; ++j) {
+        const int t0 = lane + kTreeLane * j + r0, i = t0 + u * kTreeThreads;
+        const T x = i < len ? w[j] : zero;
+        if (t0 < len) v[j] = op(v[j], x);
+      }
+    }
+  }
+#pragma unroll
+  for (int h = kTreePerLane / 2; h >= 1; h >>= 1)
+#pragma unroll
+    for (int j = 0; j < h; ++j) v[j] = op(v[j], v[j + h]);
+  return v[0];
+}
+
+}
diff --git a/ar_slam_amd/csrc/lm_capi.hip b/ar_slam_amd/csrc/lm_capi.hip
--- a/ar_slam_amd/csrc/lm_capi.hip
+++ b/ar_slam_amd/csrc/lm_capi.hip
@@ -486,6 +486,19 @@
   return ARSLAM_OK;
 }
 
+int arslam_lm_debug_separate_lin_reductions(arslam_lm *h, int on) {
+  if (!h || (on != 0 && on != 1)) return ARSLAM_E_INVALID_ARG;
+  h->dbg_separate_lin = on != 0;
+  return ARSLAM_OK;
+}
+
+int arslam_lm_debug_lin_reduction_launches(arslam_lm *h, int *separate, int *ridealong) {
+  if (!h) return ARSLAM_E_INVALID_ARG;
+  if (separate) *separate = h->n_lin_separate;
+  if (ridealong) *ridealong = h->n_lin_ride;
+  return ARSLAM_OK;
+}
+
 int arslam_lm_debug_force_multirank(arslam_lm *h, int on) {
   if (!h || (on != 0 && on != 1)) return ARSLAM_E_INVALID_ARG;
   return guarded([&] {
diff --git a/ar_slam_amd/csrc/lm_handle.h b/ar_slam_amd/csrc/lm_handle.h
--- a/ar_slam_amd/csrc/lm_handle.h
+++ b/ar_slam_amd/csrc/lm_handle.h
@@ -57,6 +57,7 @@
   int dag_trace_skip = std::getenv("ARSLAM_DAG_TRACE_SKIP") ? std::atoi(std::getenv("ARSLAM_DAG_TRACE_SKIP")) : 0;
   bool setup_profile = std::getenv("ARSLAM_SETUP_PROFILE") != nullptr;
   bool write_back_dma = std::getenv("ARSLAM_WRITE_BACK_DMA") != nullptr;
+  const char *lin_ride_place = std::getenv("ARSLAM_LIN_RIDE_PLACE");
 };
 inline const DebugEnv &debug_env() {
   static const DebugEnv e;
@@ -352,7 +353,12 @@
   int prev_order_height = 0;
   static int etree_height(const arslam::ReducedLayout &L);
   void linearize(double *x_cost, double *fixed_cost, double *gmax, double *gnorm, double *xnorm);
-  void linearize_launch();
+  void linearize_launch(bool defer = false);
+  void lin_reductions_launch();
+  bool lin_ride_ok() const;
+  bool lin_red_deferred = false;
+  bool dbg_separate_lin = false;
+  int n_lin_separate = 0, n_lin_ride = 0;
   void linearize_collect(double *x_cost, double *fixed_cost, double *gmax, double *gnorm, double *xnorm);
   bool lin_xpending = false, norms_pending = false;
   DevBuf<double> d_lx, d_ag;
diff --git a/ar_slam_amd/csrc/lm_internal.h b/ar_slam_amd/csrc/lm_internal.h
--- a/ar_slam_amd/csrc/lm_internal.h
+++ b/ar_slam_amd/csrc/lm_internal.h
@@ -269,9 +269,19 @@
 void launch_lm_diag(const DevProblem &P, const double *scale, const double *colnorm, double dmin,
                     double dmax, double *diag, hipStream_t s);
 void set_schur_big_lds_attribute();
+struct LinRide {
+  int on = 0, front = 0;
+  int first = 0, count = 0, shift = 0;
+  const double *obs_tg = nullptr, *parts = nullptr, *x = nullptr, *scale = nullptr;
+  double *g = nullptr, *colnorm = nullptr;
+  double *red = nullptr, *hout = nullptr;
+  double *norms = nullptr, *norms_hout = nullptr;
+  double dmin = 0.0, dmax = 0.0, seq = 0.0;
+  double *diag = nullptr;
+};
 void launch_schur(const DevProblem &P, const double *x, const double *scale, const double *diag,
                   double radius, double *S, hipStream_t s, bool prep = false, long zero_tiles = 0,
-                  const ExecReset *er = nullptr);
+                  const ExecReset *er = nullptr, const LinRide *ride = nullptr);
 void launch_schur_gather(const DevProblem &P, const double *diag, double radius, double *S, hipStream_t s);
 void launch_prep_reduced(const DevProblem &P, const double *diag, double radius, double *S,
                          hipStream_t s, int which = -1);
diff --git a/ar_slam_amd/csrc/lm_kernels.hip b/ar_slam_amd/csrc/lm_kernels.hip
--- a/ar_slam_amd/csrc/lm_kernels.hip
+++ b/ar_slam_amd/csrc/lm_kernels.hip
@@ -2,6 +2,7 @@
 #include "projection.h"
 #include "loss.h"
 #include "schur_store_table.h"
+#include "lin_tree64.h"
 
 #include <cfloat>
 #include <mutex>
@@ -47,9 +48,24 @@
   return P.cap_kind && P.cap_kind[c] == kMixDirect;
 }
 
+__device__ __forceinline__ double lm_d2v(double dg, double radius) {
+  const double d = sqrt(dg / radius);
+  return d * d;
+}
 __device__ __forceinline__ double lm_d2(const double *diag, long slot, double radius) {
-  const double d = sqrt(diag[slot] / radius);
-  return d * d;
+  return lm_d2v(diag[slot], radius);
+}
+__device__ __forceinline__ double ride_diag_cn(const LinRide &r, long slot, double cn) {
+  const double sv = r.scale[slot];
+  return fmin(fmax(sv * sv * cn, r.dmin), r.dmax);
+}
+__device__ __forceinline__ double ride_diag(const DevProblem &P, const LinRide &r, long slot) {
+  return ride_diag_cn(r, slot, slot >= 3 ? r.colnorm[slot] : (slot == 0 && P.slot_free[0] ? r.red[P_CF] : 0.0));
+}
+__device__ __forceinline__ double ride_diag_own(const double *__restrict__ scale, const double *__restrict__ colnorm,
+                                                long slot, double dmin, double dmax) {
+  const double sv = scale[slot];
+  return fmin(fmax(sv * sv * colnorm[slot], dmin), dmax);
 }
 
 __device__ __forceinline__ double robustify_row(int kind, double a, double &r, double J[13]) {
@@ -311,18 +327,19 @@
   }
 }
 
+template <int kFlight>
 __device__ __forceinline__ void tag_reduce_elem(const DevProblem &P, const double *__restrict__ obs_tg, long e,
                                                 double *__restrict__ g, double *__restrict__ colnorm) {
   if (e >= 12L * P.nt) return;
   const int t = (int)(e / 12), j = (int)(e % 12);
   double s = 0.0;
   const int qa = P.tag_start[t], qb = P.tag_start[t + 1];
-  for (int q0 = qa; q0 < qb; q0 += 32) {
-    double v[32];
-#pragma unroll
-    for (int u = 0; u < 32; ++u) v[u] = obs_tg[12L * min(q0 + u, qb - 1) + j];
-#pragma unroll
-    for (int u = 0; u < 32; ++u) s += (q0 + u < qb) ? v[u] : 0.0;
+  for (int q0 = qa; q0 < qb; q0 += kFlight) {
+    double v[kFlight];
+#pragma unroll
+    for (int u = 0; u < kFlight; ++u) v[u] = obs_tg[12L * min(q0 + u, qb - 1) + j];
+#pragma unroll
+    for (int u = 0; u < kFlight; ++u) s += (q0 + u < qb) ? v[u] : 0.0;
   }
   const long slot = slot_tag(P, t) + (j % 6);
   if (P.f_alias) {
@@ -395,14 +412,48 @@
   }
 }
 
+__device__ __forceinline__ double wave_tree_sum(double v, int n);
+__device__ __forceinline__ double wave_tree_max(double v, int n);
+
+__device__ __forceinline__ void reduce_parts_wave(int p, const double *__restrict__ parts, int nc,
+                                                  double *__restrict__ out, double *__restrict__ hout,
+                                                  double *__restrict__ save, int lane) {
+  const bool is_max = (p == P_YBAD || p == P_CBAD || p == NPART + 1);
+  const double *src = parts + (long)(p < NPART ? p : 0) * nc;
+  const int len = p < NPART ? nc : 0;
+  double r = tree1024_on_wave(
+      lane, len, [&](int i) { return src[i]; }, [&](double a, double b) { return is_max ? fmax(a, b) : a + b; }, 0.0);
+  r = is_max ? wave_tree_max(r, kWave) : wave_tree_sum(r, kWave);
+  if (lane == 0) {
+    out[p] = r;
+    if (hout) hout[p] = r;
+    if (save && p < 2) save[p] = r;
+    if (hout) __threadfence_system();
+  }
+}
+
+__device__ __forceinline__ void lin_reduce_rider(const DevProblem &P, const LinRide &r, int b, int lane) {
+  if (b < NPART + 2) reduce_parts_wave(b, r.parts, P.nc, r.red, r.hout, nullptr, lane);
+  else tag_reduce_elem<16>(P, r.obs_tg, (long)(b - (NPART + 2)) * kWave + lane, r.g, r.colnorm);
+}
+
 template <bool kBig>
 __global__ __launch_bounds__(kWave) void k_schur(DevProblem P, const double *__restrict__ scale,
                                                  const double *__restrict__ diag, double radius,
                                                  double *__restrict__ zero_tiles, long n_zero, ExecReset er,
-                                                 const int *__restrict__ cap_list) {
+                                                 const int *__restrict__ cap_list, LinRide ride,
+                                                 const double *__restrict__ own_colnorm) {
   extern __shared__ __attribute__((aligned(16))) double sm[];
   SCHUR_STAMP_INIT;
-  const int c = kBig ? cap_list[blockIdx.x] : (int)blockIdx.x, lane = threadIdx.x;
+  const int lane = threadIdx.x;
+  if (!kBig && ride.count) {
+    const int rb = (int)blockIdx.x - ride.first;
+    if (rb >= 0 && rb < ride.count) {
+      lin_reduce_rider(P, ride, rb, lane);
+      return;
+    }
+  }
+  const int c = kBig ? cap_list[blockIdx.x] : (int)blockIdx.x - ride.shift;
   if (c >= P.nc + n_zero) {
     exec_reset_elem(er, (long)(c - P.nc - n_zero) * kWave + lane);
     return;
@@ -545,10 +596,18 @@
     double L[21];
     double rd[6];
     int e = 0;
+    double dg[6];
+    if (ride.on) {
+#pragma unroll
+      for (int i = 0; i < 6; ++i) dg[i] = ride_diag_own(scale, own_colnorm, sc + i, ride.dmin, ride.dmax);
+    } else {
+#pragma unroll
+      for (int i = 0; i < 6; ++i) dg[i] = diag[sc + i];
+    }
 #pragma unroll
     for (int i = 0; i < 6; ++i)
 #pragma unroll
-      for (int j = 0; j <= i; ++j) L[e++] = U[6 * i + j] + (i == j ? lm_d2(diag, sc + i, radius) : 0.0);
+      for (int j = 0; j <= i; ++j) L[e++] = U[6 * i + j] + (i == j ? lm_d2v(dg[i], radius) : 0.0);
 #define LI6(i, j) L[(i) * ((i) + 1) / 2 + (j)]
 #pragma unroll
     for (int j = 0; j < 6; ++j) {
@@ -748,34 +807,53 @@
 }
 
 __device__ __forceinline__ double prep_d2(const DevProblem &P, const double *diag, double radius, long r,
-                                          long col) {
+                                          long col, const LinRide &ride) {
   if (!diag || r != col || r >= P.nR) return 0.0;
   const int slot = P.row_slot[r];
-  return slot >= 0 ? lm_d2(diag, slot, radius) : 0.0;
+  if (slot < 0) return 0.0;
+  return ride.on ? lm_d2v(ride_diag(P, ride, slot), radius) : lm_d2(diag, slot, radius);
 }
 
 __device__ __forceinline__ void prep_pad_row(const DevProblem &P, const double *diag, double radius, double *S,
-                                             long i) {
+                                             long i, const LinRide &ride) {
   if (i >= P.N) return;
   if (i < P.nR && P.row_slot[i] >= 0) {
     if (P.cam_row >= 0 && i > P.cam_row && i <= P.cam_row + 2)
-      *reduced_elem(S, P, i, i) = lm_d2(diag, P.row_slot[i], radius);
+      *reduced_elem(S, P, i, i) = ride.on ? lm_d2v(ride_diag(P, ride, P.row_slot[i]), radius)
+                                          : lm_d2(diag, P.row_slot[i], radius);
     return;
   }
   *reduced_elem(S, P, i, i) = i == P.nR ? 1e300 : 1.0;
 }
 
+__device__ __forceinline__ void slot_norms_block(int b, long n, long cap_lo, long cap_hi,
+                                                 const unsigned char *__restrict__ free_,
+                                                 const unsigned char *__restrict__ f_own, double *__restrict__ g,
+                                                 double *__restrict__ colnorm, const double *__restrict__ red,
+                                                 const double *__restrict__ x, double *__restrict__ out,
+                                                 double *__restrict__ hout, const double *__restrict__ scale,
+                                                 double dmin, double dmax, double *__restrict__ diag, double seq);
+
 __global__ __launch_bounds__(256) void k_schur_gather(DevProblem P, double *__restrict__ S,
-                                                      const double *__restrict__ diag, double radius) {
+                                                      const double *__restrict__ diag, double radius, LinRide ride) {
   __shared__ double part[4][kWave];
   __shared__ SchurContrib cts[4][kWave];
+  if (ride.count) {
+    const int rb = (int)blockIdx.x - ride.first;
+    if (rb >= 0 && rb < ride.count) {
+      slot_norms_block(rb, P.n, 3L, 3L + 6L * P.nc, P.slot_free, P.f_own, ride.g, ride.colnorm, ride.red, ride.x,
+                       ride.norms, ride.norms_hout, ride.scale, ride.dmin, ride.dmax, ride.diag, ride.seq);
+      return;
+    }
+  }
+  const int bid = (int)blockIdx.x - ride.shift;
   const int w = threadIdx.x >> 6, lane = threadIdx.x & 63;
   const int n_item_blocks = (P.n_items + 3) / 4;
-  if (diag && (int)blockIdx.x >= n_item_blocks) {
-    prep_pad_row(P, diag, radius, S, (long)(blockIdx.x - n_item_blocks) * 256 + threadIdx.x);
+  if (diag && bid >= n_item_blocks) {
+    prep_pad_row(P, diag, radius, S, (long)(bid - n_item_blocks) * 256 + threadIdx.x, ride);
     return;
   }
-  const int it = blockIdx.x * 4 + w;
+  const int it = bid * 4 + w;
   if (it >= P.n_items) return;
   const int4 item = P.gather_items[it];
   const int2 rr = P.dest_row[item.x];
@@ -810,7 +888,8 @@
     P.gather_part[(long)item.w * 36 + lane] = s;
   } else {
     const long r = rr.x + g.i, col = rr.y + g.j;
-    if (r >= col && !(diag && r == P.nR && col == P.nR)) *reduced_elem(S, P, r, col) = s + prep_d2(P, diag, radius, r, col);
+    if (r >= col && !(diag && r == P.nR && col == P.nR))
+      *reduced_elem(S, P, r, col) = s + prep_d2(P, diag, radius, r, col, ride);
   }
 }
 
@@ -837,7 +916,7 @@
   s = gather_groups(s, g, part[w], lane);
   const long r = rr.x + g.i, col = rr.y + g.j;
   if (lane < g.E && r >= col && !(diag && r == P.nR && col == P.nR))
-    *reduced_elem(S, P, r, col) = s + prep_d2(P, diag, radius, r, col);
+    *reduced_elem(S, P, r, col) = s + prep_d2(P, diag, radius, r, col, LinRide{});
 }
 
 __global__ void k_prep_reduced(DevProblem P, const double *__restrict__ diag, double radius,
@@ -1204,24 +1283,22 @@
   if ((int)blockIdx.x < NPART + 2)
     reduce_parts_block(blockIdx.x, parts, P.nc, nullptr, 0, out, nullptr, red, hout, nullptr, 0.0, save);
   else
-    tag_reduce_elem(P, obs_tg, (long)(blockIdx.x - (NPART + 2)) * 1024 + threadIdx.x, g, colnorm);
-}
-
-
-__global__ __launch_bounds__(256) void k_slot_norms(long n, long cap_lo, long cap_hi,
-                                                    const unsigned char *__restrict__ free_,
-                                                    const unsigned char *__restrict__ f_own,
-                                                    double *__restrict__ g, double *__restrict__ colnorm,
-                                                    const double *__restrict__ red,
-                                                    const double *__restrict__ x,
-                                                    double *__restrict__ out,
-                                                    double *__restrict__ hout, const double *__restrict__ scale,
-                                                    double dmin, double dmax, double *__restrict__ diag, double seq) {
+    tag_reduce_elem<32>(P, obs_tg, (long)(blockIdx.x - (NPART + 2)) * 1024 + threadIdx.x, g, colnorm);
+}
+
+
+__device__ __forceinline__ void slot_norms_block(int b, long n, long cap_lo, long cap_hi,
+                                                 const unsigned char *__restrict__ free_,
+                                                 const unsigned char *__restrict__ f_own, double *__restrict__ g,
+                                                 double *__restrict__ colnorm, const double *__restrict__ red,
+                                                 const double *__restrict__ x, double *__restrict__ out,
+                                                 double *__restrict__ hout, const double *__restrict__ scale,
+                                                 double dmin, double dmax, double *__restrict__ diag, double seq) {
   __shared__ double rs[6][256];
   __shared__ int last;
   const int t = threadIdx.x;
   const double g0 = free_[0] ? red[P_GF] : 0.0;
-  if (blockIdx.x == 0 && t == 0) {
+  if (b == 0 && t == 0) {
     g[0] = g0;
     colnorm[0] = free_[0] ? red[P_CF] : 0.0;
     g[1] = g[2] = 0.0;
@@ -1229,7 +1306,7 @@
   }
   const double cn0 = free_[0] ? red[P_CF] : 0.0;
   double v[6] = {0, 0, 0, 0, 0, 0};
-  for (long i = (long)blockIdx.x * 256 + t; i < n; i += (long)kNormBlocks * 256) {
+  for (long i = (long)b * 256 + t; i < n; i += (long)kNormBlocks * 256) {
     if (diag) {
       const double cn = i >= 3 ? colnorm[i] : (i == 0 ? cn0 : 0.0);
       diag[i] = fmin(fmax(scale[i] * scale[i] * cn, dmin), dmax);
@@ -1262,7 +1339,7 @@
   double *part = out + 8;
   int *done = reinterpret_cast<int *>(out + 7);
   if (t == 0) {
-    for (int q = 0; q < 6; ++q) part[6L * blockIdx.x + q] = rs[q][0];
+    for (int q = 0; q < 6; ++q) part[6L * b + q] = rs[q][0];
     __threadfence();
     last = atomicAdd(done, 1) == kNormBlocks - 1;
   }
@@ -1301,6 +1378,19 @@
     __syncthreads();
     if (t == 0) __hip_atomic_store(hout + kHostSeq, seq, __ATOMIC_RELEASE, __HIP_MEMORY_SCOPE_SYSTEM);
   }
+}
+
+__global__ __launch_bounds__(256) void k_slot_norms(long n, long cap_lo, long cap_hi,
+                                                    const unsigned char *__restrict__ free_,
+                                                    const unsigned char *__restrict__ f_own,
+                                                    double *__restrict__ g, double *__restrict__ colnorm,
+                                                    const double *__restrict__ red,
+                                                    const double *__restrict__ x,
+                                                    double *__restrict__ out,
+                                                    double *__restrict__ hout, const double *__restrict__ scale,
+                                                    double dmin, double dmax, double *__restrict__ diag, double seq) {
+  slot_norms_block(blockIdx.x, n, cap_lo, cap_hi, free_, f_own, g, colnorm, red, x, out, hout, scale, dmin, dmax, diag,
+                   seq);
 }
 
 __global__ void k_pack(PackSegs sg, double *__restrict__ buf, int unpack) {
@@ -1456,8 +1546,11 @@
 }
 
 void launch_schur(const DevProblem &P, const double *x, const double *scale, const double *diag,
-                  double radius, double *S, hipStream_t s, bool prep, long zero_tiles, const ExecReset *er) {
+                  double radius, double *S, hipStream_t s, bool prep, long zero_tiles, const ExecReset *er,
+                  const LinRide *ride) {
   const ExecReset r = er ? *er : ExecReset{};
+  if (ride && ride->on && (P.nc == 0 || !prep || P.f_alias))
+    throw ApiError(ARSLAM_E_STATE, "launch_schur: the linearization's riders on a launch that cannot carry them");
   if (P.nc == 0) {
     if (zero_tiles) (void)hipMemsetAsync(S, 0, (size_t)zero_tiles * 4096 * sizeof(double), s);
     if (prep) launch_prep_reduced(P, diag, radius, S, s);
@@ -1465,16 +1558,26 @@
   }
   const size_t lds = schur_lds_bytes(std::min(P.max_blk_per_cap, kSchurMfmaBlocks));
   const long reset_blocks = (r.n() + kWave - 1) / kWave;
-  hipLaunchKernelGGL(k_schur<false>, dim3((unsigned)(P.nc + zero_tiles + reset_blocks)), dim3(kWave), lds, s, P, scale,
-                     diag, radius, S, zero_tiles, r, (const int *)nullptr);
+  const long own_blocks = P.nc + zero_tiles + reset_blocks;
+  LinRide rd = ride ? *ride : LinRide{};
+  auto place = [&](long own, long riders) {
+    rd.count = rd.on ? (int)riders : 0;
+    rd.first = rd.front ? 0 : (int)own;
+    rd.shift = rd.front ? rd.count : 0;
+  };
+  place(own_blocks, NPART + 2 + (12L * P.nt + kWave - 1) / kWave);
+  hipLaunchKernelGGL(k_schur<false>, dim3((unsigned)(own_blocks + rd.count)), dim3(kWave), lds, s, P, scale, diag,
+                     radius, S, zero_tiles, r, (const int *)nullptr, rd, rd.colnorm);
   if (P.n_big_caps > 0) {
     const size_t lds_big = schur_lds_bytes(P.max_blk_per_cap);
+    place(0, 0);
     hipLaunchKernelGGL(k_schur<true>, dim3((unsigned)P.n_big_caps), dim3(kWave), lds_big, s, P, scale, diag, radius, S,
-                       0L, ExecReset{}, P.big_caps);
+                       0L, ExecReset{}, P.big_caps, rd, rd.colnorm);
   }
   const double *pd = prep ? diag : nullptr;
   const unsigned gb = (unsigned)((P.n_items + 3) / 4) + (prep ? (unsigned)((P.N + 255) / 256) : 0u);
-  if (gb) hipLaunchKernelGGL(k_schur_gather, dim3(gb), dim3(256), 0, s, P, S, pd, radius);
+  place(gb, kNormBlocks);
+  if (gb + rd.count) hipLaunchKernelGGL(k_schur_gather, dim3(gb + rd.count), dim3(256), 0, s, P, S, pd, radius, rd);
   if (P.n_splits)
     hipLaunchKernelGGL(k_schur_combine, dim3((unsigned)((P.n_splits + 3) / 4)), dim3(256), 0, s, P, S, pd,
                        radius);
@@ -1482,7 +1585,7 @@
 
 void launch_schur_gather(const DevProblem &P, const double *diag, double radius, double *S, hipStream_t s) {
   const unsigned gb = (unsigned)((P.n_items + 3) / 4) + (unsigned)((P.N + 255) / 256);
-  hipLaunchKernelGGL(k_schur_gather, dim3(gb), dim3(256), 0, s, P, S, diag, radius);
+  hipLaunchKernelGGL(k_schur_gather, dim3(gb), dim3(256), 0, s, P, S, diag, radius, LinRide{});
   if (P.n_splits)
     hipLaunchKernelGGL(k_schur_combine, dim3((unsigned)((P.n_splits + 3) / 4)), dim3(256), 0, s, P, S, diag, radius);
 }
diff --git a/ar_slam_amd/csrc/lm_solve.hip b/ar_slam_amd/csrc/lm_solve.hip
--- a/ar_slam_amd/csrc/lm_solve.hip
+++ b/ar_slam_amd/csrc/lm_solve.hip
@@ -69,11 +69,26 @@
                            op == ARSLAM_OP_SUM ? ncclSum : ncclMax, comm, stream));
 }
 
-void arslam_lm::linearize_launch() {
+void arslam_lm::linearize_launch(bool defer) {
   h_lin.alloc(32);
-  const bool direct = !multi();
   timers[PH_LIN].start(stream);
   arslam::launch_linearize(P, x, d_g.p, d_colnorm.p, d_obs_tg.p, d_parts.p, stream);
+  lin_red_deferred = defer;
+  if (!defer) lin_reductions_launch();
+  timers[PH_LIN].stop(stream);
+}
+
+constexpr bool kLinRideFront = true;
+
+bool arslam_lm::lin_ride_ok() const {
+  return !dbg_separate_lin && !multi() && has_f && nc > 0 && !P.f_alias && !env.dag_trace && diag_in_lin &&
+         opt.factor_executor == 1;
+}
+
+void arslam_lm::lin_reductions_launch() {
+  const bool direct = !multi();
+  lin_red_deferred = false;
+  ++n_lin_separate;
   arslam::launch_lin_reduce(P, d_obs_tg.p, d_g.p, d_colnorm.p, d_parts.p, d_red.p, stream,
                             direct ? h_lin.p : nullptr, multi() ? d_red.p + kLinSave : nullptr);
   if (multi()) lin_xpending = true;
@@ -81,7 +96,6 @@
   lin_seq = direct ? next_seq(h_lin.p + 16 + arslam::kHostSeq) : 0.0;
   arslam::launch_slot_norms(P, d_red.p, d_g.p, d_colnorm.p, x, d_norms_p, stream, direct ? h_lin.p + 16 : nullptr,
                             diag_in_lin ? &ld : nullptr, lin_seq);
-  timers[PH_LIN].stop(stream);
 }
 
 void arslam_lm::lin_norms() {
@@ -257,6 +271,8 @@
                 ARSLAM_SOLVER_CONTINUE;
   comm_bytes = 0.0;
   comm_calls = 0;
+  lin_red_deferred = false;
+  n_lin_separate = n_lin_ride = 0;
 }
 
 bool arslam_lm::prepare_step(bool reuse_diag, arslam::ExecReset *er) {
@@ -389,8 +405,31 @@
   if (has_f) {
     timers[PH_SCHUR].start(stream);
     const bool fill_first_store = !multi() && opt.factor_executor == 1;
+    arslam::LinRide ride;
+    if (lin_red_deferred) {
+      fail_if(!lin_ride_ok() || reuse_diag, ARSLAM_E_STATE, "deferred linearization reductions on a step that cannot carry them");
+      lin_red_deferred = false;
+      ++n_lin_ride;
+      ride.on = 1;
+      ride.front = env.lin_ride_place ? std::strcmp(env.lin_ride_place, "front") == 0 : kLinRideFront;
+      ride.obs_tg = d_obs_tg.p;
+      ride.parts = d_parts.p;
+      ride.x = x;
+      ride.scale = d_scale.p;
+      ride.g = d_g.p;
+      ride.colnorm = d_colnorm.p;
+      ride.red = d_red.p;
+      ride.hout = h_lin.p;
+      ride.norms = d_norms_p;
+      ride.norms_hout = h_lin.p + 16;
+      ride.dmin = opt.min_lm_diagonal;
+      ride.dmax = opt.max_lm_diagonal;
+      ride.diag = d_diag.p;
+      ride.seq = lin_seq = next_seq(h_lin.p + 16 + arslam::kHostSeq);
+    }
     arslam::launch_schur(P, x, d_scale.p, d_diag.p, radius, Sp, stream, !multi(),
-                         fill_first_store ? n_clear : plan.n_tiles, reset_in_schur ? &er : nullptr);
+                         fill_first_store ? n_clear : plan.n_tiles, reset_in_schur ? &er : nullptr,
+                         ride.on ? &ride : nullptr);
     const bool force_indefinite = dbg_indefinite_mask >> std::min(solve_index, 63) & 1ull;
     if (multi()) arslam::launch_prep_reduced(P, d_diag.p, radius, Sp, stream, 0);
     else if (force_indefinite)
@@ -567,6 +606,7 @@
   for (;;) {
     const bool stop_rule = it.iteration >= o.max_num_iterations || tr.radius <= o.min_trust_region_radius;
     if (lin_pending && stop_rule) {
+      if (lin_red_deferred) lin_reductions_launch();
       complete_pending_lin();
       exchange_norms();
       lin_sync();
@@ -617,7 +657,7 @@
       double *old = x;
       x = xc;
       xc = old != xbest ? old : (d_xa.p != x && d_xa.p != xbest) ? d_xa.p : (d_xb.p != x && d_xb.p != xbest) ? d_xb.p : d_xbest.p;
-      linearize_launch();
+      linearize_launch(lin_ride_ok());
       lin_pending = true;
       it.step_is_successful = 1;
       tr.accepted(it.relative_decrease, o.max_trust_region_radius);
diff --git a/ar_slam_amd/lm.py b/ar_slam_amd/lm.py
--- a/ar_slam_amd/lm.py
+++ b/ar_slam_amd/lm.py
@@ -35,6 +35,7 @@
            "arslam_lm_debug_force_multirank", "arslam_lm_debug_break_dependency", "arslam_lm_debug_tag_pair_tile",
            "arslam_debug_reduced_plan", "arslam_debug_reduced_plan_side", "arslam_debug_schur_stamps", "arslam_debug_ceres_e_blocks",
            "arslam_debug_mixed_groups",
+           "arslam_lm_debug_separate_lin_reductions", "arslam_lm_debug_lin_reduction_launches",
            "arslam_debug_dag_simulate", "arslam_debug_dag_simulate_started", "arslam_debug_dag_workgroup_limit",
            "arslam_debug_dag_fault_detail", "arslam_debug_box_fingerprint",
            "arslam_debug_rank_split", "arslam_debug_gather_extend", "arslam_debug_schur_store_table",
@@ -400,6 +401,14 @@
     def debug_force_multirank(self, on=True):
         _check(lib().arslam_lm_debug_force_multirank(self._h, 1 if on else 0))
 
+    def debug_separate_lin_reductions(self, on=True):
+        _check(lib().arslam_lm_debug_separate_lin_reductions(self._h, 1 if on else 0))
+
+    def debug_lin_reduction_launches(self):
+        a, b = C.c_int(0), C.c_int(0)
+        _check(lib().arslam_lm_debug_lin_reduction_launches(self._h, C.byref(a), C.byref(b)))
+        return a.value, b.value
+
     def set_comm(self, rank, nranks, uid):
         if callable(uid):
             fn = uid
diff --git a/include/arslam_lm_debug.h b/include/arslam_lm_debug.h
--- a/include/arslam_lm_debug.h
+++ b/include/arslam_lm_debug.h
@@ -73,6 +73,8 @@
 int arslam_lm_debug_force_indefinite(arslam_lm *h, unsigned long long step_mask);
 int arslam_lm_debug_break_dependency(arslam_lm *h, long ticket, long *broken);
 int arslam_lm_debug_force_multirank(arslam_lm *h, int on);
+int arslam_lm_debug_separate_lin_reductions(arslam_lm *h, int on);
+int arslam_lm_debug_lin_reduction_launches(arslam_lm *h, int *separate, int *ridealong);
 int arslam_lm_debug_tag_pair_tile(arslam_lm *h, const double *tag_a, const double *tag_b, int *status);
 
 int arslam_debug_ceres_e_blocks(const arslam_soa_problem *p, int out[4]);
```
